# whwu95/MVFNet

Measured on AMD Instinct MI355X. Metric: clips/sec (fwd+bwd) MVFNet-R50 8x8 224^2, higher is better.
Workload: dtype bf16; 1 GPU; MVFNet-ResNet50 8x8, 32 clips/GPU of 8x3x224x224, bf16, train step: fwd (batch-stat BN) + loss + bwd + clip + SGD-nesterov; all through the HIP C ABI (stem + 16 bottlenecks + MVF + TSN head); clips_per_gpu=32, frames_per_clip=8, parallelism=dp1: replicas, one flat gradient all-reduce per step

## Files before the change

### include/mvfnet_hip.h

```cpp
#ifndef MVFNET_HIP_H
#define MVFNET_HIP_H

#include <stddef.h>
#include <stdint.h>

#ifdef __cplusplus
extern "C" {
#endif

#define MVF_ABI_VERSION 2

enum { MVF_OK = 0, MVF_EINVAL = -1, MVF_ESHAPE = -2, MVF_EWS = -3, MVF_EHIP = -4, MVF_EUNSUPPORTED = -5 };
enum { MVF_F32 = 0, MVF_BF16 = 1 };
enum { MVF_NCHW = 0, MVF_NHWC = 1 };
enum { MVF_VIEW_T = 1, MVF_VIEW_H = 2, MVF_VIEW_W = 4 };

int mvf_abi_version(void);
const char* mvf_last_error(void);

typedef struct {
    int32_t nt, c, h, w;
    int32_t n_segment;
    int32_t cs;
    int32_t mode;
// ... 34 lines not shown
    int32_t relu;
    int32_t split_c;
    int32_t x2_pix_stride;
    int32_t in_dil;
    int32_t res_c0;
    int32_t x_c0;
} mvf_conv_desc_t;

int mvf_conv2d_nhwc_fwd(const mvf_conv_desc_t* d, const void* x, const void* x2, const void* w_packed,
                        const float* bias, const void* residual, void* y, void* stream);
size_t mvf_conv2d_workspace_bytes(const mvf_conv_desc_t* d);
int mvf_conv2d_nhwc_fwd_ws(const mvf_conv_desc_t* d, const void* x, const void* x2, const void* w_packed,
                           const float* bias, const void* residual, void* y, void* ws, size_t ws_bytes, void* stream);
int mvf_conv2d_nhwc_fwd_mvf(const mvf_conv_desc_t* d, const void* x, const void* w_packed, const float* bias, const float* mvf_coef,
                            int cs, int n_segment, int act, void* y, void* ws, size_t ws_bytes, void* stream);
int mvf_conv2d_nhwc_fwd_bnapply(const mvf_conv_desc_t* d, const void* x, const void* x2, const void* w_packed, const float* bn_scale,
                                const float* bn_shift, const void* residual, const float* res_scale, const float* res_shift, void* out,
                                unsigned char* sign_bits, void* ws, size_t ws_bytes, void* stream);
int mvf_conv2d_nhwc_fwd_bnbwd_sums(const mvf_conv_desc_t* d, const void* x, const void* x2, const void* w_packed, const void* g,
                                   const unsigned char* sign_bits, const float* bn_mean, const float* bn_invstd, float* sums_part, void* ws,
                                   size_t ws_bytes, void* stream);
int mvf_conv2d_nhwc_fwd_bnbwd_apply(const mvf_conv_desc_t* d, const void* x, const void* x2, const void* w_packed, const void* g,
                                    const unsigned char* sign_bits, const float* bn_gamma, const float* bn_mean, const float* bn_invstd,
                                    const float* dgamma, const float* dbeta, void* dz, void* ws, size_t ws_bytes, void* stream);
int mvf_conv2d_nhwc_fwd_resmask(const mvf_conv_desc_t* d, const void* x, const void* x2, const void* w_packed,
                                const float* bias, const void* residual, const unsigned char* res_sign_bits, void* y,
                                void* ws, size_t ws_bytes, void* stream);
int mvf_conv2d_nhwc_fwd_resmask_gate(const mvf_conv_desc_t* d, const void* x, const void* x2, const void* w_packed, const float* bias,
                                     const void* residual, const unsigned char* res_sign_bits, const unsigned char* out_gate_bits, void* y,
                                     void* ws, size_t ws_bytes, void* stream);
int mvf_conv2d_nhwc_fwd_resmask_gate_colsums(const mvf_conv_desc_t* d, const void* x, const void* x2, const void* w_packed, const void* residual,
                                             const unsigned char* res_sign_bits, const unsigned char* out_gate_bits, void* y, float* sums_part, void* ws,
                                             size_t ws_bytes, void* stream);
int mvf_conv2d_nhwc_dgrad_bnsums(const mvf_conv_desc_t* d, const void* dz, const void* w_packed_dgrad, void* y, const void* bn_z,
                                 const float* bn_mean, const float* bn_invstd, const float* bn_scale, const float* bn_shift,
                                 float* sums_part, void* ws, size_t ws_bytes, void* stream);
int mvf_bn_bwd_finalize(const float* sums_part, int nblk, int c, float* dgamma, float* dbeta, void* stream);
int mvf_conv2d_stats_rows(const mvf_conv_desc_t* d);
int mvf_conv2d_nhwc_fwd_stats(const mvf_conv_desc_t* d, const void* x, const void* x2, const void* w_packed, void* y,
                              float* stats_part, const float* stats_shift, void* ws, size_t ws_bytes, void* stream);

int mvf_pack_conv_weight(const float* w_oihw, int cout, int cin, int kh, int kw, int kw_pad, int cin_pad,
                         const float* scale, void* w_packed, int dtype, void* stream);
int mvf_bn_fold(const float* gamma, const float* beta, const float* mean, const float* var, float eps, int c,
                float* scale, float* shift, void* stream);

int mvf_stem_prep(const float* x_nchw, int n, int c, int h, int w, int pad, int wp, void* out, int dtype, void* stream);

int mvf_frames_prep_u8(const unsigned char* frames_hwc, int n, int hs, int ws, const int* window, int h, int w,
                       const float* mean3, const float* std3, int to_rgb, int div_255, int pad, int wp, void* out_stem,
                       float* out_nchw, int dtype, void* stream);
int mvf_frames_resample_u8(const unsigned char* frames_hwc, int n, int hs, int ws, const int* rows, int h, int w,
                           const float* mean3, const float* std3, int to_rgb, int div_255, int pad, int wp, void* out_stem,
                           float* out_nchw, int dtype, void* stream);
int mvf_frames_resample_color_u8(const unsigned char* frames_hwc, int n, int hs, int ws, const int* rows, const float* color, int h, int w,
                                 const float* mean3, const float* std3, int to_rgb, int div_255, int pad, int wp, void* out_stem,
                                 float* out_nchw, int dtype, void* stream);
int mvf_frames_gather_resample_u8(const unsigned char* frames_hwc, int n_src, int hs, int ws, const int* src_index, int n_out, const int* rows,
                                  const float* color, int h, int w, const float* mean3, const float* std3, int to_rgb, int div_255, int pad,
                                  int wp, void* out_stem, float* out_nchw, int dtype, void* stream);
int mvf_frames_yuv420_gather_resample_u8(const unsigned char* frames, int n_src, int hs, int ws, int pitch, int layout, int standard, int order,
                                         const int* src_index, int n_out, const int* rows, const float* color, int h, int w, const float* mean3,
                                         const float* std3, int to_rgb, int div_255, int pad, int wp, void* out_stem, float* out_nchw, int dtype,
                                         void* stream);

int mvf_maxpool3x3s2_nhwc(const void* x, int n, int h, int w, int c, void* y, int dtype, void* stream);

int mvf_head_pool_fc(const void* feat, int clips, int t, int hw, int c, const float* fc_w, const float* fc_b,
                     int classes, float* pooled_ws, float* scores, int dtype, void* stream);
int mvf_average_clip(const float* scores, int clips, int classes, int kind, float* out, void* stream);

int mvf_conv2d_nhwc_dgrad_bnsums_split(const mvf_conv_desc_t* d, const void* x, const void* x2, const void* w_packed, const float* bias, void* y,
                                       const void* bn_z, const float* bn_mean, const float* bn_invstd, const float* bn_scale, const float* bn_shift,
                                       float* sums_part, void* ws, size_t ws_bytes, void* stream);
int mvf_bn_bwd_dzfree_prep(const void* w_packed_dgrad, int c, int k, const float* gamma, const float* mean, const float* invstd, const float* dgamma,
                           const float* dbeta, long m, void* w_out, float* bias_out, int dtype, void* stream);
int mvf_bn_bwd_dzfree_wgrad(float* dw, const void* w_packed, const float* gram, const float* a_mean, const float* gamma, const float* mean,
                            const float* invstd, const float* dgamma, const float* dbeta, long m, int c, int k, int dtype, void* stream);
int mvf_bn_bwd_dzfree_sums(const float* q, const void* w_packed, int c, int k, const float* mean, const float* invstd, const float* part_lo, int rows_lo,
                           int c_split, const float* part_hi, int rows_hi, float* dgamma, float* dbeta, int dtype, void* stream);
size_t mvf_bn_workspace_bytes(long m, int c);
int mvf_bn_train_stats(const void* z, long m, int c, const float* gamma, const float* beta, float eps, float momentum,
                       float* running_mean, float* running_var, float* save_mean, float* save_invstd, float* scale,
                       float* shift, void* ws, size_t ws_bytes, int dtype, void* stream);
int mvf_bn_train_finalize(const float* part, int nblk, long m, int c, const float* gamma, const float* beta, float eps,
                          float momentum, float* running_mean, float* running_var, float* save_mean, float* save_invstd,
                          float* scale, float* shift, void* stream);
int mvf_bn_train_stats_gram(const float* gram, const float* a_mean, const void* w_packed, long m, int c, int k, const float* gamma, const float* beta,
                            float eps, float momentum, float* running_mean, float* running_var, float* save_mean, float* save_invstd, float* scale,
                            float* shift, int dtype, void* stream);
int mvf_bn_apply_colmeans(const void* z, long m, int c, const float* scale, const float* shift, int act, void* out, float* mean_out, void* ws,
                          size_t ws_bytes, int dtype, void* stream);
int mvf_bn_apply(const void* z, long m, int c, const float* scale, const float* shift, const void* residual,
                 const float* rscale, const float* rshift, int act, void* out, int dtype, void* stream);
int mvf_bn_bwd_reduce(const void* g, int g_pitch, const void* z, const void* ymask, long m, int c, const float* mean,
                      const float* invstd, const float* scale, const float* shift, int mask_mode, void* gm_out,
                      float* dgamma, float* dbeta, void* ws, size_t ws_bytes, int dtype, void* stream);
int mvf_bn_bwd_apply(const void* g, int g_pitch, const void* z, long m, int c, const float* gamma, const float* mean,
                     const float* invstd, const float* scale, const float* shift, const float* dgamma,
                     const float* dbeta, int mask_mode, void* dz, int dtype, void* stream);
int mvf_bn_apply_bits(const void* z, long m, int c, const float* scale, const float* shift, const void* residual,
                      const float* rscale, const float* rshift, int relu, void* out, unsigned char* sign_bits, int dtype,
                      void* stream);
int mvf_bn_bwd_apply_masked(const void* g, int g_pitch, const void* z, const void* ymask, long m, int c, const float* gamma,
                            const float* mean, const float* invstd, const float* scale, const float* shift,
                            const float* dgamma, const float* dbeta, int mask_mode, void* dz, int dtype, void* stream);
int mvf_bn_bwd_pair(const void* g, int g_pitch, const void* z_a, const void* z_b, const unsigned char* sign_bits, long m, int c,
                    const float* gamma_a, const float* mean_a, const float* invstd_a, float* dgamma_a, float* dbeta_a,
                    const float* gamma_b, const float* mean_b, const float* invstd_b, float* dgamma_b, float* dbeta_b,
                    void* dz_a, void* dz_b, void* ws, size_t ws_bytes, int dtype, void* stream);
int mvf_bn_bwd_wgrad_splits(long m, int c, int k, int nbn, int mask_mode);
size_t mvf_bn_bwd_wgrad_slab_bytes(long m, int c, int k, int nbn, int mask_mode);
int mvf_bn_bwd_apply_wgrad(const void* g, int g_pitch, const void* z, const void* ymask, long m, int c, const float* gamma, const float* mean,
                           const float* invstd, const float* scale, const float* shift, const float* dgamma, const float* dbeta, int mask_mode,
                           void* dz, const void* x, int x_pitch, int k, float* slabs, size_t slab_bytes, int dtype, void* stream);
int mvf_bn_bwd_pair_wgrad(const void* g, int g_pitch, const void* z_a, const void* z_b, const unsigned char* sign_bits, long m, int c,
                          const float* gamma_a, const float* mean_a, const float* invstd_a, float* dgamma_a, float* dbeta_a,
                          const float* gamma_b, const float* mean_b, const float* invstd_b, float* dgamma_b, float* dbeta_b,
                          void* dz_a, void* dz_b, const void* x_a, int xa_pitch, const void* x_b, int xb_pitch, int k,
                          float* slabs_a, float* slabs_b, size_t slab_bytes, void* ws, size_t ws_bytes, int dtype, void* stream);
int mvf_conv1x1_bwd_fused_splits(long m, int c, int k);
int mvf_conv1x1_bwd_fused(const void* a_in, int a_pitch, const void* w_packed, const void* g, int g_pitch, const unsigned char* sign_bits, long m, int c,
                          int k, const float* gamma, const float* mean, const float* invstd, const float* dgamma, const float* dbeta, const void* z_in,
                          const float* in_mean, const float* in_invstd, const float* in_scale, const float* in_shift, void* dx, float* sums_part,
                          int sums_rows, float* slabs, size_t slab_bytes, int dtype, void* stream);
int mvf_conv1x1_bnbwd_sums_pair(const void* a_in, int a_pitch, const void* w_a, const void* x_in, int x_pitch, const void* w_b, const void* g, int g_pitch,
                                const unsigned char* sign_bits, long m, int c, int k, const float* mean_a, const float* invstd_a, const float* mean_b,
                                const float* invstd_b, float* part_a, float* part_b, int rows, int dtype, void* stream);
int mvf_wgrad_slab_reduce(const float* slabs, int nsplit, int cout, int k, float* dw_oihw, void* stream);
int mvf_maxpool_bn_relu_fwd(const void* z, int n, int h, int w, int c, const float* scale, const float* shift, void* y,
                            unsigned char* argmax, int dtype, void* stream);
int mvf_maxpool_bn_relu_bwd(const unsigned char* argmax, const void* g, int n, int h, int w, int c, void* ga, int dtype,
                            void* stream);
int mvf_maxpool_bwd_sums_rows(int n, int h);
int mvf_maxpool_bn_relu_bwd_apply(const unsigned char* argmax, const void* g, int n, int h, int w, int c, const void* z, const float* gamma,
                                  const float* mean, const float* invstd, const float* scale, const float* shift, const float* dgamma,
                                  const float* dbeta, void* dz, int dtype, void* stream);
int mvf_maxpool_bn_relu_bwd_sums(const unsigned char* argmax, const void* g, int n, int h, int w, int c, void* ga, const void* z, const float* mean,
                                 const float* invstd, const float* scale, const float* shift, float* sums_part, int dtype, void* stream);
int mvf_head_train_fwd(const void* feat, int clips, int t, int hw, int c, const float* fc_w, const float* fc_b, int classes,
                       const long long* labels, const float* drop_mask ,
                       float* pooled, float* scores, float* dscores, float* loss_part, float* loss, int dtype, void* stream);
int mvf_ce_loss(const float* scores, const long long* labels, int clips, int classes, float* dscores, float* loss_part, float* loss,
                void* stream);
int mvf_head_train_bwd(const float* dscores, const float* pooled, const float* fc_w, const float* drop_mask, int clips, int t,
                       int hw, int c, int classes, float* dfc_w, float* dfc_b, float* dpool_ws , void* dfeat, int dtype,
                       void* stream);
size_t mvf_conv2d_wgrad_workspace_bytes(const mvf_conv_desc_t* d);
int mvf_conv2d_nhwc_wgrad(const mvf_conv_desc_t* d, const void* dz, const void* x, const void* x2, int kw_real,
                          int cin_real, int kw_packed, int cin_packed, float* dw_oihw, void* ws, size_t ws_bytes,
                          void* stream);
int mvf_conv2d_nhwc_wgrad_wgs(const mvf_conv_desc_t* d, const void* dz, const void* x, const void* x2, int kw_real,
                              int cin_real, int kw_packed, int cin_packed, float* dw_oihw, void* ws, size_t ws_bytes, int wgs, void* stream);
typedef struct {
    const float* w;
    void* out;
    int cout, cin, kh, kw, kw_pad, cin_pad;
    int kind, first_block;
} mvf_pack_job_t;
int mvf_pack_conv_weights_batched(const mvf_pack_job_t* jobs_dev, int njobs, int total_blocks, int dtype, void* stream);

int mvf_pack_conv_weight_dgrad(const float* w_oihw, int cout, int cin, int kh, int kw, void* w_packed, int dtype,
                               void* stream);
int mvf_nhwc_stencil(const mvf_desc_t* d, const void* x, int x_c, void* out, int out_c, const float* w_t,
                     const float* w_h, const float* w_w, const float* scale, const float* shift, int flip,
                     const void* addend, int addend_c, const unsigned char* addend_sign_bits, void* stream);
int mvf_nhwc_stencil_gate(const mvf_desc_t* d, const void* x, int x_c, void* out, int out_c, const float* w_t,
                          const float* w_h, const float* w_w, const float* scale, const float* shift, int flip,
                          const void* addend, int addend_c, const unsigned char* addend_sign_bits,
                          const unsigned char* out_gate_bits, void* stream);
int mvf_nhwc_stencil_gate_colsums(const mvf_desc_t* d, const void* x, int x_c, void* out, int out_c, const float* w_t, const float* w_h,
                                  const float* w_w, int flip, const void* addend, int addend_c, const unsigned char* addend_sign_bits,
                                  const unsigned char* out_gate_bits, float* sums_part, void* stream);
int mvf_nhwc_stencil_stats_rows(const mvf_desc_t* d, int x_c, int out_c);
int mvf_nhwc_stencil_tile_plan(const mvf_desc_t* d, int x_c, int out_c, int* rows_per_band, int* chan_per_wg);
int mvf_nhwc_stencil_stats(const mvf_desc_t* d, const void* x, int x_c, void* out, int out_c, const float* w_t, const float* w_h,
                           const float* w_w, float* stats_part, const float* stats_shift, void* stream);
size_t mvf_nhwc_tapgrad_workspace_bytes(const mvf_desc_t* d);
int mvf_nhwc_tapgrad(const mvf_desc_t* d, const void* x, int x_c, const void* dy, int dy_c, float* dw_t, float* dw_h,
                     float* dw_w, void* ws, size_t ws_bytes, void* stream);
size_t mvf_sgd_workspace_bytes(long n);
int mvf_sgd_nesterov_step(float* params, const float* grads, float* momentum_buf, long n, float grad_scale, float max_norm,
                          float lr, float momentum, float weight_decay, int first_step, float* norm_out, void* ws,
                          size_t ws_bytes, void* stream);
typedef struct mvf_sgd_segment {
    long long first;
    float lr_mult, decay_mult;
} mvf_sgd_segment_t;
int mvf_sgd_step_segments(float* params, const float* grads, float* momentum_buf, long n, float grad_scale, float max_norm, float lr,
                          float momentum, float weight_decay, int first_step, int nesterov, const mvf_sgd_segment_t* segments, int nseg,
                          float* norm_out, void* ws, size_t ws_bytes, void* stream);

enum { MVF_PLAN_CALL = 0, MVF_PLAN_RECORD = 1, MVF_PLAN_WAIT = 2 };
typedef struct mvf_plan_op {
    int kind, n_int, n_flt, reserved;
    void* fn;
    long long word0, float0;
} mvf_plan_op_t;
int mvf_plan_run(const mvf_plan_op_t* ops, int n_ops, const unsigned long long* words, const float* floats, int* failed_op);

#ifdef __cplusplus
}
#endif
#endif
```

### mvfnet_amd/_lib.py

```python
import ctypes as C
import os

import torch

_HERE = os.path.dirname(os.path.abspath(__file__))
LIB_PATH = os.environ.get("MVF_LIB_PATH") or os.path.join(_HERE, "libmvfnet_hip.so")

MVF_F32, MVF_BF16 = 0, 1
MVF_NCHW, MVF_NHWC = 0, 1
VIEW_T, VIEW_H, VIEW_W = 1, 2, 4
MODE_BITS = {"T": 1, "TH": 3, "THW": 7}
ERRNAMES = {-1: "MVF_EINVAL", -2: "MVF_ESHAPE", -3: "MVF_EWS", -4: "MVF_EHIP", -5: "MVF_EUNSUPPORTED"}


class MvfDesc(C.Structure):
    _fields_ = [("nt", C.c_int32), ("c", C.c_int32), ("h", C.c_int32), ("w", C.c_int32), ("n_segment", C.c_int32),
                ("cs", C.c_int32), ("mode", C.c_int32), ("layout", C.c_int32), ("dtype", C.c_int32)]


class ConvDesc(C.Structure):
    _fields_ = [("n", C.c_int32), ("h", C.c_int32), ("w", C.c_int32), ("cin", C.c_int32), ("cout", C.c_int32),
                ("kh", C.c_int32), ("kw", C.c_int32), ("stride", C.c_int32), ("pad", C.c_int32),
                ("ho", C.c_int32), ("wo", C.c_int32), ("x_pix_stride", C.c_int32),
                ("dtype", C.c_int32), ("relu", C.c_int32), ("split_c", C.c_int32), ("x2_pix_stride", C.c_int32), ("in_dil", C.c_int32),
# ... 27 lines not shown
    lib.mvf_last_error.restype = C.c_char_p
    lib.mvf_last_error.argtypes = []
    lib.mvf_fwd_infer.restype = i32
    lib.mvf_fwd_infer.argtypes = [dp, vp, vp, fp, fp, fp, fp, fp, vp]
    lib.mvf_fwd_train_workspace_bytes.restype = sz
    lib.mvf_fwd_train_workspace_bytes.argtypes = [dp]
    lib.mvf_fwd_train.restype = i32
    lib.mvf_fwd_train.argtypes = [dp, vp, vp, fp, fp, fp, fp, fp, f32, f32, fp, fp, fp, fp, vp, sz, vp]
    lib.mvf_bwd_workspace_bytes.restype = sz
    lib.mvf_bwd_workspace_bytes.argtypes = [dp]
    lib.mvf_bwd.restype = i32
    lib.mvf_bwd.argtypes = [dp, vp, vp, fp, fp, fp, fp, fp, fp, fp, i32, vp, fp, fp, fp, fp, fp, vp, sz, vp]
    lib.mvf_fwd_infer_slice.restype = i32
    lib.mvf_fwd_infer_slice.argtypes = [dp, vp, vp, fp, fp, fp, fp, fp, vp]
    cp = C.POINTER(ConvDesc)
    lib.mvf_conv2d_nhwc_fwd.restype = i32
    lib.mvf_conv2d_nhwc_fwd.argtypes = [cp, vp, vp, vp, fp, vp, vp, vp]
    lib.mvf_conv2d_workspace_bytes.restype = sz
    lib.mvf_conv2d_workspace_bytes.argtypes = [cp]
    lib.mvf_conv2d_nhwc_fwd_ws.restype = i32
    lib.mvf_conv2d_nhwc_fwd_ws.argtypes = [cp, vp, vp, vp, fp, vp, vp, vp, sz, vp]
    lib.mvf_conv2d_nhwc_dgrad_bnsums.restype = i32
    lib.mvf_conv2d_nhwc_dgrad_bnsums.argtypes = [cp, vp, vp, vp, vp, fp, fp, fp, fp, fp, vp, sz, vp]
    lib.mvf_bn_bwd_finalize.restype = i32
    lib.mvf_bn_bwd_finalize.argtypes = [fp, i32, i32, fp, fp, vp]
    lib.mvf_conv2d_nhwc_fwd_bnapply.restype = i32
    lib.mvf_conv2d_nhwc_fwd_bnapply.argtypes = [cp, vp, vp, vp, fp, fp, vp, fp, fp, vp, vp, vp, sz, vp]
    lib.mvf_conv2d_nhwc_fwd_bnbwd_sums.restype = i32
    lib.mvf_conv2d_nhwc_fwd_bnbwd_sums.argtypes = [cp, vp, vp, vp, vp, vp, fp, fp, fp, vp, sz, vp]
    lib.mvf_conv2d_nhwc_fwd_bnbwd_apply.restype = i32
    lib.mvf_conv2d_nhwc_fwd_bnbwd_apply.argtypes = [cp, vp, vp, vp, vp, vp, fp, fp, fp, fp, fp, vp, vp, sz, vp]
    lib.mvf_conv2d_nhwc_fwd_resmask.restype = i32
    lib.mvf_conv2d_nhwc_fwd_resmask.argtypes = [cp, vp, vp, vp, fp, vp, vp, vp, vp, sz, vp]
    i64_ = C.c_long
    lib.mvf_conv2d_nhwc_fwd_resmask_gate.restype = i32
    lib.mvf_conv2d_nhwc_fwd_resmask_gate.argtypes = [cp, vp, vp, vp, fp, vp, vp, vp, vp, vp, sz, vp]
    lib.mvf_conv2d_nhwc_fwd_resmask_gate_colsums.restype = i32
    lib.mvf_conv2d_nhwc_fwd_resmask_gate_colsums.argtypes = [cp, vp, vp, vp, vp, vp, vp, vp, fp, vp, sz, vp]
    lib.mvf_nhwc_stencil_gate_colsums.restype = i32
    lib.mvf_nhwc_stencil_gate_colsums.argtypes = [dp, vp, i32, vp, i32, fp, fp, fp, i32, vp, i32, vp, vp, fp, vp]
    lib.mvf_conv2d_nhwc_dgrad_bnsums_split.restype = i32
    lib.mvf_conv2d_nhwc_dgrad_bnsums_split.argtypes = [cp, vp, vp, vp, fp, vp, vp, fp, fp, fp, fp, fp, vp, sz, vp]
    lib.mvf_bn_bwd_dzfree_prep.restype = i32
    lib.mvf_bn_bwd_dzfree_prep.argtypes = [vp, i32, i32, fp, fp, fp, fp, fp, i64_, vp, fp, i32, vp]
    lib.mvf_bn_bwd_dzfree_wgrad.restype = i32
    lib.mvf_bn_bwd_dzfree_wgrad.argtypes = [fp, vp, fp, fp, fp, fp, fp, fp, fp, i64_, i32, i32, i32, vp]
    lib.mvf_bn_bwd_dzfree_sums.restype = i32
    lib.mvf_bn_bwd_dzfree_sums.argtypes = [fp, vp, i32, i32, fp, fp, fp, i32, i32, fp, i32, fp, fp, i32, vp]
    lib.mvf_nhwc_stencil_stats_rows.restype = i32
    lib.mvf_nhwc_stencil_stats_rows.argtypes = [dp, i32, i32]
    lib.mvf_nhwc_stencil_tile_plan.restype = i32
    lib.mvf_nhwc_stencil_tile_plan.argtypes = [dp, i32, i32, C.POINTER(C.c_int), C.POINTER(C.c_int)]
    lib.mvf_nhwc_stencil_stats.restype = i32
    lib.mvf_nhwc_stencil_stats.argtypes = [dp, vp, i32, vp, i32, fp, fp, fp, fp, fp, vp]
    lib.mvf_nhwc_stencil_gate.restype = i32
    lib.mvf_nhwc_stencil_gate.argtypes = [dp, vp, i32, vp, i32, fp, fp, fp, fp, fp, i32, vp, i32, vp, vp, vp]
    lib.mvf_conv2d_stats_rows.restype = i32
    lib.mvf_conv2d_stats_rows.argtypes = [cp]
    lib.mvf_conv2d_nhwc_fwd_stats.restype = i32
    lib.mvf_conv2d_nhwc_fwd_stats.argtypes = [cp, vp, vp, vp, vp, fp, fp, vp, sz, vp]
    lib.mvf_pack_conv_weight.restype = i32
    lib.mvf_pack_conv_weight.argtypes = [fp, i32, i32, i32, i32, i32, i32, fp, vp, i32, vp]
    lib.mvf_pack_conv_weights_batched.restype = i32
    lib.mvf_pack_conv_weights_batched.argtypes = [vp, i32, i32, i32, vp]
    lib.mvf_bn_fold.restype = i32
    lib.mvf_bn_fold.argtypes = [fp, fp, fp, fp, f32, i32, fp, fp, vp]
    lib.mvf_stem_prep.restype = i32
    lib.mvf_stem_prep.argtypes = [fp, i32, i32, i32, i32, i32, i32, vp, i32, vp]
    lib.mvf_frames_prep_u8.restype = i32
    lib.mvf_frames_prep_u8.argtypes = [vp, i32, i32, i32, vp, i32, i32, C.POINTER(C.c_float), C.POINTER(C.c_float),
                                       i32, i32, i32, i32, vp, vp, i32, vp]
    lib.mvf_frames_resample_u8.restype = i32
    lib.mvf_frames_resample_u8.argtypes = [vp, i32, i32, i32, vp, i32, i32, C.POINTER(C.c_float), C.POINTER(C.c_float),
                                           i32, i32, i32, i32, vp, vp, i32, vp]
    lib.mvf_frames_resample_color_u8.restype = i32
    lib.mvf_frames_resample_color_u8.argtypes = [vp, i32, i32, i32, vp, vp, i32, i32, C.POINTER(C.c_float), C.POINTER(C.c_float),
                                                 i32, i32, i32, i32, vp, vp, i32, vp]
    lib.mvf_frames_gather_resample_u8.restype = i32
    lib.mvf_frames_gather_resample_u8.argtypes = [vp, i32, i32, i32, vp, i32, vp, vp, i32, i32, C.POINTER(C.c_float), C.POINTER(C.c_float),
                                                  i32, i32, i32, i32, vp, vp, i32, vp]
    lib.mvf_frames_yuv420_gather_resample_u8.restype = i32
    lib.mvf_frames_yuv420_gather_resample_u8.argtypes = [vp, i32, i32, i32, i32, i32, i32, i32, vp, i32, vp, vp, i32, i32, C.POINTER(C.c_float),
                                                         C.POINTER(C.c_float), i32, i32, i32, i32, vp, vp, i32, vp]
    lib.mvf_maxpool3x3s2_nhwc.restype = i32
    lib.mvf_maxpool3x3s2_nhwc.argtypes = [vp, i32, i32, i32, i32, vp, i32, vp]
    lib.mvf_head_pool_fc.restype = i32
    lib.mvf_head_pool_fc.argtypes = [vp, i32, i32, i32, i32, fp, fp, i32, fp, fp, i32, vp]
    lib.mvf_average_clip.restype = i32
    lib.mvf_average_clip.argtypes = [fp, i32, i32, i32, fp, vp]
    i64, ll = C.c_long, C.c_void_p
    lib.mvf_bn_workspace_bytes.restype = sz
    lib.mvf_bn_workspace_bytes.argtypes = [i64, i32]
    lib.mvf_bn_train_stats.restype = i32
    lib.mvf_bn_train_stats.argtypes = [vp, i64, i32, fp, fp, f32, f32, fp, fp, fp, fp, fp, fp, vp, sz, i32, vp]
    lib.mvf_bn_train_finalize.restype = i32
    lib.mvf_bn_train_finalize.argtypes = [fp, i32, i64, i32, fp, fp, f32, f32, fp, fp, fp, fp, fp, fp, vp]
    lib.mvf_bn_train_stats_gram.restype = i32
    lib.mvf_bn_train_stats_gram.argtypes = [fp, fp, vp, i64, i32, i32, fp, fp, f32, f32, fp, fp, fp, fp, fp, fp, i32, vp]
    lib.mvf_bn_apply_colmeans.restype = i32
    lib.mvf_bn_apply_colmeans.argtypes = [vp, i64, i32, fp, fp, i32, vp, fp, vp, sz, i32, vp]
    lib.mvf_bn_apply.restype = i32
    lib.mvf_bn_apply.argtypes = [vp, i64, i32, fp, fp, vp, fp, fp, i32, vp, i32, vp]
    lib.mvf_bn_apply_bits.restype = i32
    lib.mvf_bn_apply_bits.argtypes = [vp, i64, i32, fp, fp, vp, fp, fp, i32, vp, vp, i32, vp]
    lib.mvf_bn_bwd_apply_masked.restype = i32
    lib.mvf_bn_bwd_apply_masked.argtypes = [vp, i32, vp, vp, i64, i32, fp, fp, fp, fp, fp, fp, fp, i32, vp, i32, vp]
    lib.mvf_bn_bwd_reduce.restype = i32
    lib.mvf_bn_bwd_reduce.argtypes = [vp, i32, vp, vp, i64, i32, fp, fp, fp, fp, i32, vp, fp, fp, vp, sz, i32, vp]
    lib.mvf_bn_bwd_apply.restype = i32
    lib.mvf_bn_bwd_apply.argtypes = [vp, i32, vp, i64, i32, fp, fp, fp, fp, fp, fp, fp, i32, vp, i32, vp]
    lib.mvf_maxpool_bn_relu_fwd.restype = i32
    lib.mvf_maxpool_bn_relu_fwd.argtypes = [vp, i32, i32, i32, i32, fp, fp, vp, vp, i32, vp]
    lib.mvf_maxpool_bn_relu_bwd.restype = i32
    lib.mvf_maxpool_bn_relu_bwd.argtypes = [vp, vp, i32, i32, i32, i32, vp, i32, vp]
    lib.mvf_maxpool_bwd_sums_rows.restype = i32
    lib.mvf_maxpool_bwd_sums_rows.argtypes = [i32, i32]
    lib.mvf_maxpool_bn_relu_bwd_apply.restype = i32
    lib.mvf_maxpool_bn_relu_bwd_apply.argtypes = [vp, vp, i32, i32, i32, i32, vp, fp, fp, fp, fp, fp, fp, fp, vp, i32, vp]
    lib.mvf_maxpool_bn_relu_bwd_sums.restype = i32
    lib.mvf_maxpool_bn_relu_bwd_sums.argtypes = [vp, vp, i32, i32, i32, i32, vp, vp, fp, fp, fp, fp, fp, i32, vp]
    lib.mvf_head_train_fwd.restype = i32
    lib.mvf_head_train_fwd.argtypes = [vp, i32, i32, i32, i32, fp, fp, i32, ll, fp, fp, fp, fp, fp, fp, i32, vp]
    lib.mvf_conv2d_nhwc_fwd_mvf.restype = i32
    lib.mvf_conv2d_nhwc_fwd_mvf.argtypes = [cp, vp, vp, fp, fp, i32, i32, i32, vp, vp, sz, vp]
    lib.mvf_bn_bwd_pair.restype = i32
    lib.mvf_bn_bwd_pair.argtypes = [vp, i32, vp, vp, vp, i64, i32, fp, fp, fp, fp, fp, fp, fp, fp, fp, fp, vp, vp, vp, sz, i32, vp]
    lib.mvf_bn_bwd_wgrad_splits.restype = i32
    lib.mvf_bn_bwd_wgrad_splits.argtypes = [i64, i32, i32, i32, i32]
    lib.mvf_bn_bwd_wgrad_slab_bytes.restype = sz
    lib.mvf_bn_bwd_wgrad_slab_bytes.argtypes = [i64, i32, i32, i32, i32]
    lib.mvf_bn_bwd_apply_wgrad.restype = i32
    lib.mvf_bn_bwd_apply_wgrad.argtypes = [vp, i32, vp, vp, i64, i32, fp, fp, fp, fp, fp, fp, fp, i32, vp, vp, i32, i32, fp, sz, i32, vp]
    lib.mvf_bn_bwd_pair_wgrad.restype = i32
    lib.mvf_bn_bwd_pair_wgrad.argtypes = [vp, i32, vp, vp, vp, i64, i32, fp, fp, fp, fp, fp, fp, fp, fp, fp, fp, vp, vp, vp, i32, vp, i32, i32,
                                          fp, fp, sz, vp, sz, i32, vp]
    lib.mvf_conv1x1_bwd_fused_splits.restype = i32
    lib.mvf_conv1x1_bwd_fused_splits.argtypes = [i64, i32, i32]
    lib.mvf_conv1x1_bwd_fused.restype = i32
    lib.mvf_conv1x1_bwd_fused.argtypes = [vp, i32, vp, vp, i32, vp, i64, i32, i32, fp, fp, fp, fp, fp, vp, fp, fp, fp, fp, vp, fp, i32, fp, sz, i32, vp]
    lib.mvf_conv1x1_bnbwd_sums_pair.restype = i32
    lib.mvf_conv1x1_bnbwd_sums_pair.argtypes = [vp, i32, vp, vp, i32, vp, vp, i32, vp, i64, i32, i32, fp, fp, fp, fp, fp, fp, i32, i32, vp]
    lib.mvf_wgrad_slab_reduce.restype = i32
    lib.mvf_wgrad_slab_reduce.argtypes = [fp, i32, i32, i32, fp, vp]
    lib.mvf_ce_loss.restype = i32
    lib.mvf_ce_loss.argtypes = [fp, ll, i32, i32, fp, fp, fp, vp]
    lib.mvf_head_train_bwd.restype = i32
    lib.mvf_head_train_bwd.argtypes = [fp, fp, fp, fp, i32, i32, i32, i32, i32, fp, fp, fp, vp, i32, vp]
    lib.mvf_conv2d_wgrad_workspace_bytes.restype = sz
    lib.mvf_conv2d_wgrad_workspace_bytes.argtypes = [cp]
    lib.mvf_conv2d_nhwc_wgrad.restype = i32
    lib.mvf_conv2d_nhwc_wgrad.argtypes = [cp, vp, vp, vp, i32, i32, i32, i32, fp, vp, sz, vp]
    lib.mvf_conv2d_nhwc_wgrad_wgs.restype = i32
    lib.mvf_conv2d_nhwc_wgrad_wgs.argtypes = [cp, vp, vp, vp, i32, i32, i32, i32, fp, vp, sz, i32, vp]
    lib.mvf_pack_conv_weight_dgrad.restype = i32
    lib.mvf_pack_conv_weight_dgrad.argtypes = [fp, i32, i32, i32, i32, vp, i32, vp]
    lib.mvf_nhwc_stencil.restype = i32
    lib.mvf_nhwc_stencil.argtypes = [dp, vp, i32, vp, i32, fp, fp, fp, fp, fp, i32, vp, i32, vp, vp]
    lib.mvf_nhwc_tapgrad_workspace_bytes.restype = sz
    lib.mvf_nhwc_tapgrad_workspace_bytes.argtypes = [dp]
    lib.mvf_nhwc_tapgrad.restype = i32
    lib.mvf_nhwc_tapgrad.argtypes = [dp, vp, i32, vp, i32, fp, fp, fp, vp, sz, vp]
    lib.mvf_sgd_workspace_bytes.restype = sz
    lib.mvf_sgd_workspace_bytes.argtypes = [i64]
    lib.mvf_sgd_nesterov_step.restype = i32
    lib.mvf_sgd_nesterov_step.argtypes = [fp, fp, fp, i64, f32, f32, f32, f32, f32, i32, fp, vp, sz, vp]
    lib.mvf_sgd_step_segments.restype = i32
    lib.mvf_sgd_step_segments.argtypes = [fp, fp, fp, i64, f32, f32, f32, f32, f32, i32, i32, vp, i32, fp, vp, sz, vp]
    lib.mvf_plan_run.restype = i32
    lib.mvf_plan_run.argtypes = [C.POINTER(PlanOp), i32, C.POINTER(C.c_ulonglong), C.POINTER(C.c_float), C.POINTER(C.c_int)]
    missing = [n for n in declared_symbols() if hasattr(lib, n) and getattr(lib, n).argtypes is None]
    if missing:
        raise ImportError("mvfnet_amd._lib: no argtypes declared for %s" % missing)
    return lib


def check(rc, what=""):
    if rc != 0:
        msg = lib.mvf_last_error().decode("utf-8", "replace")
        raise RuntimeError("%s failed: %s (%s)" % (what or "libmvfnet_hip", ERRNAMES.get(rc, rc), msg))


def declared_symbols():
    import re
    hdr = os.path.join(os.path.dirname(_HERE), "include", "mvfnet_hip.h")
    txt = open(hdr).read()
    txt = re.sub(r"/\*.*?\*/", "", txt, flags=re.S)
    return sorted(set(re.findall(r"\b((?:mvf|mvfnet)_[a-z0-9_]+)\s*\(", txt)))


lib = _load()
```

### mvfnet_amd/csrc/common.h

```cpp
#pragma once
#include <hip/hip_runtime.h>
#include <stdlib.h>
#include <string.h>
#include <strings.h>
#include <stdint.h>
#include <stdio.h>

#include "mvfnet_hip.h"

void mvf_set_error(const char* fmt, ...);

#define MVF_HIP_OK(call)                                                                        \
    do {                                                                                        \
        hipError_t e__ = (call);                                                                \
        if (e__ != hipSuccess) {                                                                \
            mvf_set_error("%s:%d: %s -> %s", __FILE__, __LINE__, #call, hipGetErrorString(e__)); \
            return MVF_EHIP;                                                                    \
        }                                                                                       \
    } while (0)

#define MVF_REQUIRE(cond, code, ...)    \
    do {                                \
        if (!(cond)) {                  \
            mvf_set_error(__VA_ARGS__); \
            return (code);              \
        }                               \
    } while (0)

#define MVF_LAUNCH_CHECK()                                                              \
    do {                                                                                \
        hipError_t e__ = hipGetLastError();                                             \
        if (e__ != hipSuccess) {                                                        \
            mvf_set_error("%s:%d: launch -> %s", __FILE__, __LINE__, hipGetErrorString(e__)); \
            return MVF_EHIP;                                                            \
        }                                                                               \
    } while (0)

struct bf16_t {
    uint16_t v;
};

__device__ __forceinline__ float bf16_to_f32(uint16_t v) { return __uint_as_float(((uint32_t)v) << 16); }
typedef __bf16 mvf_bf16x2 __attribute__((ext_vector_type(2)));
typedef float mvf_f32x2 __attribute__((ext_vector_type(2)));
__device__ __forceinline__ uint32_t pack_bf16x2(float lo, float hi) {
    const mvf_f32x2 v = {lo, hi};
    const mvf_bf16x2 b = __builtin_convertvector(v, mvf_bf16x2);
    uint32_t u;
    __builtin_memcpy(&u, &b, 4);
    return u;
}
__device__ __forceinline__ uint16_t f32_to_bf16(float f) { return (uint16_t)(pack_bf16x2(f, 0.f) & 0xffffu); }

__device__ __forceinline__ float ldf(const float* p) { return *p; }
__device__ __forceinline__ float ldf(const bf16_t* p) { return bf16_to_f32(p->v); }
__device__ __forceinline__ void stf(float* p, float v) { *p = v; }
__device__ __forceinline__ void stf(bf16_t* p, float v) { p->v = f32_to_bf16(v); }

__device__ __forceinline__ float4 ld4(const float* p) { return *reinterpret_cast<const float4*>(p); }
__device__ __forceinline__ float4 ld4(const bf16_t* p) {
    uint2 r = *reinterpret_cast<const uint2*>(p);
    return make_float4(__uint_as_float(r.x << 16), __uint_as_float(r.x & 0xffff0000u),
                       __uint_as_float(r.y << 16), __uint_as_float(r.y & 0xffff0000u));
}
__device__ __forceinline__ void st4(float* p, float4 v) { *reinterpret_cast<float4*>(p) = v; }
__device__ __forceinline__ void st4(bf16_t* p, float4 v) {
    uint2 r;
    r.x = pack_bf16x2(v.x, v.y);
    r.y = pack_bf16x2(v.z, v.w);
    *reinterpret_cast<uint2*>(p) = r;
}

__device__ __forceinline__ float hswish_f(float u) { return u * fminf(fmaxf(u + 3.0f, 0.0f), 6.0f) * (1.0f / 6.0f); }
__device__ __forceinline__ float hswish_grad_f(float u) {
    float r6 = fminf(fmaxf(u + 3.0f, 0.0f), 6.0f);
    float inner = (u > -3.0f && u < 3.0f) ? 1.0f : 0.0f;
    return r6 * (1.0f / 6.0f) + u * inner * (1.0f / 6.0f);
}

static inline size_t align_up(size_t v, size_t a) { return (v + a - 1) / a * a; }

static inline bool mvf_policy_lookup(const char* name, long* out) {
    const char* p = getenv("MVF_POLICY");
    if (!p) return false;
    const size_t n = strlen(name);
    while (*p) {
        while (*p == ',' || *p == ';' || *p == ' ') ++p;
        const char* e = p;
        while (*e && *e != ',' && *e != ';') ++e;
        const char* eq = (const char*)memchr(p, '=', (size_t)(e - p));
        if (eq && (size_t)(eq - p) == n && strncasecmp(p, name, n) == 0) {
            *out = strtol(eq + 1, nullptr, 10);
            return true;
        }
        p = e;
    }
    return false;
}
static inline int mvf_policy_int(const char* name, int dflt) {
    long v;
    return mvf_policy_lookup(name, &v) ? (int)v : dflt;
}
static inline bool mvf_policy_has(const char* name) {
    long v;
    return mvf_policy_lookup(name, &v);
}

struct StemDirectArgs {
    const void* x;
    const void* w;
    void* y;
    const float* bias;
    float* stats_part;
    const float* stats_shift;
    int stats_rows, epi;
    int N, H, W, Ho, Wo;
    long wK;
};
struct Conv3x3C64Args {
    const void* x;
    const void* w;
    void* y;
    const float* bias;
    float* stats_part;
    const float* stats_shift;
    const void* bn_z;
    const float *bn_mean, *bn_invstd, *bn_scale, *bn_shift;
    int stats_rows, epi;
    int N, H, W, xps;
    long wK;
};
struct PwSumsArgs {
    const void* a;
    const void* w;
    const void* g;
    const unsigned char* bits;
    const float* c0;
    const float* c1;
    float* part;
    int rows, mode, M, N, K, xps;
};
struct Wgrad3x3C64Args {
    const void* dz;
    const void* x;
    float* part;
    int N, H, W, xps, nwg;
};
struct WgradStemArgs {
    const void* dz;
    const void* x;
    float* part;
    int N, H, W, Ho, Wo, nwg;
};
namespace mvf_internal {
struct BnBwdWgradArgs {
    const void* g;
    const void* z[2];
    const void* bits;
    const float *gamma[2], *mean[2], *invstd[2], *dgamma[2], *dbeta[2];
    const float *scale, *shift;
    void* dz[2];
    const void* x[2];
    int xps[2];
    float* part[2];
    int g_pitch, M, C, K;
    int rows_per_split, nsplit, ctiles, ktiles;
};
struct PwBwdFusedArgs {
    const void* a;
    const void* w;
    const void* g;
    const unsigned char* bits;
    const float *gamma, *mean, *invstd, *dgamma, *dbeta;
    const void* z_in;
    const float *in_scale, *in_shift, *in_mean, *in_invstd;
    void* dx;
    float* sums_part;
    float* part;
    int aps, g_pitch, M, sums_rows, rows_per_split, nsplit;
    int ablate;
};
struct PwSumsPairArgs {
    const void *a, *x;
    const void *w_a, *w_b;
    const void* g;
    const unsigned char* bits;
    const float *mean_a, *invstd_a, *mean_b, *invstd_b;
    float *part_a, *part_b;
    int aps, xps, g_pitch, M, rows, rows_per_split, nsplit;
};
int pw_sums_pair_launch(const PwSumsPairArgs& a, hipStream_t st);
int pw_bwd_fused_plan(long m, int c, int k, int* rows_per_split);
int pw_bwd_fused_launch(const PwBwdFusedArgs& a, hipStream_t st);
bool bnbwd_wgrad_tile(int c, int k, int nbn, int mask_mode, int* ct, int* kt);
int bnbwd_wgrad_plan(long m, int c, int k, int nbn, int mask_mode, int* rows_per_split, int* ctiles, int* ktiles);
int bnbwd_wgrad_launch(const BnBwdWgradArgs& a, int nbn, int mask_mode, hipStream_t st);
int wgrad_slab_reduce_launch(const float* part, int nsplit, int cout, int k, float* dw_oihw, hipStream_t st);
bool wgrad3x3_c64_ok(int n, int h, int w, int xps);
int wgrad3x3_c64_wgs(int n, int h);
int wgrad3x3_c64_launch(const Wgrad3x3C64Args& a, hipStream_t st);
bool wgrad_stem_ok(int n, int h, int w, int ho, int wo);
int wgrad_stem_wgs(int n, int ho);
int wgrad_stem_launch(const WgradStemArgs& a, hipStream_t st);
int stem_direct_launch(const StemDirectArgs& a, hipStream_t st);
int conv3x3_c64_launch(const Conv3x3C64Args& a, hipStream_t st);
int pw_sums_launch(const PwSumsArgs& a, hipStream_t st);
}

#ifdef __HIPCC__
typedef int i32x4 __attribute__((ext_vector_type(4)));
__device__ __forceinline__ i32x4 rsrc_words(const void* base, unsigned nbytes) {
    const unsigned long p = (unsigned long)base;
    i32x4 r;
    r.x = __builtin_amdgcn_readfirstlane((int)(unsigned)p);
    r.y = __builtin_amdgcn_readfirstlane((int)((unsigned)(p >> 32) & 0xffffu));
    r.z = __builtin_amdgcn_readfirstlane((int)nbytes);
    r.w = 0x00020000;
    return r;
}
__device__ __forceinline__ void glds16(const i32x4 rs, const unsigned lds_dst, const unsigned voff) {
    unsigned keep;
    asm volatile("s_mov_b32 %0, m0\n\ts_mov_b32 m0, %2\n\ts_nop 0\n\tbuffer_load_dwordx4 %1, %3, 0 offen lds\n\ts_mov_b32 m0, %0"
                 : "=&s"(keep) : "v"(voff), "s"(lds_dst), "s"(rs) : "memory");
}

#endif
```

### mvfnet_amd/csrc/train_ops.hip

```cpp
#include <algorithm>
#include <math.h>
#include <stdlib.h>

#include "common.h"

namespace {

constexpr int kThreads = 256;

struct ColPlan {
    int cqb;
    int rl;
    int gx;
    int gy;
    int rows;
};

ColPlan col_plan(long M, int C, int vn = 4, int blocks = 2048) {
    ColPlan p;
    const int cq = C / vn;
    int cqb = 1;
    while (cqb < cq && cqb < 64) cqb <<= 1;
    p.cqb = cqb;
    p.rl = kThreads / cqb;
    p.gx = (cq + cqb - 1) / cqb;
    long want = std::max<long>(1, blocks / p.gx);
    long rows = std::max<long>((M + want - 1) / want, (long)p.rl * 8);
    rows = (rows + p.rl - 1) / p.rl * p.rl;
    p.rows = (int)rows;
    p.gy = (int)((M + rows - 1) / rows);
    return p;
}

template <typename ET, int VN>
__device__ __forceinline__ void ldv(const ET* p, float (&f)[VN]) {
    if constexpr (sizeof(ET) == 4) {
        static_assert(VN == 4, "fp32 lane vector is 4 wide");
        const float4 v = *reinterpret_cast<const float4*>(p);
        f[0] = v.x; f[1] = v.y; f[2] = v.z; f[3] = v.w;
    } else if constexpr (VN == 4) {
        const uint2 r = *reinterpret_cast<const uint2*>(p);
        f[0] = __uint_as_float(r.x << 16); f[1] = __uint_as_float(r.x & 0xffff0000u);
        f[2] = __uint_as_float(r.y << 16); f[3] = __uint_as_float(r.y & 0xffff0000u);
    } else {
        static_assert(VN == 8, "bf16 lane vector is 4 or 8 wide");
        const uint4 r = *reinterpret_cast<const uint4*>(p);
        f[0] = __uint_as_float(r.x << 16); f[1] = __uint_as_float(r.x & 0xffff0000u);
        f[2] = __uint_as_float(r.y << 16); f[3] = __uint_as_float(r.y & 0xffff0000u);
        f[4] = __uint_as_float(r.z << 16); f[5] = __uint_as_float(r.z & 0xffff0000u);
        f[6] = __uint_as_float(r.w << 16); f[7] = __uint_as_float(r.w & 0xffff0000u);
    }
}
template <typename ET, int VN>
__device__ __forceinline__ void stv(ET* p, const float (&f)[VN]) {
    if constexpr (sizeof(ET) == 4) {
        *reinterpret_cast<float4*>(p) = make_float4(f[0], f[1], f[2], f[3]);
    } else if constexpr (VN == 4) {
        uint2 r;
        r.x = pack_bf16x2(f[0], f[1]);
        r.y = pack_bf16x2(f[2], f[3]);
        *reinterpret_cast<uint2*>(p) = r;
    } else {
        uint4 r;
        r.x = pack_bf16x2(f[0], f[1]);
        r.y = pack_bf16x2(f[2], f[3]);
        r.z = pack_bf16x2(f[4], f[5]);
        r.w = pack_bf16x2(f[6], f[7]);
        *reinterpret_cast<uint4*>(p) = r;
    }
}
template <int VN>
__device__ __forceinline__ void ldp(const float* p, int c, float (&f)[VN], float fill = 0.f) {
#pragma unroll
    for (int j = 0; j < VN; j += 4) {
        const float4 v = p ? *reinterpret_cast<const float4*>(p + c + j) : make_float4(fill, fill, fill, fill);
        f[j] = v.x; f[j + 1] = v.y; f[j + 2] = v.z; f[j + 3] = v.w;
    }
}

template <int VN>
__device__ __forceinline__ void rowlane_reduce(float (&a)[VN], float (&b)[VN], int cqb, int rl, float* red) {
    (void)rl;
    const int lane = threadIdx.x & 63, wave = threadIdx.x >> 6, cq = lane % cqb;
    for (int off = cqb; off < 64; off <<= 1) {
#pragma unroll
        for (int j = 0; j < VN; ++j) {
            a[j] += __shfl_xor(a[j], off, 64);
            b[j] += __shfl_xor(b[j], off, 64);
        }
    }
    if (lane < cqb) {
#pragma unroll
        for (int j = 0; j < VN; ++j) {
            red[((wave * 2 * VN) + 2 * j) * cqb + cq] = a[j];
            red[((wave * 2 * VN) + 2 * j + 1) * cqb + cq] = b[j];
        }
    }
    __syncthreads();
    if (threadIdx.x < cqb) {
#pragma unroll
        for (int j = 0; j < VN; ++j) {
            float s = 0.f, t = 0.f;
#pragma unroll
            for (int w = 0; w < kThreads / 64; ++w) {
                s += red[((w * 2 * VN) + 2 * j) * cqb + cq];
                t += red[((w * 2 * VN) + 2 * j + 1) * cqb + cq];
            }
            a[j] = s;
            b[j] = t;
        }
    }
}

template <typename ET, int VN>
__global__ __launch_bounds__(kThreads) void bn_stats_kernel(const ET* z, long M, int C, const float* kshift, int cqb, int rows,
                                                            float* part) {
    __shared__ float red[2 * VN * kThreads];
    const int rl = kThreads / cqb;
    const int cq = blockIdx.x * cqb + threadIdx.x % cqb, lane_r = threadIdx.x / cqb;
    const bool ok = cq * VN < C;
    const int c = cq * VN;
    float k[VN], s1[VN], s2[VN];
#pragma unroll
    for (int j = 0; j < VN; ++j) k[j] = s1[j] = s2[j] = 0.f;
    if (ok && kshift) ldp<VN>(kshift, c, k);
    const long r0 = (long)blockIdx.y * rows, r1 = min(M, r0 + rows);
    if (ok) {
        auto accum = [&](const float (&a)[VN]) {
#pragma unroll
            for (int j = 0; j < VN; ++j) {
                const float d = a[j] - k[j];
                s1[j] += d;
                s2[j] += d * d;
            }
        };
        long r = r0 + lane_r;
        for (; r + 3 * rl < r1; r += 4 * rl) {
            float a0[VN], a1[VN], a2[VN], a3[VN];
            ldv<ET, VN>(z + r * C + c, a0); ldv<ET, VN>(z + (r + rl) * C + c, a1);
            ldv<ET, VN>(z + (r + 2 * rl) * C + c, a2); ldv<ET, VN>(z + (r + 3 * rl) * C + c, a3);
            accum(a0); accum(a1); accum(a2); accum(a3);
        }
        for (; r < r1; r += rl) {
            float a0[VN];
            ldv<ET, VN>(z + r * C + c, a0);
            accum(a0);
        }
    }
    rowlane_reduce<VN>(s1, s2, cqb, rl, red);
    if (ok && lane_r == 0) {
        float* p = part + ((long)blockIdx.y * C + c) * 2;
#pragma unroll
        for (int j = 0; j < VN; ++j) { p[2 * j] = s1[j]; p[2 * j + 1] = s2[j]; }
    }
}

constexpr int kFinCh = 4;
// ... 624 lines not shown
template <typename ET>
__global__ __launch_bounds__(256) void maxpool_bn_bwd_rows_sums_kernel(const unsigned char* amax, const ET* g, int n, int h, int w, int c, int ho, int wo, ET* ga,
                                                                       const ET* z, const float* mean, const float* invstd, const float* scale, const float* shift,
                                                                       float* part, int nblk) {
    __shared__ float red[256 * 8];
    const int c4 = c >> 2;
    const int per = w * c4;
    const int cq = threadIdx.x % c4;
    const float4 sc = *reinterpret_cast<const float4*>(scale + cq * 4), sh = *reinterpret_cast<const float4*>(shift + cq * 4);
    const float4 mu = *reinterpret_cast<const float4*>(mean + cq * 4), rs = *reinterpret_cast<const float4*>(invstd + cq * 4);
    float s1[4] = {0.f, 0.f, 0.f, 0.f}, s2[4] = {0.f, 0.f, 0.f, 0.f};
    const int row_end = min(n * h, ((int)blockIdx.x + 1) * kPoolRB);
    for (int row = blockIdx.x * kPoolRB; row < row_end; ++row) {
        const int img = row / h, ih = row - img * h;
        for (int i = threadIdx.x; i < per; i += 256) {
            const int iw = i / c4;
            float acc[4] = {0.f, 0.f, 0.f, 0.f};
            unsigned amv[4];
            float4 gvv[4];
            bool okv[4];
            unsigned mev[4];
            const long zi = ((long)row * w + iw) * c + cq * 4;
            const float4 zv = ld4(z + zi);
#pragma unroll
            for (int k = 0; k < 4; ++k) {
                const int oh = (ih + (k >> 1)) >> 1, ow = (iw + (k & 1)) >> 1;
                okv[k] = oh < ho && ow < wo && ((k >> 1) == 0 || (ih & 1)) && ((k & 1) == 0 || (iw & 1));
                const int ohc = min(oh, ho - 1), owc = min(ow, wo - 1);
                mev[k] = (unsigned)(ih - (oh * 2 - 1)) * 3u + (unsigned)(iw - (ow * 2 - 1));
                const long oidx = (((long)img * ho + ohc) * wo + owc) * c + cq * 4;
                amv[k] = *reinterpret_cast<const unsigned*>(amax + oidx);
                gvv[k] = ld4(g + oidx);
            }
#pragma unroll
            for (int k = 0; k < 4; ++k) {
                const unsigned am = amv[k], me = mev[k];
                if (okv[k] && (am & 255u) == me) acc[0] += gvv[k].x;
                if (okv[k] && ((am >> 8) & 255u) == me) acc[1] += gvv[k].y;
                if (okv[k] && ((am >> 16) & 255u) == me) acc[2] += gvv[k].z;
                if (okv[k] && (am >> 24) == me) acc[3] += gvv[k].w;
            }
            if (ga) st4(ga + zi, make_float4(acc[0], acc[1], acc[2], acc[3]));
            if constexpr (sizeof(ET) == 2) {
#pragma unroll
                for (int j = 0; j < 4; ++j) acc[j] = bf16_to_f32(f32_to_bf16(acc[j]));
            }
            const float zz[4] = {zv.x, zv.y, zv.z, zv.w};
            const float scv[4] = {sc.x, sc.y, sc.z, sc.w}, shv[4] = {sh.x, sh.y, sh.z, sh.w};
            const float muv[4] = {mu.x, mu.y, mu.z, mu.w}, rsv[4] = {rs.x, rs.y, rs.z, rs.w};
#pragma unroll
            for (int j = 0; j < 4; ++j) {
                const float gm = (zz[j] * scv[j] + shv[j]) > 0.f ? acc[j] : 0.f;
                s1[j] += gm;
                s2[j] += gm * ((zz[j] - muv[j]) * rsv[j]);
            }
        }
    }
#pragma unroll
    for (int j = 0; j < 4; ++j) {
        red[(2 * j) * 256 + threadIdx.x] = s1[j];
        red[(2 * j + 1) * 256 + threadIdx.x] = s2[j];
    }
    __syncthreads();
    if ((int)threadIdx.x < c4 * 4) {
        const int q = threadIdx.x >> 2, j = threadIdx.x & 3;
        float a = 0.f, b = 0.f;
        for (int t = q; t < 256; t += c4) {
            a += red[(2 * j) * 256 + t];
            b += red[(2 * j + 1) * 256 + t];
        }
        reinterpret_cast<float2*>(part)[(long)(q * 4 + j) * nblk + blockIdx.x] = make_float2(a, b);
    }
}

template <typename ET>
__global__ __launch_bounds__(256) void maxpool_bn_bwd_rows_apply_kernel(const unsigned char* amax, const ET* g, int n, int h, int w, int c, int ho, int wo,
                                                                        const ET* z, const float* gamma, const float* mean, const float* invstd,
                                                                        const float* scale, const float* shift, const float* dgamma, const float* dbeta,
                                                                        float inv_m, ET* dz) {
    const int c4 = c >> 2;
    const int per = w * c4;
    const int cq = threadIdx.x % c4;
    float av[4], d0[4], kx[4], muv[4], scv[4], shv[4];
    {
        const float4 ga_ = *reinterpret_cast<const float4*>(gamma + cq * 4), rs = *reinterpret_cast<const float4*>(invstd + cq * 4);
        const float4 dg = *reinterpret_cast<const float4*>(dgamma + cq * 4), db = *reinterpret_cast<const float4*>(dbeta + cq * 4);
        const float4 mu = *reinterpret_cast<const float4*>(mean + cq * 4);
        const float4 sc = *reinterpret_cast<const float4*>(scale + cq * 4), sh = *reinterpret_cast<const float4*>(shift + cq * 4);
        const float gav[4] = {ga_.x, ga_.y, ga_.z, ga_.w}, rsv[4] = {rs.x, rs.y, rs.z, rs.w}, dgv[4] = {dg.x, dg.y, dg.z, dg.w}, dbv[4] = {db.x, db.y, db.z, db.w};
        const float mu_[4] = {mu.x, mu.y, mu.z, mu.w}, sc_[4] = {sc.x, sc.y, sc.z, sc.w}, sh_[4] = {sh.x, sh.y, sh.z, sh.w};
#pragma unroll
        for (int j = 0; j < 4; ++j) {
            av[j] = gav[j] * rsv[j];
            d0[j] = dbv[j] * inv_m;
            kx[j] = rsv[j] * dgv[j] * inv_m;
            muv[j] = mu_[j]; scv[j] = sc_[j]; shv[j] = sh_[j];
        }
    }
    const int row_end = min(n * h, ((int)blockIdx.x + 1) * kPoolRB);
    for (int row = blockIdx.x * kPoolRB; row < row_end; ++row) {
        const int img = row / h, ih = row - img * h;
        for (int i = threadIdx.x; i < per; i += 256) {
            const int iw = i / c4;
            float acc[4] = {0.f, 0.f, 0.f, 0.f};
            unsigned amv[4];
            float4 gvv[4];
            bool okv[4];
            unsigned mev[4];
            const long zi = ((long)row * w + iw) * c + cq * 4;
            const float4 zv = ld4(z + zi);
#pragma unroll
            for (int k = 0; k < 4; ++k) {
                const int oh = (ih + (k >> 1)) >> 1, ow = (iw + (k & 1)) >> 1;
                okv[k] = oh < ho && ow < wo && ((k >> 1) == 0 || (ih & 1)) && ((k & 1) == 0 || (iw & 1));
                const int ohc = min(oh, ho - 1), owc = min(ow, wo - 1);
                mev[k] = (unsigned)(ih - (oh * 2 - 1)) * 3u + (unsigned)(iw - (ow * 2 - 1));
                const long oidx = (((long)img * ho + ohc) * wo + owc) * c + cq * 4;
                amv[k] = *reinterpret_cast<const unsigned*>(amax + oidx);
                gvv[k] = ld4(g + oidx);
            }
#pragma unroll
            for (int k = 0; k < 4; ++k) {
                const unsigned am = amv[k], me = mev[k];
                if (okv[k] && (am & 255u) == me) acc[0] += gvv[k].x;
                if (okv[k] && ((am >> 8) & 255u) == me) acc[1] += gvv[k].y;
                if (okv[k] && ((am >> 16) & 255u) == me) acc[2] += gvv[k].z;
                if (okv[k] && (am >> 24) == me) acc[3] += gvv[k].w;
            }
            if constexpr (sizeof(ET) == 2) {
#pragma unroll
                for (int j = 0; j < 4; ++j) acc[j] = bf16_to_f32(f32_to_bf16(acc[j]));
            }
            const float zz[4] = {zv.x, zv.y, zv.z, zv.w};
            float o[4];
#pragma unroll
            for (int j = 0; j < 4; ++j) {
                const float gm = (zz[j] * scv[j] + shv[j]) > 0.f ? acc[j] : 0.f;
                o[j] = av[j] * (gm - d0[j] - (zz[j] - muv[j]) * kx[j]);
            }
            st4(dz + zi, make_float4(o[0], o[1], o[2], o[3]));
        }
    }
}

template <typename ET, int MODE>
__global__ __launch_bounds__(256) void maxpool_bn_bwd_blk_kernel(const unsigned char* amax, const ET* g, int n, int h, int w, int c, int ho, int wo, ET* ga,
                                                                 const ET* z, const float* gamma, const float* mean, const float* invstd, const float* scale,
                                                                 const float* shift, const float* dgamma, const float* dbeta, float inv_m, float* part, int nblk,
                                                                 ET* dz) {
    constexpr int VC = 16 / (int)sizeof(ET);
    __shared__ float red[MODE == 0 ? 256 * 2 * VC : 1];
    const int ncg = c / VC, hw2 = w >> 1, hb = h >> 1;
    const int cq = threadIdx.x % ncg;
    float scv[VC], shv[VC], muv[VC], k1[VC], k2[VC], k3[VC];
#pragma unroll
    for (int j = 0; j < VC; ++j) {
        const int ch = cq * VC + j;
        scv[j] = scale[ch]; shv[j] = shift[ch]; muv[j] = mean[ch];
        if constexpr (MODE == 0) { k1[j] = invstd[ch]; k2[j] = 0.f; k3[j] = 0.f; }
        else { k1[j] = gamma[ch] * invstd[ch]; k2[j] = dbeta[ch] * inv_m; k3[j] = invstd[ch] * dgamma[ch] * inv_m; }
    }
    float s1[VC], s2[VC];
#pragma unroll
    for (int j = 0; j < VC; ++j) { s1[j] = 0.f; s2[j] = 0.f; }
    auto ldv = [](const ET* p, float (&f)[VC]) {
        const uint4 u = *reinterpret_cast<const uint4*>(p);
        if constexpr (sizeof(ET) == 4) {
            f[0] = __uint_as_float(u.x); f[1] = __uint_as_float(u.y); f[2] = __uint_as_float(u.z); f[3] = __uint_as_float(u.w);
        } else {
            f[0] = __uint_as_float(u.x << 16); f[1] = __uint_as_float(u.x & 0xffff0000u); f[2] = __uint_as_float(u.y << 16); f[3] = __uint_as_float(u.y & 0xffff0000u);
            f[4] = __uint_as_float(u.z << 16); f[5] = __uint_as_float(u.z & 0xffff0000u); f[6] = __uint_as_float(u.w << 16); f[7] = __uint_as_float(u.w & 0xffff0000u);
        }
    };
    auto stv = [](ET* p, const float (&f)[VC]) {
        uint4 u;
        if constexpr (sizeof(ET) == 4) {
            u = make_uint4(__float_as_uint(f[0]), __float_as_uint(f[1]), __float_as_uint(f[2]), __float_as_uint(f[3]));
        } else {
            u = make_uint4(pack_bf16x2(f[0], f[1]), pack_bf16x2(f[2], f[3]), pack_bf16x2(f[4], f[5]), pack_bf16x2(f[6], f[7]));
        }
        *reinterpret_cast<uint4*>(p) = u;
    };
    const int items = (kPoolRB / 2) * hw2 * ncg;
    const long brows = (long)n * hb;
    for (int i = threadIdx.x; i < items; i += 256) {
        const int bi = i / ncg;
        const int br = bi / hw2, bw = bi - br * hw2;
        const long R = (long)blockIdx.x * (kPoolRB / 2) + br;
        if (R >= brows) break;
        const int img = (int)(R / hb), bh = (int)(R - (long)img * hb);
        float gv[4][VC], zv[4][VC];
        unsigned char am[4][VC];
        bool okw[4];
#pragma unroll
        for (int k = 0; k < 4; ++k) {
            const int oh = bh + (k >> 1), ow = bw + (k & 1);
            okw[k] = oh < ho && ow < wo;
            const long oidx = (((long)img * ho + min(oh, ho - 1)) * wo + min(ow, wo - 1)) * c + cq * VC;
            if constexpr (VC == 8) {
                const uint2 a8 = *reinterpret_cast<const uint2*>(amax + oidx);
#pragma unroll
                for (int j = 0; j < 4; ++j) { am[k][j] = (unsigned char)(a8.x >> (8 * j)); am[k][4 + j] = (unsigned char)(a8.y >> (8 * j)); }
            } else {
                const unsigned a4 = *reinterpret_cast<const unsigned*>(amax + oidx);
#pragma unroll
                for (int j = 0; j < 4; ++j) am[k][j] = (unsigned char)(a4 >> (8 * j));
            }
            ldv(g + oidx, gv[k]);
        }
        long zi[4];
#pragma unroll
        for (int p = 0; p < 4; ++p) {
            zi[p] = (((long)img * h + 2 * bh + (p >> 1)) * w + 2 * bw + (p & 1)) * c + cq * VC;
            ldv(z + zi[p], zv[p]);
        }
#pragma unroll
        for (int p = 0; p < 4; ++p) {
            const int a = p >> 1, b = p & 1;
            float acc[VC];
#pragma unroll
            for (int j = 0; j < VC; ++j) acc[j] = 0.f;
#pragma unroll
            for (int k = 0; k < 4; ++k) {
                const int wi = k >> 1, wj = k & 1;
                if ((wi == 1 && a == 0) || (wj == 1 && b == 0)) continue;
                const unsigned me = (unsigned)(a + 1 - 2 * wi) * 3u + (unsigned)(b + 1 - 2 * wj);
#pragma unroll
                for (int j = 0; j < VC; ++j)
                    if (okw[k] && am[k][j] == me) acc[j] += gv[k][j];
            }
            if constexpr (MODE == 0) {
                if (ga) stv(ga + zi[p], acc);
            }
            if constexpr (sizeof(ET) == 2) {
#pragma unroll
                for (int j = 0; j < VC; ++j) acc[j] = bf16_to_f32(f32_to_bf16(acc[j]));
            }
            if constexpr (MODE == 0) {
#pragma unroll
                for (int j = 0; j < VC; ++j) {
                    const float gm = (zv[p][j] * scv[j] + shv[j]) > 0.f ? acc[j] : 0.f;
                    s1[j] += gm;
                    s2[j] += gm * ((zv[p][j] - muv[j]) * k1[j]);
                }
            } else {
                float o[VC];
#pragma unroll
                for (int j = 0; j < VC; ++j) {
                    const float gm = (zv[p][j] * scv[j] + shv[j]) > 0.f ? acc[j] : 0.f;
                    o[j] = k1[j] * (gm - k2[j] - (zv[p][j] - muv[j]) * k3[j]);
                }
                stv(dz + zi[p], o);
            }
        }
    }
    if constexpr (MODE == 0) {
#pragma unroll
        for (int j = 0; j < VC; ++j) {
            red[(2 * j) * 256 + threadIdx.x] = s1[j];
            red[(2 * j + 1) * 256 + threadIdx.x] = s2[j];
        }
        __syncthreads();
        if ((int)threadIdx.x < c) {
            const int q = threadIdx.x / VC, j = threadIdx.x - q * VC;
            float a = 0.f, b = 0.f;
            for (int t = q; t < 256; t += ncg) {
                a += red[(2 * j) * 256 + t];
                b += red[(2 * j + 1) * 256 + t];
            }
            reinterpret_cast<float2*>(part)[(long)threadIdx.x * nblk + blockIdx.x] = make_float2(a, b);
        }
    }
}

template <typename ET>
__global__ void maxpool_bn_bwd_kernel(const unsigned char* amax, const ET* g, int n, int h, int w, int c, int ho, int wo, ET* ga) {
    const int c4 = c >> 2;
    const long total = (long)n * h * w * c4;
    for (long i = (long)blockIdx.x * blockDim.x + threadIdx.x; i < total; i += (long)gridDim.x * blockDim.x) {
        int cq, iw, ih, img;
        if (total <= 0x7fffffffL) {
            unsigned t = (unsigned)i;
            cq = (int)(t % (unsigned)c4); t /= (unsigned)c4;
            iw = (int)(t % (unsigned)w); t /= (unsigned)w;
            ih = (int)(t % (unsigned)h);
            img = (int)(t / (unsigned)h);
        } else {
            cq = (int)(i % c4);
            long t = i / c4;
            iw = (int)(t % w); t /= w;
            ih = (int)(t % h);
            img = (int)(t / h);
        }
        float acc[4] = {0.f, 0.f, 0.f, 0.f};
        unsigned amv[4];
        float4 gvv[4];
        bool okv[4];
        unsigned mev[4];
#pragma unroll
        for (int k = 0; k < 4; ++k) {
            const int oh = (ih + (k >> 1)) >> 1, ow = (iw + (k & 1)) >> 1;
            okv[k] = oh < ho && ow < wo && ((k >> 1) == 0 || (ih & 1)) && ((k & 1) == 0 || (iw & 1));
            const int ohc = min(oh, ho - 1), owc = min(ow, wo - 1);
            mev[k] = (unsigned)(ih - (oh * 2 - 1)) * 3u + (unsigned)(iw - (ow * 2 - 1));
            const long oidx = (((long)img * ho + ohc) * wo + owc) * c + cq * 4;
            amv[k] = *reinterpret_cast<const unsigned*>(amax + oidx);
            gvv[k] = ld4(g + oidx);
        }
#pragma unroll
        for (int k = 0; k < 4; ++k) {
            const unsigned am = amv[k], me = mev[k];
            if (okv[k] && (am & 255u) == me) acc[0] += gvv[k].x;
            if (okv[k] && ((am >> 8) & 255u) == me) acc[1] += gvv[k].y;
            if (okv[k] && ((am >> 16) & 255u) == me) acc[2] += gvv[k].z;
            if (okv[k] && (am >> 24) == me) acc[3] += gvv[k].w;
        }
        st4(ga + i * 4, make_float4(acc[0], acc[1], acc[2], acc[3]));
    }
}

template <typename ET>
__global__ void frame_pool_kernel(const ET* feat, int hw, int c, const float* drop_mask, float* pooled) {
    const int f = blockIdx.y, ch = blockIdx.x * blockDim.x + threadIdx.x;
    if (ch >= c) return;
    const ET* p = feat + (long)f * hw * c + ch;
    float s = 0.f;
    for (int r = 0; r < hw; ++r) s += ldf(p + (long)r * c);
    s = s / (float)hw;
    if (drop_mask) s *= drop_mask[(long)f * c + ch];
    pooled[(long)f * c + ch] = s;
}

__global__ void ce_loss_kernel(const float* scores, const long long* labels, int clips, int classes, float* loss_part, float* dscores) {
    __shared__ float red[256];
    const int cl = blockIdx.x, tid = threadIdx.x;
    const float* s = scores + (long)cl * classes;
    float mx = -INFINITY;
    for (int k = tid; k < classes; k += blockDim.x) mx = fmaxf(mx, s[k]);
    red[tid] = mx;
    __syncthreads();
    for (int o = blockDim.x >> 1; o > 0; o >>= 1) { if (tid < o) red[tid] = fmaxf(red[tid], red[tid + o]); __syncthreads(); }
    mx = red[0];
    __syncthreads();
    float e = 0.f;
    for (int k = tid; k < classes; k += blockDim.x) e += expf(s[k] - mx);
    red[tid] = e;
    __syncthreads();
    for (int o = blockDim.x >> 1; o > 0; o >>= 1) { if (tid < o) red[tid] += red[tid + o]; __syncthreads(); }
    const float den = red[0];
    const int lab = (int)labels[cl];
    if (tid == 0) loss_part[cl] = (logf(den) + mx) - s[lab];
    if (!dscores) return;
    for (int k = tid; k < classes; k += blockDim.x) {
        const float p = expf(s[k] - mx) / den;
        dscores[(long)cl * classes + k] = (p - (k == lab ? 1.f : 0.f)) / (float)clips;
    }
}

__global__ void mean_reduce_kernel(const float* v, int n, float* out) {
    if (blockIdx.x == 0 && threadIdx.x == 0) {
        double s = 0.0;
        for (int i = 0; i < n; ++i) s += v[i];
        out[0] = (float)(s / n);
    }
}

constexpr int kHeadKc = 4;
__global__ void head_clipmean_kernel(const float* pooled, int T, int c, float* pcm) {
    const int cl = blockIdx.y, ch = blockIdx.x * blockDim.x + threadIdx.x;
    if (ch >= c) return;
    float s = 0.f;
    for (int t = 0; t < T; ++t) s += pooled[((long)cl * T + t) * c + ch];
    pcm[(long)cl * c + ch] = s / (float)T;
}
__global__ __launch_bounds__(256) void head_fc_bwd_w_kernel(const float* dscores, const float* pcm, int clips, int T, int c, int classes, float* dw, float* db) {
    const int k0 = blockIdx.y * kHeadKc, ch = blockIdx.x * blockDim.x + threadIdx.x;
    const int nk = min(kHeadKc, classes - k0);
    if (ch < c) {
        float acc[kHeadKc];
#pragma unroll
        for (int j = 0; j < kHeadKc; ++j) acc[j] = 0.f;
        for (int cl0 = 0; cl0 < clips; cl0 += 16) {
            float pcv[16];
#pragma unroll
            for (int q = 0; q < 16; ++q) pcv[q] = pcm[(long)min(cl0 + q, clips - 1) * c + ch];
#pragma unroll
            for (int j = 0; j < kHeadKc; ++j) {
                if (j < nk) {
#pragma unroll
                    for (int q = 0; q < 16; ++q)
                        if (cl0 + q < clips) acc[j] += dscores[(long)(cl0 + q) * classes + k0 + j] * pcv[q];
                }
            }
        }
#pragma unroll
        for (int j = 0; j < kHeadKc; ++j)
            if (j < nk) dw[(long)(k0 + j) * c + ch] = acc[j];
    }
    if (blockIdx.x == 0 && threadIdx.x < nk) {
        float s = 0.f;
        for (int cl = 0; cl < clips; ++cl) s += dscores[(long)cl * classes + k0 + threadIdx.x];
        db[k0 + threadIdx.x] = s;
    }
}

__global__ void head_dpool_kernel(const float* dscores, const float* w, int classes, int c, float scale, float* dpool) {
    const int cl = blockIdx.y, ch = blockIdx.x * blockDim.x + threadIdx.x;
    if (ch >= c) return;
    float a[8] = {0.f, 0.f, 0.f, 0.f, 0.f, 0.f, 0.f, 0.f};
    const float* ds = dscores + (long)cl * classes;
    int k = 0;
    for (; k + 8 <= classes; k += 8) {
#pragma unroll
        for (int u = 0; u < 8; ++u) a[u] += ds[k + u] * w[(long)(k + u) * c + ch];
    }
    for (; k < classes; ++k) a[0] += ds[k] * w[(long)k * c + ch];
    dpool[(long)cl * c + ch] = (((a[0] + a[1]) + (a[2] + a[3])) + ((a[4] + a[5]) + (a[6] + a[7]))) * scale;
}
template <typename ET>
__global__ void head_dfeat_kernel(const float* dpool, const float* drop_mask, int T, int hw, int c, long total, ET* dfeat) {
    const int frame = blockIdx.y, c4 = c >> 2;
    const int per = hw * c4;
    for (int i = blockIdx.x * blockDim.x + threadIdx.x; i < per; i += gridDim.x * blockDim.x) {
        const int q = i % c4;
        float4 v = *reinterpret_cast<const float4*>(dpool + (long)(frame / T) * c + q * 4);
        if (drop_mask) {
            const float4 mk = *reinterpret_cast<const float4*>(drop_mask + (long)frame * c + q * 4);
            v.x *= mk.x; v.y *= mk.y; v.z *= mk.z; v.w *= mk.w;
        }
        st4(dfeat + ((long)frame * hw * c + (long)i * 4), v);
    }
}

__global__ void sqsum_partial_kernel(const float* g, long n, float* part) {
    __shared__ float red[256];
    float s = 0.f;
    for (long i = (long)blockIdx.x * blockDim.x + threadIdx.x; i < n; i += (long)gridDim.x * blockDim.x) s += g[i] * g[i];
    red[threadIdx.x] = s;
    __syncthreads();
    for (int o = blockDim.x >> 1; o > 0; o >>= 1) { if (threadIdx.x < o) red[threadIdx.x] += red[threadIdx.x + o]; __syncthreads(); }
    if (threadIdx.x == 0) part[blockIdx.x] = red[0];
}
__global__ void norm_finalize_kernel(const float* part, int nblk, float max_norm, float gscale, float* out ) {
    __shared__ double red[64];
    double acc = 0.0;
    for (int i = threadIdx.x; i < nblk; i += 64) acc += part[i];
    red[threadIdx.x] = acc;
    __syncthreads();
    if (blockIdx.x == 0 && threadIdx.x == 0) {
        double s = 0.0;
        for (int i = 0; i < 64; ++i) s += red[i];
        const float nrm = fabsf(gscale) * (float)sqrt(s);
        out[0] = nrm;
        float coef = max_norm > 0.f ? max_norm / (nrm + 1e-6f) : 1.f;
        out[1] = coef < 1.f ? coef : 1.f;
    }
}
__global__ void sgd_nesterov_kernel(float* p, const float* g, float* buf, long n, const float* coef_ptr, float gscale, float lr,
                                    float momentum, float wd, int first_step) {
    const float coef = (coef_ptr ? coef_ptr[1] : 1.f) * gscale;
    for (long i = (long)blockIdx.x * blockDim.x + threadIdx.x; i < n; i += (long)gridDim.x * blockDim.x) {
        const float pv = p[i];
        const float d = g[i] * coef + wd * pv;
        const float b = first_step ? d : momentum * buf[i] + d;
        buf[i] = b;
        p[i] = pv - lr * (d + momentum * b);
    }
}
__device__ __forceinline__ int seg_of(const mvf_sgd_segment_t* seg, int nseg, long i) {
    int lo = 0, hi = nseg - 1;
    while (lo < hi) {
        const int mid = (lo + hi + 1) >> 1;
        if (seg[mid].first <= i) lo = mid; else hi = mid - 1;
    }
    return lo;
}
__global__ void sqsum_segments_kernel(const float* g, long n, const mvf_sgd_segment_t* seg, int nseg, float* part) {
    __shared__ float red[256];
    float s = 0.f;
    for (long i = (long)blockIdx.x * blockDim.x + threadIdx.x; i < n; i += (long)gridDim.x * blockDim.x)
        if (seg[seg_of(seg, nseg, i)].lr_mult >= 0.f) s += g[i] * g[i];
    red[threadIdx.x] = s;
    __syncthreads();
    for (int o = blockDim.x >> 1; o > 0; o >>= 1) { if (threadIdx.x < o) red[threadIdx.x] += red[threadIdx.x + o]; __syncthreads(); }
    if (threadIdx.x == 0) part[blockIdx.x] = red[0];
}
__global__ void sgd_segments_kernel(float* p, const float* g, float* buf, long n, const float* coef_ptr, float gscale, float lr,
                                    float momentum, float wd, int first_step, int nesterov, const mvf_sgd_segment_t* seg, int nseg) {
    const float coef = (coef_ptr ? coef_ptr[1] : 1.f) * gscale;
    for (long i = (long)blockIdx.x * blockDim.x + threadIdx.x; i < n; i += (long)gridDim.x * blockDim.x) {
        const int lo = seg_of(seg, nseg, i);
        if (seg[lo].lr_mult < 0.f) continue;
        const float lr_i = lr * seg[lo].lr_mult, wd_i = wd * seg[lo].decay_mult;
        const float pv = p[i];
        const float d = g[i] * coef + wd_i * pv;
        const float b = first_step ? d : momentum * buf[i] + d;
        buf[i] = b;
        p[i] = pv - lr_i * (nesterov ? d + momentum * b : b);
    }
}

inline int grid_for(long total, int cap = 256 * 16) { return (int)std::min<long>((total + 255) / 256, cap); }

}

extern "C" {

size_t mvf_bn_workspace_bytes(long m, int c) {
    if (m <= 0 || c <= 0 || c % 4) return 0;
    int gy = col_plan(m, c, 4).gy;
    if (c % 8 == 0) gy = std::max(gy, col_plan(m, c, 8).gy);
    return align_up((size_t)gy * c * 2 * sizeof(float), 256);
}

#define MVF_BN_DISPATCH(KERNEL, WIDE_OK, BLOCKS, ...)                                                                        \
    do {                                                                                                                     \
        if (dtype == MVF_F32) {                                                                                              \
            using ET = float;                                                                                                \
            const ColPlan p = col_plan(m, c, 4, BLOCKS);                                                                     \
            hipLaunchKernelGGL((KERNEL<float, 4>), dim3(p.gx, p.gy), dim3(kThreads), 0, st, __VA_ARGS__);                    \
        } else if (WIDE_OK) {                                                                                                \
            using ET = bf16_t;                                                                                               \
            const ColPlan p = col_plan(m, c, 8, BLOCKS);                                                                     \
            hipLaunchKernelGGL((KERNEL<bf16_t, 8>), dim3(p.gx, p.gy), dim3(kThreads), 0, st, __VA_ARGS__);                   \
        } else {                                                                                                             \
            using ET = bf16_t;                                                                                               \
            const ColPlan p = col_plan(m, c, 4, BLOCKS);                                                                     \
            hipLaunchKernelGGL((KERNEL<bf16_t, 4>), dim3(p.gx, p.gy), dim3(kThreads), 0, st, __VA_ARGS__);                   \
        }                                                                                                                    \
    } while (0)

#define MVF_BN_DISPATCH_MM1(KERNEL, MMV, WIDE_OK, BLOCKS, ...)                                                               \
    do {                                                                                                                     \
        if (dtype == MVF_F32) {                                                                                              \
            using ET = float;                                                                                                \
            const ColPlan p = col_plan(m, c, 4, BLOCKS);                                                                     \
            hipLaunchKernelGGL((KERNEL<float, 4, MMV>), dim3(p.gx, p.gy), dim3(kThreads), 0, st, __VA_ARGS__);               \
        } else if (WIDE_OK) {                                                                                                \
            using ET = bf16_t;                                                                                               \
            const ColPlan p = col_plan(m, c, 8, BLOCKS);                                                                     \
            hipLaunchKernelGGL((KERNEL<bf16_t, 8, MMV>), dim3(p.gx, p.gy), dim3(kThreads), 0, st, __VA_ARGS__);              \
        } else {                                                                                                             \
            using ET = bf16_t;                                                                                               \
            const ColPlan p = col_plan(m, c, 4, BLOCKS);                                                                     \
            hipLaunchKernelGGL((KERNEL<bf16_t, 4, MMV>), dim3(p.gx, p.gy), dim3(kThreads), 0, st, __VA_ARGS__);              \
        }                                                                                                                    \
    } while (0)
#define MVF_BN_DISPATCH_MM(KERNEL, MODE, WIDE_OK, BLOCKS, ...)                                \
    do {                                                                                      \
        switch (MODE) {                                                                       \
            case 0: MVF_BN_DISPATCH_MM1(KERNEL, 0, WIDE_OK, BLOCKS, __VA_ARGS__); break;      \
            case 1: MVF_BN_DISPATCH_MM1(KERNEL, 1, WIDE_OK, BLOCKS, __VA_ARGS__); break;      \
            case 2: MVF_BN_DISPATCH_MM1(KERNEL, 2, WIDE_OK, BLOCKS, __VA_ARGS__); break;      \
            case 3: MVF_BN_DISPATCH_MM1(KERNEL, 3, WIDE_OK, BLOCKS, __VA_ARGS__); break;      \
            default: MVF_BN_DISPATCH_MM1(KERNEL, 4, WIDE_OK, BLOCKS, __VA_ARGS__); break;     \
        }                                                                                     \
    } while (0)

constexpr int kFinLongRows = 1024;
static inline bool al16(const void* p) { return ((uintptr_t)p & 15) == 0; }

int mvf_bn_train_stats(const void* z, long m, int c, const float* gamma, const float* beta, float eps, float momentum,
                       float* running_mean, float* running_var, float* save_mean, float* save_invstd, float* scale,
                       float* shift, void* ws, size_t ws_bytes, int dtype, void* stream) {
    MVF_REQUIRE(z && gamma && beta && save_mean && save_invstd && scale && shift && m > 0 && c > 0 && c % 4 == 0, MVF_EINVAL, "bn_train_stats: bad argument (c %% 4?)");
    MVF_REQUIRE(ws && ws_bytes >= mvf_bn_workspace_bytes(m, c), MVF_EWS, "bn_train_stats: workspace too small");
    hipStream_t st = (hipStream_t)stream;
    float* part = (float*)ws;
    const bool wide = c % 8 == 0 && al16(z);
    const int gy = col_plan(m, c, (dtype != MVF_F32 && wide) ? 8 : 4).gy;
    MVF_BN_DISPATCH(bn_stats_kernel, wide, 2048, (const ET*)z, m, c, running_mean, p.cqb, p.rows, part);
    MVF_LAUNCH_CHECK();
    hipLaunchKernelGGL(bn_stats_finalize_kernel<0>, dim3((c + kFinCh - 1) / kFinCh), dim3(256), 0, st, c, gy, m, part, gamma, beta, eps, momentum,
                       running_mean, running_var, save_mean, save_invstd, scale, shift);
    MVF_LAUNCH_CHECK();
    return MVF_OK;
}

int mvf_bn_train_finalize(const float* part, int nblk, long m, int c, const float* gamma, const float* beta, float eps,
                          float momentum, float* running_mean, float* running_var, float* save_mean, float* save_invstd,
                          float* scale, float* shift, void* stream) {
    MVF_REQUIRE(part && gamma && beta && save_mean && save_invstd && scale && shift && nblk > 0 && m > 0 && c > 0, MVF_EINVAL, "bn_train_finalize: bad argument");
    if (nblk >= kFinLongRows)
        hipLaunchKernelGGL(bn_stats_finalize_kernel<1>, dim3(c), dim3(256), 0, (hipStream_t)stream, c, nblk, m, part, gamma, beta, eps, momentum,
                           running_mean, running_var, save_mean, save_invstd, scale, shift);
    else
        hipLaunchKernelGGL(bn_stats_finalize_kernel<2>, dim3((c + 3) / 4), dim3(256), 0, (hipStream_t)stream, c, nblk, m, part, gamma, beta, eps, momentum,
                           running_mean, running_var, save_mean, save_invstd, scale, shift);
    MVF_LAUNCH_CHECK();
    return MVF_OK;
}

int mvf_bn_apply_bits(const void* z, long m, int c, const float* scale, const float* shift, const void* residual,
                      const float* rscale, const float* rshift, int relu, void* out, unsigned char* sign_bits, int dtype,
                      void* stream) {
    MVF_REQUIRE(z && scale && shift && out && m > 0 && c > 0 && c % 4 == 0, MVF_EINVAL, "bn_apply: bad argument");
    MVF_REQUIRE((rscale == nullptr) == (rshift == nullptr), MVF_EINVAL, "bn_apply: rscale/rshift must come together");
    hipStream_t st = (hipStream_t)stream;
    const bool wide = c % 8 == 0 && al16(z) && al16(out) && al16(residual) && ((uintptr_t)sign_bits & 1) == 0;
    MVF_BN_DISPATCH(bn_apply_kernel, wide, 4096, (const ET*)z, m, c, scale, shift, (const ET*)residual, rscale, rshift, relu, (ET*)out, sign_bits,
                    p.cqb, p.rows);
    MVF_LAUNCH_CHECK();
    return MVF_OK;
}

int mvf_bn_apply_colmeans(const void* z, long m, int c, const float* scale, const float* shift, int act, void* out, float* mean_out, void* ws, size_t ws_bytes,
                          int dtype, void* stream) {
    MVF_REQUIRE(z && scale && shift && out && mean_out && ws && m > 0 && c > 0 && c % 8 == 0, MVF_EINVAL, "bn_apply_colmeans: bad argument (c %% 8?)");
    MVF_REQUIRE(al16(z) && al16(out), MVF_EINVAL, "bn_apply_colmeans: z / out must be 16-byte aligned");
    hipStream_t st = (hipStream_t)stream;
    const int gy = col_plan(m, c, dtype == MVF_F32 ? 4 : 8, 4096).gy;
    MVF_REQUIRE(ws_bytes >= (size_t)gy * c * 2 * sizeof(float), MVF_EWS, "bn_apply_colmeans: workspace too small (%d partial rows)", gy);
    float* part = (float*)ws;
    const bool wide = true;
    MVF_BN_DISPATCH(bn_apply_cs_kernel, wide, 4096, (const ET*)z, m, c, scale, shift, act, (ET*)out, p.cqb, p.rows, part);
    MVF_LAUNCH_CHECK();
    hipLaunchKernelGGL(colmean_finalize_kernel, dim3((c + kFinCh - 1) / kFinCh), dim3(256), 0, st, c, gy, m, part, mean_out);
    MVF_LAUNCH_CHECK();
    return MVF_OK;
}

int mvf_bn_apply(const void* z, long m, int c, const float* scale, const float* shift, const void* residual,
                 const float* rscale, const float* rshift, int relu, void* out, int dtype, void* stream) {
    return mvf_bn_apply_bits(z, m, c, scale, shift, residual, rscale, rshift, relu, out, nullptr, dtype, stream);
}

int mvf_bn_bwd_reduce(const void* g, int g_pitch, const void* z, const void* ymask, long m, int c, const float* mean, const float* invstd,
                      const float* scale, const float* shift, int mask_mode, void* gm_out, float* dgamma, float* dbeta,
                      void* ws, size_t ws_bytes, int dtype, void* stream) {
    MVF_REQUIRE(g && z && mean && invstd && dgamma && dbeta && m > 0 && c > 0 && c % 4 == 0, MVF_EINVAL, "bn_bwd_reduce: bad argument");
    MVF_REQUIRE(mask_mode >= 0 && mask_mode <= 4 && ((mask_mode != 1 && mask_mode != 4) || ymask) &&
                    ((mask_mode != 2 && mask_mode != 3) || (scale && shift)) && g_pitch >= c && g_pitch % 4 == 0,
                MVF_EINVAL, "bn_bwd_reduce: bad mask_mode / pitch");
// ... 459 lines not shown
```

### mvfnet_amd/csrc/wgrad_nhwc.hip

```cpp
#include <algorithm>

#include <stdlib.h>

#include "common.h"

namespace {

constexpr int kThreads = 256;
constexpr int BMR = 32;
typedef float f32x16 __attribute__((ext_vector_type(16)));

struct WgArgs {
    const void* dz;
    const void* x;
    const void* x2;
    float* part;
    int N, H, W, Cin, Cout, KH, KW, stride, pad, Ho, Wo, xps, split_c, x2ps;
    int M, K, rows_per_split, tiles_k;
    int tiles, nsplit;
    unsigned fd_hw_mul, fd_hw_shr, fd_w_mul, fd_w_shr;
    int xcd_rr;
    int abl;
};

// ... 955 lines not shown
}

int launch_wgrad_bf16_big(const WgArgs& a, int tiles, int nsplit, hipStream_t st) {
    constexpr size_t lds = (size_t)2 * BMR16 * (256 * 2 + 256 * 2);
    auto kd = wgrad_bf16_kernel<2, 4, true, 4>;
    auto kp = wgrad_bf16_p4_kernel;
    static bool attr_d = false;
    if (!attr_d) {
        MVF_HIP_OK(hipFuncSetAttribute((const void*)kd, hipFuncAttributeMaxDynamicSharedMemorySize, (int)lds));
        MVF_HIP_OK(hipFuncSetAttribute((const void*)kp, hipFuncAttributeMaxDynamicSharedMemorySize, (int)lds));
        attr_d = true;
    }
    static const int p4_on = mvf_policy_int("wgrad_p4", 1);
    if (p4_on && a.Cin % 64 == 0) {
        hipLaunchKernelGGL(kp, dim3(nsplit * tiles), dim3(512), lds, st, a);
        MVF_LAUNCH_CHECK();
        return MVF_OK;
    }
    hipLaunchKernelGGL(kd, dim3(nsplit * tiles), dim3(512), lds, st, a);
    MVF_LAUNCH_CHECK();
    return MVF_OK;
}

__global__ __launch_bounds__(256) void wgrad_reduce1_kernel(const float* part, int nsplit, int cout, int cin, int kh, int kw, int kwp, int cinp,
                                    float* dw) {
    __shared__ float red[4][64];
    const long K = (long)kh * kwp * cinp;
    const long total = (long)cout * K;
    const int e = threadIdx.x & 63, sl = threadIdx.x >> 6;
    const long i = (long)blockIdx.x * 64 + e;
    float s0 = 0.f, s1 = 0.f, s2 = 0.f, s3 = 0.f;
    if (i < total) {
        int k = sl;
        for (; k + 12 < nsplit; k += 16) {
            s0 += part[(long)k * total + i];
            s1 += part[(long)(k + 4) * total + i];
            s2 += part[(long)(k + 8) * total + i];
            s3 += part[(long)(k + 12) * total + i];
        }
        for (; k < nsplit; k += 4) s0 += part[(long)k * total + i];
    }
    red[sl][e] = (s0 + s1) + (s2 + s3);
    __syncthreads();
    if (sl == 0 && i < total) {
        long t = i;
        const int ci = (int)(t % cinp); t /= cinp;
        const int x = (int)(t % kwp); t /= kwp;
        const int y = (int)(t % kh);
        const int co = (int)(t / kh);
        if (ci < cin && x < kw) dw[(((long)co * cin + ci) * kh + y) * kw + x] = (red[0][e] + red[1][e]) + (red[2][e] + red[3][e]);
    }
}
int launch_wgrad_reduce(const float* part, int nsplit, int cout, int cin, int kh, int kw, int kwp, int cinp, float* dw, hipStream_t st) {
    const long total = (long)cout * kh * kwp * cinp;
    hipLaunchKernelGGL(wgrad_reduce1_kernel, dim3((int)((total + 63) / 64)), dim3(256), 0, st, part, nsplit, cout, cin, kh, kw, kwp, cinp, dw);
    MVF_LAUNCH_CHECK();
    return MVF_OK;
}

template <typename ET>
__global__ void pack_dgrad_weight_kernel(const float* w, int cout, int cin, int kh, int kw, ET* out) {
    const long total = (long)cin * kh * kw * cout;
    for (long i = (long)blockIdx.x * blockDim.x + threadIdx.x; i < total; i += (long)gridDim.x * blockDim.x) {
        long t = i;
        const int co = (int)(t % cout); t /= cout;
        const int x = (int)(t % kw); t /= kw;
        const int y = (int)(t % kh);
        const int ci = (int)(t / kh);
        stf(out + i, w[(((long)co * cin + ci) * kh + (kh - 1 - y)) * kw + (kw - 1 - x)]);
    }
}

constexpr int kPackT = 32, kPackTapsMax = 9;
template <typename ET>
__global__ __launch_bounds__(256) void pack_batched_kernel(const mvf_pack_job_t* jobs, int njobs) {
    __shared__ float tile[kPackT * (kPackT * kPackTapsMax + 1)];
    int lo = 0, hi = njobs - 1;
    while (lo < hi) {
        const int mid = (lo + hi + 1) >> 1;
        if (jobs[mid].first_block <= (int)blockIdx.x) lo = mid; else hi = mid - 1;
    }
    const mvf_pack_job_t j = jobs[lo];
    const float* w = j.w;
    ET* out = reinterpret_cast<ET*>(j.out);
    if (j.kind >= 2) {
        const int taps = j.kh * j.kw, run = kPackT * taps, pitch = run + 1;
        const int b = (int)blockIdx.x - j.first_block, tiles_ci = j.cin / kPackT;
        const int co0 = (b / tiles_ci) * kPackT, ci0 = (b % tiles_ci) * kPackT;
        for (int e = threadIdx.x; e < kPackT * run; e += 256) {
            const int r = e / run, q = e - r * run;
            tile[r * pitch + q] = w[((long)(co0 + r) * j.cin + ci0) * taps + q];
        }
        __syncthreads();
        const int l = threadIdx.x & 31, g = threadIdx.x >> 5;
        if (j.kind == 2) {
            for (int p = g; p < kPackT * taps; p += 8) {
                const int r = p / taps, t = p - r * taps;
                stf(out + ((long)(co0 + r) * taps + t) * j.cin + ci0 + l, tile[r * pitch + l * taps + t]);
            }
        } else {
            for (int p = g; p < kPackT * taps; p += 8) {
                const int c = p / taps, t = p - c * taps;
                stf(out + ((long)(ci0 + c) * taps + t) * j.cout + co0 + l, tile[l * pitch + c * taps + (taps - 1 - t)]);
            }
        }
        return;
    }
    const long base = (long)((int)blockIdx.x - j.first_block) * 2048;
    const long total = j.kind == 0 ? (long)j.cout * j.kh * j.kw_pad * j.cin_pad : (long)j.cin * j.kh * j.kw * j.cout;
#pragma unroll
    for (int u = 0; u < 8; ++u) {
        const long i = base + u * 256 + threadIdx.x;
        if (i >= total) break;
        long t = i;
        float v = 0.f;
        if (j.kind == 0) {
            const int ci = (int)(t % j.cin_pad); t /= j.cin_pad;
            const int x = (int)(t % j.kw_pad); t /= j.kw_pad;
            const int yk = (int)(t % j.kh);
            const int co = (int)(t / j.kh);
            if (ci < j.cin && x < j.kw) v = w[(((long)co * j.cin + ci) * j.kh + yk) * j.kw + x];
        } else {
            const int co = (int)(t % j.cout); t /= j.cout;
            const int x = (int)(t % j.kw); t /= j.kw;
            const int y = (int)(t % j.kh);
            const int ci = (int)(t / j.kh);
            v = w[(((long)co * j.cin + ci) * j.kh + (j.kh - 1 - y)) * j.kw + (j.kw - 1 - x)];
        }
        stf(out + i, v);
    }
}

int plan_split(int M, int tiles, int target_override = 0) {
    static const int target_env = std::max(64, mvf_policy_int("wgrad_wgs", 1024));
    const int target = target_override > 0 ? target_override : target_env;
    int want = std::max(1, target / std::max(tiles, 1));
    int rows = std::max((M + want - 1) / want, 256);
    rows = (rows + 63) / 64 * 64;
    return rows;
}

struct WgTile { int bco, bk; };
WgTile pick_tile(int cout, int K) {
    if (cout <= 64) return {64, 128};
    if (K <= 64) return {128, 64};
    return {128, 128};
}

}

namespace mvf_internal {
int wgrad_slab_reduce_launch(const float* part, int nsplit, int cout, int k, float* dw_oihw, hipStream_t st) {
    return launch_wgrad_reduce(part, nsplit, cout, k, 1, 1, 1, k, dw_oihw, st);
}
}

extern "C" {

static bool wg_big_shape(const mvf_conv_desc_t* d) {
    static const int big_env = mvf_policy_int("wgrad_big", 1);
    const long K = (long)d->kh * d->kw * d->cin;
    if (big_env >= 2 && (d->kh != 1 || d->kw != 1)) return false;
    if (big_env >= 3 && d->cout < 512) return false;
    return big_env && d->dtype == MVF_BF16 && d->cout % 256 == 0 && K % 256 == 0 && d->cin % 8 == 0 && d->x_pix_stride % 4 == 0 &&
           (d->split_c == 0 || (d->split_c % 256 == 0 && d->cin % 256 == 0));
}
static int wg_big_rows(const mvf_conv_desc_t* d, int wgs_override = 0) {
    const int M = d->n * d->ho * d->wo, K = d->kh * d->kw * d->cin;
    static const int big_wgs = std::max(32, mvf_policy_int("wgrad_big_wgs", 128));
    return plan_split(M, (d->cout / 256) * (K / 256), wgs_override > 0 ? wgs_override : big_wgs);
}

static bool wg_direct3x3(const mvf_conv_desc_t* d) {
    return d->dtype == MVF_BF16 && d->cin == 64 && d->cout == 64 && d->kh == 3 && d->kw == 3 && d->stride == 1 && d->pad == 1 && d->split_c == 0 &&
           d->ho == d->h && d->wo == d->w && mvf_internal::wgrad3x3_c64_ok(d->n, d->h, d->w, d->x_pix_stride);
}

static bool wg_direct_stem(const mvf_conv_desc_t* d) {
    return d->dtype == MVF_BF16 && d->cin == 32 && d->cout == 64 && d->kh == 7 && d->kw == 1 && d->stride == 2 && d->pad == 0 && d->split_c == 0 &&
           d->x_pix_stride == 4 && mvf_internal::wgrad_stem_ok(d->n, d->h, d->w, d->ho, d->wo);
}

size_t mvf_conv2d_wgrad_workspace_bytes(const mvf_conv_desc_t* d) {
    if (!d || d->cout <= 0 || d->cin <= 0) return 0;
    const int M = d->n * d->ho * d->wo, K = d->kh * d->kw * d->cin;
    const WgTile t = pick_tile(d->cout, K);
    const int tiles = ((d->cout + t.bco - 1) / t.bco) * ((K + t.bk - 1) / t.bk);
    const int rows = plan_split(M, tiles);
    int nsplit = (M + rows - 1) / rows;
    if (wg_big_shape(d)) nsplit = std::max(nsplit, (M + wg_big_rows(d) - 1) / wg_big_rows(d));
    if (wg_direct3x3(d)) nsplit = std::max(nsplit, mvf_internal::wgrad3x3_c64_wgs(d->n, d->h));
    if (wg_direct_stem(d)) nsplit = std::max(nsplit, mvf_internal::wgrad_stem_wgs(d->n, d->ho));
    return align_up((size_t)nsplit * d->cout * K * sizeof(float), 256);
}

}
static int wgrad_impl(const mvf_conv_desc_t* d, const void* dz, const void* x, const void* x2, int kw_real, int cin_real,
                      int kw_packed, int cin_packed, float* dw_oihw, void* ws, size_t ws_bytes, void* stream, int wgs_target) {
    MVF_REQUIRE(d && dz && x && dw_oihw, MVF_EINVAL, "wgrad: NULL argument");
    MVF_REQUIRE(d->dtype == MVF_F32 || d->dtype == MVF_BF16, MVF_EINVAL, "wgrad: bad dtype");
    MVF_REQUIRE(d->cin % 4 == 0 && d->cout % 4 == 0 && d->x_pix_stride > 0, MVF_ESHAPE, "wgrad: cin/cout must be multiples of 4");
    MVF_REQUIRE(kw_packed * cin_packed == d->kw * d->cin && kw_real <= kw_packed && cin_real <= cin_packed, MVF_EINVAL, "wgrad: packed extents inconsistent");
    MVF_REQUIRE(ws && ws_bytes >= mvf_conv2d_wgrad_workspace_bytes(d), MVF_EWS, "wgrad: workspace too small");
    if (d->split_c) MVF_REQUIRE(x2 && d->kh == 1 && d->kw == 1 && d->split_c % 4 == 0, MVF_EINVAL, "wgrad: bad split_c");
    hipStream_t st0 = (hipStream_t)stream;
    if (wg_direct3x3(d) && kw_real == 3 && cin_real == 64 && kw_packed == 3 && cin_packed == 64 && ((uintptr_t)dz | (uintptr_t)x) % 16 == 0) {
        Wgrad3x3C64Args w = {dz, x, (float*)ws, d->n, d->h, d->w, d->x_pix_stride, mvf_internal::wgrad3x3_c64_wgs(d->n, d->h)};
        const int rc = mvf_internal::wgrad3x3_c64_launch(w, st0);
        if (rc != MVF_OK) return rc;
        return launch_wgrad_reduce((const float*)ws, w.nwg, 64, 64, 3, 3, 3, 64, dw_oihw, st0);
    }
    if (wg_direct_stem(d) && kw_real == 7 && cin_real == 3 && kw_packed == 8 && cin_packed == 4 && ((uintptr_t)dz | (uintptr_t)x) % 16 == 0) {
        WgradStemArgs w = {dz, x, (float*)ws, d->n, d->h, d->w, d->ho, d->wo, mvf_internal::wgrad_stem_wgs(d->n, d->ho)};
        const int rc = mvf_internal::wgrad_stem_launch(w, st0);
        if (rc != MVF_OK) return rc;
        return launch_wgrad_reduce((const float*)ws, w.nwg, 64, 3, 7, 7, 8, 4, dw_oihw, st0);
    }
    WgArgs a = {};
    a.dz = dz; a.x = x; a.x2 = x2; a.part = (float*)ws;
    a.N = d->n; a.H = d->h; a.W = d->w; a.Cin = d->cin; a.Cout = d->cout; a.KH = d->kh; a.KW = d->kw;
    a.stride = d->stride; a.pad = d->pad; a.Ho = d->ho; a.Wo = d->wo; a.xps = d->x_pix_stride;
    a.split_c = d->split_c; a.x2ps = d->x2_pix_stride;
    a.M = d->n * d->ho * d->wo; a.K = d->kh * d->kw * d->cin;
    WgTile t = pick_tile(d->cout, a.K);
    static const int gram_env = std::max(8, mvf_policy_int("gram_wgs", 32));
    const int gram_wgs = wgs_target > 0 ? wgs_target : (dz == x && !x2 && d->kh == 1 && d->kw == 1 && d->cin == d->cout) ? gram_env : 0;
    bool big = wg_big_shape(d) && wgs_target <= 0 && ((uintptr_t)dz | (uintptr_t)x | (uintptr_t)(x2 ? x2 : x)) % 16 == 0 &&
               (long)a.N * a.H * a.W * std::max(a.xps, a.x2ps) * 2 < 0x7ffffff0L;
    if (big) {
        const int rows = wg_big_rows(d, gram_wgs);
        big = rows >= 4 * 64 && ((long)rows + 6 * 64) * d->cout * 2 < 0x7ffffff0L;
        if (big) t = WgTile{256, 256};
    }
    a.tiles_k = (a.K + t.bk - 1) / t.bk;
    const int tiles = ((d->cout + t.bco - 1) / t.bco) * a.tiles_k;
    static const int x3_env = (mvf_policy_int("f32_x3", 1) != 0) && (mvf_policy_int("wgrad_x3", 1) != 0);
    bool x3 = d->dtype == MVF_F32 && x3_env && d->cin % 4 == 0 && d->cout % 4 == 0 && d->x_pix_stride % 4 == 0 && d->split_c % 4 == 0 &&
              (d->x2_pix_stride % 4 == 0 || !d->split_c) && ((uintptr_t)dz | (uintptr_t)x | (uintptr_t)(x2 ? x2 : x)) % 16 == 0;
    static const bool wgs_forced = mvf_policy_has("wgrad_wgs");
    const int bf16_wgs = (d->dtype == MVF_BF16 && !wgs_forced) ? 256 : 0;
    a.rows_per_split = big ? wg_big_rows(d, gram_wgs) : plan_split(a.M, tiles, gram_wgs ? gram_wgs : (x3 && !wgs_forced ? 768 : bf16_wgs));
    x3 = x3 && ((long)a.rows_per_split + 64) * d->cout * 4 < 0x7ffffff0L;
    if (d->dtype == MVF_F32 && !x3 && !wgs_forced && !gram_wgs) a.rows_per_split = plan_split(a.M, tiles);
    const int nsplit = (a.M + a.rows_per_split - 1) / a.rows_per_split;
    MVF_REQUIRE(ws_bytes >= (size_t)nsplit * d->cout * a.K * sizeof(float), MVF_EWS, "wgrad: workspace too small for %d slabs", nsplit);
    a.tiles = tiles;
    a.nsplit = nsplit;
    a.xcd_rr = nsplit % 8 == 0;
#ifdef MVF_WGRAD_ABLATE
    a.abl = mvf_policy_int("wgrad_abl", 0);
#endif
    wg_fd_make((unsigned)(a.Ho * a.Wo), a.fd_hw_mul, a.fd_hw_shr);
    wg_fd_make((unsigned)a.Wo, a.fd_w_mul, a.fd_w_shr);
    hipStream_t st = (hipStream_t)stream;
    static const int dma32_env = mvf_policy_int("wgrad_dma_f32", 1);
    const bool dma32 = d->dtype == MVF_F32 && dma32_env && d->cin % 4 == 0 && d->cout % 4 == 0 && d->x_pix_stride % 4 == 0 &&
                       (a.split_c == 0 || (a.split_c % t.bk == 0 && a.Cin % t.bk == 0)) &&
                       ((uintptr_t)dz | (uintptr_t)x | (uintptr_t)(x2 ? x2 : x)) % 16 == 0 &&
                       (long)a.N * a.H * a.W * std::max(a.xps, a.x2ps) * 4 < 0x7ffffff0L && ((long)a.rows_per_split + 64) * d->cout * 4 < 0x7ffffff0L;
    if (x3) {
        if (t.bco == 64) hipLaunchKernelGGL((wgrad_x3_kernel<1, 2>), dim3(nsplit * tiles), dim3(256), 0, st, a);
        else if (t.bk == 64) hipLaunchKernelGGL((wgrad_x3_kernel<2, 1>), dim3(nsplit * tiles), dim3(256), 0, st, a);
        else hipLaunchKernelGGL((wgrad_x3_kernel<2, 2>), dim3(nsplit * tiles), dim3(256), 0, st, a);
    } else if (dma32) {
        if (t.bco == 64) hipLaunchKernelGGL((wgrad_kernel<float, 1, 2, true>), dim3(nsplit * tiles), dim3(kThreads), 0, st, a);
        else if (t.bk == 64) hipLaunchKernelGGL((wgrad_kernel<float, 2, 1, true>), dim3(nsplit * tiles), dim3(kThreads), 0, st, a);
        else hipLaunchKernelGGL((wgrad_kernel<float, 2, 2, true>), dim3(nsplit * tiles), dim3(kThreads), 0, st, a);
    } else if (d->dtype == MVF_F32) {
        if (t.bco == 64) hipLaunchKernelGGL((wgrad_kernel<float, 1, 2>), dim3(nsplit * tiles), dim3(kThreads), 0, st, a);
        else if (t.bk == 64) hipLaunchKernelGGL((wgrad_kernel<float, 2, 1>), dim3(nsplit * tiles), dim3(kThreads), 0, st, a);
        else hipLaunchKernelGGL((wgrad_kernel<float, 2, 2>), dim3(nsplit * tiles), dim3(kThreads), 0, st, a);
    } else if (d->cin % 8 == 0 && d->cout % 8 == 0 && d->x_pix_stride % 4 == 0 && (d->split_c % 8) == 0 &&
               ((uintptr_t)dz | (uintptr_t)x | (uintptr_t)(x2 ? x2 : x)) % 16 == 0 &&
               ((long)a.rows_per_split + 6 * 64) * d->cout * 2 < 0x7ffffff0L) {
        int rc;
        if (big) rc = launch_wgrad_bf16_big(a, tiles, nsplit, st);
        else if (t.bco == 64) rc = launch_wgrad_bf16<1, 2>(a, tiles, nsplit, st);
        else if (t.bk == 64) rc = launch_wgrad_bf16<2, 1>(a, tiles, nsplit, st);
        else rc = launch_wgrad_bf16<2, 2>(a, tiles, nsplit, st);
        if (rc) return rc;
    } else {
        if (t.bco == 64) hipLaunchKernelGGL((wgrad_kernel<bf16_t, 1, 2>), dim3(nsplit * tiles), dim3(kThreads), 0, st, a);
        else if (t.bk == 64) hipLaunchKernelGGL((wgrad_kernel<bf16_t, 2, 1>), dim3(nsplit * tiles), dim3(kThreads), 0, st, a);
        else hipLaunchKernelGGL((wgrad_kernel<bf16_t, 2, 2>), dim3(nsplit * tiles), dim3(kThreads), 0, st, a);
    }
    MVF_LAUNCH_CHECK();
    const int kh_p = d->kh * d->kw * d->cin / (kw_packed * cin_packed);
    return launch_wgrad_reduce(a.part, nsplit, d->cout, cin_real, kh_p, kw_real, kw_packed, cin_packed, dw_oihw, st);
}
extern "C" {

int mvf_conv2d_nhwc_wgrad(const mvf_conv_desc_t* d, const void* dz, const void* x, const void* x2, int kw_real, int cin_real,
                          int kw_packed, int cin_packed, float* dw_oihw, void* ws, size_t ws_bytes, void* stream) {
    return wgrad_impl(d, dz, x, x2, kw_real, cin_real, kw_packed, cin_packed, dw_oihw, ws, ws_bytes, stream, 0);
}

int mvf_conv2d_nhwc_wgrad_wgs(const mvf_conv_desc_t* d, const void* dz, const void* x, const void* x2, int kw_real, int cin_real,
                              int kw_packed, int cin_packed, float* dw_oihw, void* ws, size_t ws_bytes, int wgs, void* stream) {
    MVF_REQUIRE(wgs >= 8 && wgs <= 4096, MVF_EINVAL, "wgrad_wgs: wgs=%d outside 8 .. 4096", wgs);
    return wgrad_impl(d, dz, x, x2, kw_real, cin_real, kw_packed, cin_packed, dw_oihw, ws, ws_bytes, stream, wgs);
}

int mvf_pack_conv_weights_batched(const mvf_pack_job_t* jobs_dev, int njobs, int total_blocks, int dtype, void* stream) {
    MVF_REQUIRE(jobs_dev && njobs > 0 && total_blocks > 0 && (dtype == MVF_F32 || dtype == MVF_BF16), MVF_EINVAL, "pack_conv_weights_batched: bad argument");
    if (dtype == MVF_F32)
        hipLaunchKernelGGL(pack_batched_kernel<float>, dim3(total_blocks), dim3(256), 0, (hipStream_t)stream, jobs_dev, njobs);
// ... 20 lines not shown
```

### mvfnet_amd/csrc/wgrad_stem.hip

```cpp
#include <algorithm>
#include <stdlib.h>

#include "common.h"

namespace {

typedef float f32x16 __attribute__((ext_vector_type(16)));
typedef short bf16x8_t __attribute__((ext_vector_type(8)));

struct KArgs {
    const char* dz;
    const char* x;
    float* part;
    int N, H, W, Ho, Wo;
    int bands_per_frame, bands;
    int rowb;
    int xbytes, dpix;
    int ksr;
    unsigned fd_bpf_mul, fd_bpf_shr, fd_ksr_mul, fd_ksr_shr;
};

__device__ __forceinline__ int fdiv(int n, unsigned mul, unsigned shr) { return (int)((__umulhi((unsigned)n, mul) + (unsigned)n) >> shr); }
__device__ __forceinline__ int swzf(int pixel) { return ((pixel >> 1) & 1) << 2; }

template <int kR>
__global__ __launch_bounds__(256, 2) void wgrad_stem_kernel(KArgs a) {
    extern __shared__ __attribute__((aligned(16))) char smem[];
    char* Xs = smem;
    char* Ds = smem + (a.xbytes + 1023) / 1024 * 1024;
    const int tid = threadIdx.x, lane = tid & 63;
    const int wave = __builtin_amdgcn_readfirstlane(tid >> 6);
    const int wm = wave & 1, kg = wave >> 1;
    constexpr unsigned kOOB = 0x80000000u;
    const i32x4 gs_x = rsrc_words(a.x, (unsigned)((long)a.N * a.H * a.rowb));
    const i32x4 gs_d = rsrc_words(a.dz, (unsigned)((long)a.N * a.Ho * a.Wo * 128));
    const unsigned lds_x = (unsigned)__builtin_amdgcn_readfirstlane((int)(unsigned)(size_t)(__attribute__((address_space(3))) char*)Xs);
    const unsigned lds_d = (unsigned)__builtin_amdgcn_readfirstlane((int)(unsigned)(size_t)(__attribute__((address_space(3))) char*)Ds);
    const int nx = (a.xbytes + 1023) >> 10, nd = a.dpix >> 3;
    const int lp = lane >> 3, lu = lane & 7;

    const int tg = lane >> 4, ti = lane & 15;
    const int trow = (ti >> 2) + 8 * (tg >> 1);
    const int tunit = 2 * (tg & 1) + ((ti & 3) >> 1), thalf = ti & 1;
    const int offA = trow * 128 + (((wm * 4 + tunit) ^ swzf(trow)) << 4) + thalf * 8;
    const int offB = 16 * trow + 32 * (tg & 1) + 8 * (ti & 3);
    typedef short v4s __attribute__((ext_vector_type(4)));
    typedef __attribute__((address_space(3))) v4s* lds_v4s;
    auto gather = [&](const char* lo_p, const char* hi_p) {
        const v4s lo = __builtin_amdgcn_ds_read_tr16_b64_v4i16((lds_v4s)(lo_p));
        const v4s hi = __builtin_amdgcn_ds_read_tr16_b64_v4i16((lds_v4s)(hi_p));
        bf16x8_t v;
        v[0] = lo[0]; v[1] = lo[1]; v[2] = lo[2]; v[3] = lo[3];
        v[4] = hi[0]; v[5] = hi[1]; v[6] = hi[2]; v[7] = hi[3];
        return v;
    };

    f32x16 acc[4];
#pragma unroll
    for (int t = 0; t < 4; ++t)
#pragma unroll
        for (int r = 0; r < 16; ++r) acc[t][r] = 0.f;

    const int nks = a.dpix >> 4;
    for (int b = blockIdx.x; b < a.bands; b += gridDim.x) {
        const int img = fdiv(b, a.fd_bpf_mul, a.fd_bpf_shr);
        const int oh0 = (b - img * a.bands_per_frame) * kR;
        __syncthreads();
        {
            const long xbase = ((long)img * a.H + 2 * oh0) * a.rowb;
            for (int i = wave; i < nx; i += 4) {
                const int o = i * 1024 + lane * 16;
                glds16(gs_x, lds_x + (unsigned)(i * 1024), o < a.xbytes ? (unsigned)(xbase + o) : kOOB);
            }
            const long dbase = ((long)img * a.Ho + oh0) * a.Wo * 128;
            for (int i = wave; i < nd; i += 4) {
                const int p = i * 8 + lp;
                glds16(gs_d, lds_d + (unsigned)(i * 1024), (unsigned)(dbase + p * 128 + ((lu ^ swzf(p)) << 4)));
            }
        }
        asm volatile("s_waitcnt vmcnt(0)" ::: "memory");
        __syncthreads();
        for (int ks = 0; ks < nks; ++ks) {
            const int r = fdiv(ks, a.fd_ksr_mul, a.fd_ksr_shr), ow0 = (ks - r * a.ksr) * 16;
            const bf16x8_t fa = gather(Ds + ks * 2048 + offA, Ds + ks * 2048 + offA + 4 * 128);
            const char* xb = Xs + (2 * r + 4 * kg) * a.rowb + ow0 * 16 + offB;
            bf16x8_t fb[4];
#pragma unroll
            for (int t = 0; t < 4; ++t) {
                if (t < 3 || kg == 0) fb[t] = gather(xb + t * a.rowb, xb + t * a.rowb + 64);
            }
#pragma unroll
            for (int t = 0; t < 4; ++t) {
                if (t < 3 || kg == 0) acc[t] = __builtin_amdgcn_mfma_f32_32x32x16_bf16(fa, fb[t], acc[t], 0, 0, 0);
            }
        }
    }
    const int lr = lane >> 5, lc = lane & 31;
    float* out = a.part + (long)blockIdx.x * 64 * 224;
#pragma unroll
    for (int t = 0; t < 4; ++t) {
        if (t < 3 || kg == 0) {
            const int col = (4 * kg + t) * 32 + lc;
#pragma unroll
            for (int r = 0; r < 16; ++r) {
                const int row = wm * 32 + (r & 3) + 8 * (r >> 2) + 4 * lr;
                out[row * 224 + col] = acc[t][r];
            }
        }
    }
}

inline void fd_make(unsigned d, unsigned& mul, unsigned& shr) {
    unsigned l = 0;
    while ((1ull << l) < d) ++l;
    mul = (unsigned)((((1ull << l) - d) << 32) / d + 1);
    shr = l;
}

static int band_rows() {
    static const int r = mvf_policy_int("wgrad_stem_r", 2);
    return r == 1 ? 1 : 2;
}

}

namespace mvf_internal {

bool wgrad_stem_ok(int n, int h, int w, int ho, int wo) {
    static const bool on = (mvf_policy_int("wgrad_stem_direct", 1) != 0);
    return on && n > 0 && wo >= 16 && wo % 16 == 0 && ho % 2 == 0 && (w * 8) % 16 == 0 && 2 * (ho - 1) + 6 < h && 2 * (wo - 1) + 7 < w &&
           (long)n * h * w * 8 < 0x7ffffff0L && (long)n * ho * wo * 128 < 0x7ffffff0L &&
           (2 * 2 + 5) * w * 8 + 1024 + 2 * wo * 128 <= 72 * 1024;
}

int wgrad_stem_wgs(int n, int ho) {
    static const int env = std::max(1, mvf_policy_int("wgrad_stem_wgs", 768));
    return (int)std::min<long>(env, (long)n * (ho / band_rows()));
}

int wgrad_stem_launch(const WgradStemArgs& w, hipStream_t st) {
    KArgs a = {};
    a.dz = (const char*)w.dz; a.x = (const char*)w.x; a.part = w.part;
    a.N = w.N; a.H = w.H; a.W = w.W; a.Ho = w.Ho; a.Wo = w.Wo;
    const int kR = band_rows();
    a.bands_per_frame = w.Ho / kR;
    a.bands = w.N * a.bands_per_frame;
    a.rowb = w.W * 8;
    a.xbytes = (2 * kR + 5) * a.rowb;
    a.dpix = kR * w.Wo;
    a.ksr = w.Wo / 16;
    fd_make((unsigned)a.bands_per_frame, a.fd_bpf_mul, a.fd_bpf_shr);
    fd_make((unsigned)a.ksr, a.fd_ksr_mul, a.fd_ksr_shr);
    const int lds = (a.xbytes + 1023) / 1024 * 1024 + a.dpix * 128;
    static bool attr = false;
    if (!attr) {
        MVF_HIP_OK(hipFuncSetAttribute((const void*)wgrad_stem_kernel<1>, hipFuncAttributeMaxDynamicSharedMemorySize, 72 * 1024));
        MVF_HIP_OK(hipFuncSetAttribute((const void*)wgrad_stem_kernel<2>, hipFuncAttributeMaxDynamicSharedMemorySize, 72 * 1024));
        attr = true;
    }
    if (kR == 1) hipLaunchKernelGGL(wgrad_stem_kernel<1>, dim3(w.nwg), dim3(256), lds, st, a);
    else hipLaunchKernelGGL(wgrad_stem_kernel<2>, dim3(w.nwg), dim3(256), lds, st, a);
    MVF_LAUNCH_CHECK();
    return MVF_OK;
}

}
```

### mvfnet_amd/train_engine.py

```python
import ctypes as C
import os

import torch

from . import _lib
from ._lib import ConvDesc, MvfDesc, check, lib

F32 = _lib.MVF_F32

_ConvDescT, _MvfDescT = ConvDesc, MvfDesc
_DESC_CACHE = {}


def ConvDesc(*a):
    d = _DESC_CACHE.get(a)
    if d is None:
        d = _DESC_CACHE[a] = _ConvDescT(*a)
    return d


def MvfDesc(*a):
    k = ("mvf",) + a
    d = _DESC_CACHE.get(k)
    if d is None:
# ... 195 lines not shown
        self.dw = eng.grad_of(conv.weight)
        self.cout, self.cin, self.kh, self.kw = conv.weight.shape
        self.stride, self.pad = conv.stride[0], conv.padding[0]
        self.stem = stem
        dev = conv.weight.device
        td = eng.tdtype
        if stem:
            self.wp = torch.empty(self.cout, self.kh, 8, 4, device=dev, dtype=td)
            self.wd = None
        else:
            same = self.kh == 1 and self.kw == 1 and td == torch.float32
            self.wp = self.w if same else torch.empty(self.cout, self.kh, self.kw, self.cin, device=dev, dtype=td)
            self.wd = torch.empty(self.cin, self.kh, self.kw, self.cout, device=dev, dtype=td)

    def pack(self, need_dgrad=True):
        if self.stem:
            check(lib.mvf_pack_conv_weight(_p(self.w), self.cout, self.cin, self.kh, self.kw, 8, 4, None, _p(self.wp), self.eng.dt, _st()), "pack")
            return
        if self.wp is not self.w:
            check(lib.mvf_pack_conv_weight(_p(self.w), self.cout, self.cin, self.kh, self.kw, self.kw, self.cin, None, _p(self.wp), self.eng.dt, _st()), "pack")
        if need_dgrad:
            self.pack_dgrad()

    def pack_jobs(self):
        if self.stem:
            return (self.w, self.wp, self.cout, self.cin, self.kh, self.kw, 8, 4, 0), None
        fwd = None if self.wp is self.w else (self.w, self.wp, self.cout, self.cin, self.kh, self.kw, self.kw, self.cin, 0)
        return fwd, (self.w, self.wd, self.cout, self.cin, self.kh, self.kw, self.kw, self.cin, 1)

    def pack_dgrad(self):
        if not self.stem:
            check(lib.mvf_pack_conv_weight_dgrad(_p(self.w), self.cout, self.cin, self.kh, self.kw, _p(self.wd), self.eng.dt, _st()), "pack_dgrad")

    def desc(self, n, h, w, ho, wo, x_pitch, split_c=0):
        if self.stem:
            return ConvDesc(n, h, w, 32, self.cout, self.kh, 1, 2, 0, ho, wo, 4, self.eng.dt, 0, 0, 0, 0)
        return ConvDesc(n, h, w, self.cin, self.cout, self.kh, self.kw, self.stride, self.pad, ho, wo, x_pitch, self.eng.dt, 0, split_c, split_c, 0)

    def out_hw(self, h, w):
        return (h + 2 * self.pad - self.kh) // self.stride + 1, (w + 2 * self.pad - self.kw) // self.stride + 1

    def forward(self, x, n, h, w, x_pitch=None, x2=None, split_c=0, ho=None, wo=None, bn=None, store=True):
        if ho is None:
            ho, wo = self.out_hw(h, w)
        d = self.desc(n, h, w, ho, wo, x_pitch or self.cin, split_c)
        z = self.eng.buf((id(self), "z"), (n * ho * wo, self.cout)) if store else None
        ws = _conv_ws(x.device)
        if bn is None or not self.eng.fuse_stats or bn.frozen:
            self.launch_fwd(d, x, x2, z, ws, None, None)
            if bn is not None:
                bn.stats(z, n * ho * wo, self.eng)
            return z, ho, wo
        rows = _stats_rows(d)
        part = self.eng.buf((id(self), "part"), (rows, self.cout, 2), torch.float32)
        self.launch_fwd(d, x, x2, z, ws, part, bn.mod.running_mean)
        bn.finalize(part, rows, n * ho * wo)
        return z, ho, wo

    def forward_apply(self, x, n, h, w, bn, residual, rbn=None):
        ho, wo = self.out_hw(h, w)
        d = self.desc(n, h, w, ho, wo, self.cin)
        m = n * ho * wo
        out = self.eng.buf((id(bn), "apply"), (m, self.cout))
        bits = self.eng.buf((id(bn), "bits"), (m, self.cout // 4), torch.uint8)
        self.launch_fwd_apply(d, x, bn, residual, rbn, out, bits, _conv_ws(x.device))
        return out, bits

    def bwd_recompute(self, a_in, g, bits, n, h, w, bn):
        ho, wo = self.out_hw(h, w)
        d = self.desc(n, h, w, ho, wo, self.cin)
        m = n * ho * wo
        ws = _conv_ws(a_in.device)
        rows = _stats_rows(d)
        part = self.eng.buf((id(self), "bwpart"), (rows, self.cout, 2), torch.float32)
        self.launch_bwd_sums(d, a_in, g, bits, bn, part, ws)
        check(lib.mvf_bn_bwd_finalize(_p(part), rows, self.cout, _p(bn.dgamma), _p(bn.dbeta), _st()), "mvf_bn_bwd_finalize")
        dz = self.eng.buf((id(bn), "dz"), (m, self.cout))
        self.launch_bwd_apply(d, a_in, g, bits, bn, dz, ws)
        return dz

    def bwd_fused_ok(self, m):
        return (self.eng.tdtype == torch.bfloat16 and self.kh == 1 and self.kw == 1 and self.stride == 1 and not self.stem and
                lib.mvf_conv1x1_bwd_fused_splits(m, self.cout, self.cin) > 0)

    def bwd_fused(self, a_in, g, bits, n, h, w, bn, bn_in=None, z_in=None, a_pitch=None, sums_done=False):
        pitch = a_pitch or self.cin
        d = self.desc(n, h, w, h, w, pitch)
        m = n * h * w
        ws = _conv_ws(a_in.device)
        rows = _stats_rows(d)
        ns = lib.mvf_conv1x1_bwd_fused_splits(m, self.cout, self.cin)
        if not sums_done and self.eng.pair_ds_sums & 2:
            part = self.eng.buf((id(self), "bwpart_pair"), (self.cout, 2 * ns, 2), torch.float32)
            self.launch_bwd_sums1(m, a_in, pitch, g, bits, bn, part, ns)
            check(lib.mvf_bn_bwd_finalize(_p(part), 2 * ns, self.cout, _p(bn.dgamma), _p(bn.dbeta), _st()), "mvf_bn_bwd_finalize")
        elif not sums_done:
            part = self.eng.buf((id(self), "bwpart"), (rows, self.cout, 2), torch.float32)
            self.launch_bwd_sums(d, a_in, g, bits, bn, part, ws)
            check(lib.mvf_bn_bwd_finalize(_p(part), rows, self.cout, _p(bn.dgamma), _p(bn.dbeta), _st()), "mvf_bn_bwd_finalize")
        dx = self.eng.buf((id(self), "dx"), (m, self.cin))
        spart = self.eng.buf((id(self), "bnsums_fused"), (self.cin, 2 * ns, 2), torch.float32) if bn_in is not None else None
        slabs = self.eng.buf((id(self), "wslab"), (ns * self.cout * self.cin,), torch.float32)
        self.launch_bwd_fused(m, a_in, g, bits, bn, bn_in, z_in, dx, spart, ns, slabs, pitch)
        if bn_in is not None:
            check(lib.mvf_bn_bwd_finalize(_p(spart), 2 * ns, self.cin, _p(bn_in.dgamma), _p(bn_in.dbeta), _st()), "bn bwd finalize")
        self.slab_reduce(slabs, ns, self.eng)
        return dx

    def launch_bwd_sums1(self, m, a_in, a_pitch, g, bits, bn, part, ns):
        check(lib.mvf_conv1x1_bnbwd_sums_pair(_p(a_in), a_pitch, _p(self.wp), None, 0, None, _p(g), self.cout, _p(bits), m, self.cout, self.cin, _p(bn.mean),
                                              _p(bn.invstd), None, None, _p(part), None, 2 * ns, self.eng.dt, _st()), "bn backward sums (one branch)")

    def launch_bwd_fused(self, m, a_in, g, bits, bn, bn_in, z_in, dx, spart, ns, slabs, a_pitch=None):
        i = bn_in
        check(lib.mvf_conv1x1_bwd_fused(_p(a_in), a_pitch or self.cin, _p(self.wp), _p(g), self.cout, _p(bits), m, self.cout, self.cin, _p(bn.gamma), _p(bn.mean),
                                        _p(bn.invstd), _p(bn.dgamma), _p(bn.dbeta), _p(z_in) if i is not None else None, _p(i.mean) if i else None,
                                        _p(i.invstd) if i else None, _p(i.scale) if i else None, _p(i.shift) if i else None,
                                        _p(dx), _p(spart), 2 * ns, _p(slabs), slabs.numel() * 4, self.eng.dt, _st()), "conv1x1 backward fused")

    def launch_bwd_sums(self, d, a_in, g, bits, bn, part, ws):
        check(lib.mvf_conv2d_nhwc_fwd_bnbwd_sums(C.byref(d), _p(a_in), None, _p(self.wp), _p(g), _p(bits), _p(bn.mean), _p(bn.invstd), _p(part),
                                                 _p(ws), ws.numel(), _st()), "conv + bn backward sums")

    def launch_bwd_apply(self, d, a_in, g, bits, bn, dz, ws):
        check(lib.mvf_conv2d_nhwc_fwd_bnbwd_apply(C.byref(d), _p(a_in), None, _p(self.wp), _p(g), _p(bits), _p(bn.gamma), _p(bn.mean), _p(bn.invstd),
                                                  _p(bn.dgamma), _p(bn.dbeta), _p(dz), _p(ws), ws.numel(), _st()), "conv + bn backward apply")

    def launch_fwd_apply(self, d, x, bn, residual, rbn, out, bits, ws):
        check(lib.mvf_conv2d_nhwc_fwd_bnapply(C.byref(d), _p(x), None, _p(self.wp), _p(bn.scale), _p(bn.shift), _p(residual),
                                              _p(rbn.scale if rbn else None), _p(rbn.shift if rbn else None), _p(out), _p(bits),
                                              _p(ws), ws.numel(), _st()), "conv fwd + bn apply")

    def launch_fwd(self, d, x, x2, z, ws, part, shift):
        if part is None:
            check(lib.mvf_conv2d_nhwc_fwd_ws(C.byref(d), _p(x), _p(x2), _p(self.wp), None, None, _p(z), _p(ws), ws.numel(), _st()), "conv fwd")
        else:
            check(lib.mvf_conv2d_nhwc_fwd_stats(C.byref(d), _p(x), _p(x2), _p(self.wp), _p(z), _p(part), _p(shift), _p(ws), ws.numel(), _st()),
                  "conv fwd+stats")

    def wgrad(self, dz, x, n, h, w, ho, wo, eng, x_pitch=None, x2=None, split_c=0, on_main=False):
        d = self.desc(n, h, w, ho, wo, x_pitch or self.cin, split_c)
        kwr, cinr, kwp, cinp = (self.kw, self.cin, 8, 4) if self.stem else (self.kw, self.cin, self.kw, self.cin)
        nbytes = lib.mvf_conv2d_wgrad_workspace_bytes(C.byref(d))
        side = None if on_main else eng.side_stream()
        if side is None:
            ws = eng.workspace(nbytes)
            check(lib.mvf_conv2d_nhwc_wgrad(C.byref(d), _p(dz), _p(x), _p(x2), kwr, cinr, kwp, cinp, _p(self.dw), _p(ws), ws.numel(), _st()), "conv wgrad")
            return
        ws = eng.workspace(nbytes, side=True)

        def launch():
            check(lib.mvf_conv2d_nhwc_wgrad(C.byref(d), _p(dz), _p(x), _p(x2), kwr, cinr, kwp, cinp, _p(self.dw), _p(ws), ws.numel(), _st()), "conv wgrad")
        eng.on_side(launch)

    def fuses_wgrad(self, eng, m, c, mask_mode, nbn=1):
        return (eng.tdtype == torch.bfloat16 and self.kh == 1 and self.kw == 1 and self.stride == 1 and not self.stem and c == self.cout and
                lib.mvf_bn_bwd_wgrad_splits(m, c, self.cin, nbn, mask_mode) > 0)

    def slab_reduce(self, slabs, ns, eng):
        def launch():
            check(lib.mvf_wgrad_slab_reduce(_p(slabs), ns, self.cout, self.cin, _p(self.dw), _st()), "wgrad slab reduce")
        if eng.side_stream() is None:
            launch()
        else:
            eng.on_side(launch)

    def dgrad_bnsums(self, dz, n, ho, wo, h, w, bn, z):
        d = ConvDesc(n, ho, wo, self.cout, self.cin, self.kh, self.kw, 1, self.kh - 1 - self.pad, h, w, self.cout, self.eng.dt, 0, 0, 0,
                     self.stride if self.stride > 1 else 0, 0)
        dx = self.eng.buf((id(self), "dx"), (n * h * w, self.cin))
        ws = _conv_ws(dz.device)
        rows = _stats_rows(d)
        part = self.eng.buf((id(self), "bnsums"), (rows, self.cin, 2), torch.float32)
        self.launch_dgrad_bnsums(d, dz, dx, z, bn, part, ws)
        check(lib.mvf_bn_bwd_finalize(_p(part), rows, self.cin, _p(bn.dgamma), _p(bn.dbeta), _st()), "bn bwd finalize")
        return dx

    def launch_dgrad_bnsums(self, d, dz, dx, z, bn, part, ws):
        check(lib.mvf_conv2d_nhwc_dgrad_bnsums(C.byref(d), _p(dz), _p(self.wd), _p(dx), _p(z), _p(bn.mean), _p(bn.invstd), _p(bn.scale), _p(bn.shift),
                                               _p(part), _p(ws), ws.numel(), _st()), "conv dgrad+bn sums")

    def dgrad(self, dz, n, ho, wo, h, w, residual=None, res_c0=0, res_bits=None, out_gate=None, gsum=None):
        d = ConvDesc(n, ho, wo, self.cout, self.cin, self.kh, self.kw, 1, self.kh - 1 - self.pad, h, w, self.cout, self.eng.dt, 0, 0, 0,
                     self.stride if self.stride > 1 else 0, res_c0)
        dx = self.eng.buf((id(self), "dx"), (n * h * w, self.cin))
        ws = _conv_ws(dz.device)
        if out_gate is not None and gsum is not None:
            bn = gsum["bn"]
            rows = _stats_rows(d)
            part = self.eng.buf((id(bn), "gsum_conv"), (self.cin, rows, 2), torch.float32)
            check(lib.mvf_conv2d_nhwc_fwd_resmask_gate_colsums(C.byref(d), _p(dz), None, _p(self.wd), _p(residual), _p(res_bits), _p(out_gate), _p(dx), _p(part), _p(ws),
                                                               ws.numel(), _st()), "conv dgrad (gated output + column sums)")
            bn._s1 = [None, 0, res_c0, part, rows]
        elif out_gate is not None:
            check(lib.mvf_conv2d_nhwc_fwd_resmask_gate(C.byref(d), _p(dz), None, _p(self.wd), None, _p(residual), _p(res_bits), _p(out_gate), _p(dx), _p(ws),
                                                       ws.numel(), _st()), "conv dgrad (gated output)")
        else:
            check(lib.mvf_conv2d_nhwc_fwd_resmask(C.byref(d), _p(dz), None, _p(self.wd), None, _p(residual), _p(res_bits), _p(dx), _p(ws), ws.numel(),
                                                  _st()), "conv dgrad")
        return dx

    def dzfree_ok(self, m):
        return (self.eng.tdtype == torch.bfloat16 and self.kh == 1 and self.kw == 1 and self.stride == 1 and not self.stem and
                self.cout % 256 == 0 and self.cin % 64 == 0 and self.cout <= 4096 and m * (self.cout + self.cin) * 2 < 0x7ffffff0)

    def dzfree_dgrad(self, gm, a_in, bn, n, h, w, bn_in, z_in, frozen_zero=None):
        eng = self.eng
        c, k, m = self.cout, self.cin, n * h * w
        bd = eng.buf((id(self), "dzfree_w"), (k, c + k))
        bias = eng.buf((id(self), "dzfree_b"), (k,), torch.float32)
        sg, sb = (frozen_zero, frozen_zero) if frozen_zero is not None else (bn.dgamma, bn.dbeta)
        check(lib.mvf_bn_bwd_dzfree_prep(_p(self.wd), c, k, _p(bn.gamma), _p(bn.mean), _p(bn.invstd), _p(sg), _p(sb), m, _p(bd), _p(bias), eng.dt, _st()),
              "bn backward without dz: operands")
        d = ConvDesc(n, h, w, c + k, k, 1, 1, 1, 0, h, w, k, eng.dt, 0, c, c, 0, 0, c)
        dx = eng.buf((id(self), "dx"), (m, k))
        ws = _conv_ws(gm.device)
        rows = _stats_rows(d)
        part = eng.buf((id(self), "bnsums"), (rows, k, 2), torch.float32)
        self.launch_dzfree_dgrad(d, a_in, gm, bd, bias, dx, z_in, bn_in, part, ws)
        check(lib.mvf_bn_bwd_finalize(_p(part), rows, k, _p(bn_in.dgamma), _p(bn_in.dbeta), _st()), "bn bwd finalize")
        return dx

    def launch_dzfree_dgrad(self, d, a_in, gm, bd, bias, dx, z_in, bn_in, part, ws):
        check(lib.mvf_conv2d_nhwc_dgrad_bnsums_split(C.byref(d), _p(a_in), _p(gm), _p(bd), _p(bias), _p(dx), _p(z_in), _p(bn_in.mean), _p(bn_in.invstd),
                                                     _p(bn_in.scale), _p(bn_in.shift), _p(part), _p(ws), ws.numel(), _st()), "conv dgrad on [gm | a] + bn sums")

    def dzfree_q_sums(self, gm, a_in, bn, n, h, w, eng):
        c, k = self.cout, self.cin
        d = self.desc(n, h, w, h, w, k, 0)
        ws = eng.workspace(lib.mvf_conv2d_wgrad_workspace_bytes(C.byref(d)))
        self.launch_q(d, gm, a_in, ws, eng.dzfree_q_wgs)
        lo, rows_lo, c_split, hi, rows_hi = bn._s1
        assert c_split == 0 or lo is not None, "the MVF slice's column sums are missing"
        check(lib.mvf_bn_bwd_dzfree_sums(_p(self.dw), _p(self.wp), c, k, _p(bn.mean), _p(bn.invstd), _p(lo), rows_lo, c_split, _p(hi), rows_hi, _p(bn.dgamma),
                                         _p(bn.dbeta), eng.dt, _st()), "bn backward sums from the weight-gradient GEMM")
        bn._s1 = None

    def launch_q(self, d, gm, a_in, ws, wgs):
        check(lib.mvf_conv2d_nhwc_wgrad_wgs(C.byref(d), _p(gm), _p(a_in), None, self.kw, self.cin, self.kw, self.cin, _p(self.dw), _p(ws), ws.numel(), wgs, _st()),
              "conv wgrad (launch stream)")

    def gram_ok(self):
        return (self.eng.tdtype == torch.bfloat16 and self.kh == 1 and self.kw == 1 and self.stride == 1 and not self.stem and
                self.cin % 32 == 0 and self.cout % 32 == 0)

    def gram_stats(self, a_in, bn, n, h, w, eng, means_done=False):
        c, k, m = self.cout, self.cin, n * h * w
        gram = eng.buf((id(self), "gram"), (k, k), torch.float32)
        amean = eng.buf((id(self), "amean"), (4, k), torch.float32)
        d = ConvDesc(n, h, w, k, k, 1, 1, 1, 0, h, w, k, eng.dt, 0, 0, 0, 0)
        ws = eng.workspace(max(lib.mvf_conv2d_wgrad_workspace_bytes(C.byref(d)), lib.mvf_bn_workspace_bytes(m, k), (eng.gram_stats_wgs + 8) * k * k * 4))
        if k not in eng._ones:
            eng._ones[k] = (torch.ones(k, device=a_in.device), torch.zeros(k, device=a_in.device))
        one, zero = eng._ones[k]
        self.launch_gram(d, a_in, gram, ws, eng.gram_stats_wgs)
        if not means_done:
            check(lib.mvf_bn_train_stats(_p(a_in), m, k, _p(one), _p(zero), C.c_float(1e-5), C.c_float(0.1), None, None, _p(amean[0]), _p(amean[1]),
                                         _p(amean[2]), _p(amean[3]), _p(ws), ws.numel(), eng.dt, _st()), "column means")
        check(lib.mvf_bn_train_stats_gram(_p(gram), _p(amean[0]), _p(self.wp), m, c, k, _p(bn.gamma), _p(bn.beta), C.c_float(bn.eps), C.c_float(bn.momentum),
                                          _p(bn.mod.running_mean), _p(bn.mod.running_var), _p(bn.mean), _p(bn.invstd), _p(bn.scale), _p(bn.shift), eng.dt,
                                          _st()), "bn statistics from the Gram matrix")
        bn._count()

    def launch_gram(self, d, a_in, gram, ws, wgs):
        k = self.cin
        check(lib.mvf_conv2d_nhwc_wgrad_wgs(C.byref(d), _p(a_in), _p(a_in), None, 1, k, 1, k, _p(gram), _p(ws), ws.numel(), wgs, _st()), "gram (launch stream)")

    def dzfree_wgrad(self, gm, a_in, bn, n, h, w, eng, frozen_zero=None, q_done=False, gram_done=False):
        c, k, m = self.cout, self.cin, n * h * w
        if not q_done:
            self.wgrad(gm, a_in, n, h, w, h, w, eng)
        gram = eng.buf((id(self), "gram"), (k, k), torch.float32)
        amean = eng.buf((id(self), "amean"), (4, k), torch.float32)
        d = ConvDesc(n, h, w, k, k, 1, 1, 1, 0, h, w, k, eng.dt, 0, 0, 0, 0)
        nbytes = max(lib.mvf_conv2d_wgrad_workspace_bytes(C.byref(d)), lib.mvf_bn_workspace_bytes(m, k))
        if k not in eng._ones:
            eng._ones[k] = (torch.ones(k, device=gm.device), torch.zeros(k, device=gm.device))
        one, zero = eng._ones[k]
        sg, sb = (frozen_zero, frozen_zero) if frozen_zero is not None else (bn.dgamma, bn.dbeta)
        side = eng.side_stream()
        ws = eng.workspace(nbytes, side=side is not None)

        def launch():
            if not gram_done:
                check(lib.mvf_conv2d_nhwc_wgrad(C.byref(d), _p(a_in), _p(a_in), None, 1, k, 1, k, _p(gram), _p(ws), ws.numel(), _st()), "gram")
                check(lib.mvf_bn_train_stats(_p(a_in), m, k, _p(one), _p(zero), C.c_float(1e-5), C.c_float(0.1), None, None, _p(amean[0]), _p(amean[1]),
                                             _p(amean[2]), _p(amean[3]), _p(ws), ws.numel(), eng.dt, _st()), "column means")
            check(lib.mvf_bn_bwd_dzfree_wgrad(_p(self.dw), _p(self.wp), _p(gram), _p(amean[0]), _p(bn.gamma), _p(bn.mean), _p(bn.invstd), _p(sg), _p(sb),
                                              m, c, k, eng.dt, _st()), "weight gradient without dz: correction")
        if side is None:
            launch()
        else:
            eng.on_side(launch)


class _TMvf(object):
    def __init__(self, mvf, eng):
        self.eng = eng
        self.cs, self.T = mvf.num_shift_channel, mvf.n_segment
        self.mode = _lib.MODE_BITS[mvf.mode]
        self.share, self.use_hs = mvf.share, mvf.use_hs
        cs = self.cs
        self.wt = mvf.shift_conv.weight
        self.wh = mvf.shift_conv.weight if mvf.share else (mvf.h_conv.weight if self.mode & 2 else None)
        self.ww = mvf.shift_conv.weight if mvf.share else (mvf.w_conv.weight if self.mode & 4 else None)
        self.dwt = eng.grad_of(mvf.shift_conv.weight)
# ... 287 lines not shown
        self.c2.wgrad(dz2, s["a1"], nt, h, w, ho, wo, eng)
        del dz2
        w1_done = (eng.fuse_bnwg & 4) and self.mvf is None and self.c1.fuses_wgrad(eng, m, self.c1.cout, 2)
        if w1_done:
            dz1 = self.b1.backward_wgrad(da1, self.c1.cout, s["z1"], m, eng, 2, None, self.c1, s["x"], c, sums_done=fuse1)
        else:
            dz1 = self.b1.backward(da1, self.c1.cout, s["z1"], m, eng, 2, sums_done=fuse1)
        del da1
        resid, rbits = (g, None) if g_gated else (g, bits)
        if resid_ds is not None:
            resid, rbits = resid_ds, None
        elif self.cd is not None:
            if dzd is None:
                dzd = self.bd.backward(g, self.cd.cout, s["zd"], m2, eng, 4, ymask=bits)
            resid, rbits = self.cd.dgrad(dzd, nt, ho, wo, h, w), None
            if not wd_done:
                self.cd.wgrad(dzd, s["x"], nt, h, w, ho, wo, eng, x_pitch=c)
            del dzd
        if self.mvf is None:
            dx = self.c1.dgrad(dz1, nt, h, w, h, w, residual=resid, res_bits=rbits, out_gate=out_gate, gsum=gsum)
            self.gated_out, self.sums_out = out_gate is not None, (gsum["sums"] if gsum is not None else False)
            if not w1_done:
                self.c1.wgrad(dz1, s["x"], nt, h, w, h, w, eng, x_pitch=c)
        else:
            fuse = self.mvf.cs % 4 == 0
            og = out_gate if fuse else None
            gs = gsum if fuse else None
            dxp = self.c1.dgrad(dz1, nt, h, w, h, w, residual=resid if fuse else None, res_c0=self.mvf.cs, res_bits=rbits if fuse else None, out_gate=og, gsum=gs)
            self.gated_out, self.sums_out = og is not None, (gs["sums"] if gs is not None else False)
            if self.split_ok:
                self.c1.wgrad(dz1, s["x"], nt, h, w, h, w, eng, x_pitch=c, x2=s["o"], split_c=self.mvf.cs)
            else:
                self.c1.wgrad(dz1, s["xin"], nt, h, w, h, w, eng, x_pitch=c)
            self.mvf.backward(dxp, s["x"], s["y"], nt, h, w, c, eng, addend=resid if fuse else None, addend_bits=rbits if fuse else None, out_gate=og, gsum=gs)
            if not fuse:
                if rbits is not None:
                    resid = resid * (s["out"] > 0).to(resid.dtype)
                dx = eng.add(dxp, resid, key=id(self))
            else:
                dx = dxp
        if eng.keep_io:
            self.io = dict(x=s["x"], out=s["out"], g=g, dx=dx, h=h, w=w, c=c, ho=ho, wo=wo, g_gated=g_gated, dx_gated=self.gated_out)
        self.saved = None
        eng.flush_side(late=True)
        return dx


class _ParamStore(object):

    def _init_store(self, model, dtype=torch.float32, rehome=True):
        if dtype not in (torch.float32, torch.bfloat16):
            raise TypeError("training dtype must be float32 or bfloat16 (activation storage; weights/statistics/gradients stay fp32)")
        self.tdtype = dtype
        self.dt = _lib.MVF_F32 if dtype == torch.float32 else _lib.MVF_BF16
        dev = next(model.parameters()).device
        if dev.type != "cuda":
            raise RuntimeError("the HIP training engine needs the model on an MI355X device; no CPU fallback")
        self.model, self.device = model, dev
        self._side_pending = []
        self._side_keep = []
        params = [p for p in model.parameters()]
        n = sum(p.numel() for p in params)
        pad = lambda k: (k + 3) // 4 * 4
        total = sum(pad(p.numel()) for p in params)
        self.rehomed = bool(rehome)
        self.flat_params = torch.zeros(total, device=dev) if rehome else None
        self.flat_grads = torch.zeros(total, device=dev)
        self.flat_mom = torch.zeros(total, device=dev) if rehome else None
        self._grad_view = {}
        off = 0
        with torch.no_grad():
            for p in params:
                k = p.numel()
                if rehome:
                    v = self.flat_params[off:off + k].view(p.shape)
                    v.copy_(p.data.float())
                    p.data = v
                elif p.dtype != torch.float32 or not p.is_contiguous() or p.device != dev:
                    raise TypeError("stand-alone block: parameters must be contiguous float32 tensors on %s" % dev)
                gv = self.flat_grads[off:off + k].view(p.shape)
                self._grad_view[id(p)] = gv
                off += pad(k)
        self.n_params = n
        if rehome:
            for m_ in model.modules():
                if hasattr(m_, "invalidate_engine"):
                    m_.invalidate_engine()
        self._ws = None
        self.norm_out = torch.zeros(2, device=dev)
        self.steps = 0
        self._ones = {}
        self._bufs = {}
        self._caps = {}
        self._last_shape = {}

    def grad_of(self, p):
        return self._grad_view[id(p)]

    def buf(self, key, shape, dtype=None):
        dt = dtype or self.tdtype
        shape = tuple(shape)
        k = (key, shape, dt)
        step = getattr(self, "forward_count", None)
        if step is not None:
            last = self._last_shape.get((key, dt))
            if last is not None and last[0] == step and last[1] != shape:
                raise RuntimeError("engine buffer %r requested with shapes %s and %s inside one step: they would share storage" % (key, last[1], shape))
            self._last_shape[(key, dt)] = (step, shape)
        t = self._bufs.get(k)
        if t is None:
            n = 1
            for v in shape:
                n *= int(v)
            ck = (key, dt)
            flat = self._caps.get(ck)
            if flat is None or flat.numel() < n:
                if flat is not None:
                    self._side_keep.append(flat)
                    self._storage_epoch += 1
                    for kk in [kk for kk in self._bufs if kk[0] == key and kk[2] == dt]:
                        del self._bufs[kk]
                flat = torch.empty(max(n, 1), device=self.device, dtype=dt)
                self._caps[ck] = flat
            t = flat[:n].view(shape)
            self._bufs[k] = t
        return t

    def workspace(self, nbytes, side=False):
        key = "_ws_side" if side else "_ws"
        ws = getattr(self, key, None)
        if ws is None or ws.numel() < nbytes:
            if ws is not None:
                self._storage_epoch += 1
            ws = torch.empty(max(int(nbytes), 1 << 20), dtype=torch.uint8, device=self.device)
            setattr(self, key, ws)
        return ws

    _storage_epoch = 0

    overlap_wgrad = True
    keep_io = False
    fuse_stats = True
    overlap_downsample = _policy("side_downsample", 1) != 0
    z3_free = _policy("z3_free", 1)
    fuse_bn3_apply = _policy("fuse_bn3_apply", 1)
    fuse_bn_bwd_sums = _policy("fuse_bn_bwd", 1) != 0
    fuse_bn_bwd_strided = _policy("fuse_bn_bwd_strided", 1) != 0
    pair_bn_bwd = _policy("pair_bn_bwd", 1) != 0
    fuse_bnwg = _policy("fuse_bnwg", 7)
    pair_ds_sums = _policy("pair_ds_sums", 3)
    z3_free_ds = _policy("z3_free_ds", 1)
    fuse_c3_bwd = _policy("fuse_c3_bwd", 1)
    fuse_mvf_stats = _policy("fuse_mvf_stats", 1) != 0
    dzfree = _policy("dzfree", 2)
    gate_producer = _policy("gate_producer", 1) != 0
    dzfree_q = _policy("dzfree_q", 1)
    dzfree_q_wgs = _policy("dzfree_q_wgs", 256)
    dzfree_q_maxk = _policy("dzfree_q_maxk", 256)
    dzfree_q_mink = _policy("dzfree_q_mink", 0)
    gram_stats = _policy("gram_stats", 1) != 0
    gram_stats_wgs = _policy("gram_stats_wgs", 256)
    gram_colsums = _policy("gram_colsums", 1) != 0

    def side_stream(self):
        if not self.overlap_wgrad:
            return None
        if getattr(self, "_side", None) is None:
            from .streams import concurrent_stream
            self._side = concurrent_stream(self.main_stream())
        return self._side

    def main_stream(self):
        ms = getattr(self, "_main", None)
        return ms if ms is not None else torch.cuda.current_stream()

    _rec = None

    def _wait(self, dst, src):
        if self._rec is not None:
            self._rec.wait(dst, src)
        else:
            dst.wait_stream(src)

    def _mark(self, stream):
        if self._rec is not None:
            return self._rec.mark(stream)
        ev = torch.cuda.Event()
        ev.record(stream)
        return ev

    def _wait_mark(self, stream, ev):
        if self._rec is not None:
            self._rec.wait_mark(stream, ev)
        else:
            stream.wait_event(ev)

    def on_side(self, launch):
        self._side_keep.append(launch)
        self._side_pending.append(launch)


    def flush_side(self, late=False):
        pend = getattr(self, "_side_pending", None)
        marked = getattr(self, "_side_marked", None)
        if late and pend:
            ev = self._mark(self.main_stream())
            if marked is None:
                marked = self._side_marked = []
            marked.append((ev, list(pend)))
            del pend[:]
            return
        self.issue_marked()
        if pend:
            self._wait(self._side, self.main_stream())
            with _on_stream(self._side):
                for launch in pend:
                    launch()
            del pend[:]

    def issue_marked(self):
        marked = getattr(self, "_side_marked", None)
        if marked:
            for ev, launches in marked:
                self._wait_mark(self._side, ev)
                with _on_stream(self._side):
                    for launch in launches:
                        launch()
            del marked[:]

    def join_side(self):
        self.flush_side()
        if getattr(self, "_side", None) is not None:
            self._wait(self.main_stream(), self._side)
        del self._side_keep[:]

    def add(self, a, b, key=None):
        m, c = a.shape
        if c not in self._ones:
            self._ones[c] = (torch.ones(c, device=a.device), torch.zeros(c, device=a.device))
        one, zero = self._ones[c]
        out = self.buf((key or id(a), "add"), a.shape, a.dtype) if key is not None else torch.empty_like(a)
        check(lib.mvf_bn_apply(_p(a), m, c, _p(one), _p(zero), _p(b), None, None, 0, _p(out), self.dt, _st()), "add")
        return out

    lr, momentum, weight_decay, max_norm = 0.015, 0.9, 1e-4, 40.0

    def trainable_offset(self):
        params = list(self.model.parameters())
        flags = [p.requires_grad for p in params]
        k = flags.index(True) if True in flags else len(flags)
        self._scattered_frozen = not all(flags[k:])
        return self._grad_view[id(params[k])].storage_offset() if k < len(params) else self.flat_grads.numel()

    nesterov = True
    param_options = None

    def set_param_options(self, options):
        self.param_options = {id(p): (float(a), float(b)) for p, (a, b) in options.items()} if options else None
        self._seg_tables = {}

    def _segments(self, off):
        tabs = self.__dict__.setdefault("_seg_tables", {})
        key = (off, tuple(p.requires_grad for p in self.model.parameters()))
        if key not in tabs:
            segs, last = [], None
            for p in self.model.parameters():
                first = self._grad_view[id(p)].storage_offset()
                if first + p.numel() <= off:
                    continue
                mult = (self.param_options or {}).get(id(p), (1.0, 1.0)) if p.requires_grad else (-1.0, 0.0)
                if mult != last:
                    segs.append(_lib.SgdSegment(max(first - off, 0) if segs else 0, mult[0], mult[1]))
                    last = mult
            arr = (_lib.SgdSegment * len(segs))(*segs)
            tabs[key] = (torch.frombuffer(bytearray(bytes(arr)), dtype=torch.uint8).to(self.device), len(segs))
        return tabs[key]

    def apply_sgd(self, lr=None, world=1):
        if not self.rehomed:
            raise RuntimeError("apply_sgd: this store does not own its parameters (stand-alone Bottleneck.forward); use the model's train engine or a torch optimizer")
        off = self.trainable_offset()
        n = self.flat_params.numel() - off
        if n <= 0:
            return None
        ws = self.workspace(lib.mvf_sgd_workspace_bytes(n))
        args = (_p(self.flat_params[off:]), _p(self.flat_grads[off:]), _p(self.flat_mom[off:]), n, C.c_float(1.0 / world),
                C.c_float(self.max_norm or 0.0), C.c_float(self.lr if lr is None else lr), C.c_float(self.momentum),
                C.c_float(self.weight_decay), int(self.steps == 0))
        if self.nesterov and not self.param_options and not self._scattered_frozen:
            check(lib.mvf_sgd_nesterov_step(*(args + (_p(self.norm_out), _p(ws), ws.numel(), _st()))), "sgd step")
        else:
            tab, nseg = self._segments(off)
            check(lib.mvf_sgd_step_segments(*(args + (int(self.nesterov), _p(tab), nseg, _p(self.norm_out), _p(ws), ws.numel(), _st()))), "sgd step")
        self.steps += 1
        return self.norm_out

    def optimizer_state_dict(self):
        from .checkpoint import sgd_state_dict
        params = list(self.model.parameters())
        off = self.trainable_offset()
        bufs = []
        for p in params:
            v = self._grad_view[id(p)]
            first = v.storage_offset()
            stepped = self.steps > 0 and first >= off and p.requires_grad
            bufs.append(self.flat_mom[first:first + p.numel()].view(p.shape).detach().cpu().clone() if stepped else None)
# ... 103 lines not shown
        self._nbt_mods, self._nbt_inc = bns, {}
        self.input_pipeline, self.input_window = None, None
        self._pack_tables = None

    def _pack_all(self, kind):
        if self._pack_tables is None:
            self._pack_tables = {}
            convs = [self.stem] + [cv for blk in self.blocks for cv in blk.convs()]
            for k in (0, 1):
                jobs, first = [], 0
                for cv in convs:
                    j = cv.pack_jobs()[k]
                    if j is None:
                        continue
                    w, out, cout, cin, kh, kw, kwp, cinp, kd = j
                    total = cout * kh * kwp * cinp if kd == 0 else cin * kh * kw * cout
                    tiled = cout % 32 == 0 and cin % 32 == 0 and kh * kw <= 9 and kwp == kw and cinp == cin
                    jobs.append(_lib.PackJob(w.data_ptr(), out.data_ptr(), cout, cin, kh, kw, kwp, cinp, kd + 2 if tiled else kd, first))
                    first += (cout // 32) * (cin // 32) if tiled else (total + 2047) // 2048
                if not jobs:
                    self._pack_tables[k] = None
                    continue
                arr = (_lib.PackJob * len(jobs))(*jobs)
                host = torch.frombuffer(bytearray(bytes(arr)), dtype=torch.uint8)
                self._pack_tables[k] = (host.to(self.device), len(jobs), first)
        t = self._pack_tables[kind]
        if t is not None:
            check(lib.mvf_pack_conv_weights_batched(_p(t[0]), t[1], t[2], self.dt, _st()), "pack_conv_weights_batched")

    def forward(self, imgs, labels, stages=None, _prepared=None):
        if not imgs.is_cuda or imgs.dtype not in (torch.float32, torch.uint8):
            raise RuntimeError("TrainEngine.forward: float32 (or uint8 frames) GPU input required")
        self._main = torch.cuda.current_stream()
        self.forward_count += 1
        with _on_stream(self._main, main=True):
            return self._forward(imgs, labels, stages, _prepared)

    def _step_tensors(self, imgs, labels):
        lab = labels.reshape(-1).to(device=imgs.device, dtype=torch.int64).contiguous()
        mask = None
        if self.dropout > 0.0:
            nt, cc = imgs.shape[0] * imgs.shape[1], self.fc_w.shape[1]
            cache = self.__dict__.setdefault("_drop_ones", {})
            ones = cache.get((nt, cc))
            if ones is None:
                ones = cache[(nt, cc)] = torch.ones(nt, cc, device=imgs.device, dtype=torch.float32)
            mask = torch.nn.functional.dropout(ones, self.dropout, True)
        loss = torch.empty(1, device=imgs.device, dtype=torch.float32)
        return lab, mask, loss

    def set_options(self, lr=None, momentum=None, weight_decay=None, max_norm=None, dtype=None):
        if dtype is not None and dtype != self.tdtype:
            raise RuntimeError("the model's train engine was built with dtype %s; it cannot be switched to %s" % (self.tdtype, dtype))
        for k, v in (("lr", lr), ("momentum", momentum), ("weight_decay", weight_decay), ("max_norm", max_norm)):
            if v is not None:
                setattr(self, k, v)

    def _forward(self, imgs, labels, stages=None, prepared=None):
        b, t = imgs.shape[0], imgs.shape[1]
        lab, mask, loss = prepared if prepared is not None else self._step_tensors(imgs, labels)
        u8 = imgs.dtype == torch.uint8
        if u8:
            if self.input_pipeline is None:
                raise RuntimeError("uint8 frames need engine.input_pipeline = preprocess.FramePipeline(...)")
            x = None
            nt = b * t
            h, w = self.input_pipeline.crop_hw
        else:
            x = imgs.reshape((-1, 3) + tuple(imgs.shape[3:])).contiguous()
            nt, _, h, w = x.shape
        self._pack_all(0)
        side = self.side_stream()
        if side is not None:
            self._wait(side, self.main_stream())
        with _on_stream(side if side is not None else self.main_stream()):
            self._pack_all(1)
        self._packs_on_side = side is not None
        hp, wp = h + 6, (w + 6 + 2 + 1) // 2 * 2
        xp = self.buf("xp", (nt, hp, wp, 4))
        if u8:
            self.input_pipeline.to_stem(imgs, self.input_window, 3, wp, self.tdtype, out=xp)
        else:
            check(lib.mvf_stem_prep(_p(x), nt, 3, h, w, 3, wp, _p(xp), self.dt, _st()), "stem_prep")
        ho, wo = (h + 6 - 7) // 2 + 1, (w + 6 - 7) // 2 + 1
        z0, _, _ = self.stem.forward(xp, nt, hp, wp, ho=ho, wo=wo, bn=self.stem_bn)
        h2, w2 = (ho - 1) // 2 + 1, (wo - 1) // 2 + 1
        p0 = self.buf("p0", (nt * h2 * w2, 64))
        amax = self.buf("amax", (nt * h2 * w2, 64), torch.uint8)
        check(lib.mvf_maxpool_bn_relu_fwd(_p(z0), nt, ho, wo, 64, _p(self.stem_bn.scale), _p(self.stem_bn.shift), _p(p0), _p(amax), self.dt, _st()), "maxpool fwd")
        self.saved = dict(xp=xp, z0=z0, amax=amax, nt=nt, hp=hp, wp=wp, ho=ho, wo=wo, t=t, b=b)
        if stages is not None:
            stages["maxpool"] = p0.view(nt, h2, w2, 64)
        xcur, hc, wc, cc = p0, h2, w2, 64
        ends, k = [], 0
        for name in self.model.backbone.res_layers:
            k += len(getattr(self.model.backbone, name))
            ends.append(k)
        for i, blk in enumerate(self.blocks):
            xcur, hc, wc, cc = blk.forward(xcur, nt, hc, wc, cc, self)
            if stages is not None and (i + 1) in ends:
                stages["layer%d" % (ends.index(i + 1) + 1)] = xcur.view(nt, hc, wc, cc)
        dev = imgs.device
        f32 = torch.float32
        pooled = self.buf("pooled", (nt, cc), f32)
        scores = self.buf("scores", (b, self.num_classes), f32)
        dscores = self.buf("dscores", (b, self.num_classes), f32)
        loss_part = self.buf("loss_part", (b,), f32)
        check(lib.mvf_head_train_fwd(_p(xcur), b, t, hc * wc, cc, _p(self.fc_w), _p(self.fc_b), self.num_classes, _p(lab), _p(mask), _p(pooled),
                                     _p(scores), _p(dscores), _p(loss_part), _p(loss), self.dt, _st()), "head fwd")
        self.saved.update(pooled=pooled, dscores=dscores, mask=mask, hw=hc * wc, c=cc, feat_shape=xcur.shape, scores=scores)
        if self._nbt_touched:
            self._count_batches()
        return loss

    def _count_batches(self):
        key = tuple(m_.training for m_ in self._nbt_mods)
        if all(key):
            self._nbt_flat += 1
        else:
            if key not in self._nbt_inc:
                self._nbt_inc[key] = torch.tensor([int(k) for k in key] or [0], dtype=torch.int64, device=self.device)
            self._nbt_flat += self._nbt_inc[key]
        self._nbt_touched = False

    def backward(self, exchange=False):
        self._main = torch.cuda.current_stream()
        self._exchange = bool(exchange)
        with _on_stream(self._main, main=True):
            self._backward()

    def _backward(self):
        s = self.saved
        if getattr(self, "_packs_on_side", False):
            self._wait(self.main_stream(), self._side)
        nt, b, t = s["nt"], s["b"], s["t"]
        dpool = self.buf("dpool", (b, s["c"]), torch.float32)
        g = self.buf("gfeat", tuple(s["feat_shape"]))
        check(lib.mvf_head_train_bwd(_p(s["dscores"]), _p(s["pooled"]), _p(self.fc_w), _p(s["mask"]), b, t, s["hw"], s["c"], self.num_classes,
                                     _p(self.dfc_w), _p(self.dfc_b), _p(dpool), _p(g), self.dt, _st()), "head bwd")
        gated = sums = False
        for i in range(len(self.blocks) - 1, -1, -1):
            req = self.blocks[i - 1].wants_gated_gradient(self) if i > 0 else None
            g = self.blocks[i].backward(g, nt, self, g_gated=gated, gate=req, sums_done=sums)
            gated, sums = self.blocks[i].gated_out, self.blocks[i].sums_out
            if i == self._tail_block:
                self._launch_tail_allreduce()
        ho, wo = s["ho"], s["wo"]
        bn = self.stem_bn
        rows = lib.mvf_maxpool_bwd_sums_rows(nt, ho)
        part = self.buf("stem_bnsums", (64, rows, 2), torch.float32)
        check(lib.mvf_maxpool_bn_relu_bwd_sums(_p(s["amax"]), _p(g), nt, ho, wo, 64, None, _p(s["z0"]), _p(bn.mean), _p(bn.invstd),
                                               _p(bn.scale), _p(bn.shift), _p(part), self.dt, _st()), "maxpool bwd + bn sums")
        check(lib.mvf_bn_bwd_finalize(_p(part), rows, 64, _p(bn.dgamma), _p(bn.dbeta), _st()), "bn bwd finalize")
        dz0 = self.buf((id(bn), "dz"), s["z0"].shape, s["z0"].dtype)
        sg, sb = (bn._zero, bn._zero) if bn.frozen else (bn.dgamma, bn.dbeta)
        check(lib.mvf_maxpool_bn_relu_bwd_apply(_p(s["amax"]), _p(g), nt, ho, wo, 64, _p(s["z0"]), _p(bn.gamma), _p(bn.mean), _p(bn.invstd), _p(bn.scale),
                                                _p(bn.shift), _p(sg), _p(sb), _p(dz0), self.dt, _st()), "maxpool bwd + bn apply")
        self.flush_side()
        self.stem.wgrad(dz0, s["xp"], nt, s["hp"], s["wp"], ho, wo, self, on_main=True)
        self.join_side()
        if self.keep_io:
            self.io = dict(p0=self.buf("p0", (g.shape[0], 64)), g_p0=g, gfeat=self.buf("gfeat", tuple(s["feat_shape"])), nt=nt, b=b, t=t)
        self.saved = None

    exchange_enabled = True

    def _ddp_active(self):
        import torch.distributed as dist
        return self.exchange_enabled and dist.is_available() and dist.is_initialized() and (dist.get_world_size() > 1 or self.force_allreduce)

    overlap_allreduce = _policy("ddp_overlap", 1) != 0

    def _launch_tail_allreduce(self):
        self._tail_launched = False
        if not (getattr(self, "_exchange", False) and self.overlap_allreduce and self._tail_off and self._ddp_active() and self.overlap_wgrad):
            return
        import torch.distributed as dist
        side = self.side_stream()
        self.flush_side()
        if getattr(self, "_comm", None) is None:
            from .streams import concurrent_stream
            self._comm = concurrent_stream(self.main_stream(), avoid=[side])

        def exchange():
            comm = self._comm
            comm.wait_stream(side)
            comm.wait_stream(self.main_stream())
            with torch.cuda.stream(comm):
                dist.all_reduce(self.flat_grads[self._tail_off:])
            self._tail_launched = True
        if self._rec is not None:
            self._rec.py_op(exchange)
        else:
            exchange()

    def allreduce_grads(self):
        import torch.distributed as dist
        if not self._ddp_active():
            return 1
        if self._tail_launched:
            torch.cuda.current_stream().wait_stream(self._comm)
            dist.all_reduce(self.flat_grads[:self._tail_off])
            self._tail_launched = False
        else:
            dist.all_reduce(self.flat_grads)
        return dist.get_world_size()

    force_allreduce = False

    def step(self, lr=None):
        with _on_stream(torch.cuda.current_stream(), main=True):
            return self._step(lr)

    def _step(self, lr=None):
        world = self.allreduce_grads()
        if self.apply_sgd(lr, world) is None:
            return self.norm_out
        for m_ in (self.model.backbone, self.model.cls_head):
            if hasattr(m_, "invalidate_engine"):
                m_.invalidate_engine()
        return self.norm_out

    use_plan = _policy("plan", 1) != 0
    plan_warmup = 2

    def _plan_key(self, imgs, labels):
        if not (self.use_plan and imgs.dtype == torch.float32 and imgs.is_contiguous() and not self.keep_io and self.input_pipeline is None):
            return None
        if not all(m_.training for m_ in self._nbt_mods):
            return None
        sw = self.__dict__.get("_switch_names")
        if sw is None:
            sw = self._switch_names = sorted(k for c_ in type(self).__mro__ for k, v in vars(c_).items()
                                             if not k.startswith("_") and isinstance(v, (bool, int, float, str)) and k not in ("lr", "momentum", "weight_decay", "max_norm"))
        return (tuple(imgs.shape), tuple(labels.shape), labels.dtype, str(imgs.device), torch.cuda.current_stream().cuda_stream, self._ddp_active(),
                self.dropout > 0.0, tuple(p.requires_grad for p in self.model.parameters()), tuple(getattr(self, k) for k in sw))

    def _record_step(self, imgs, labels, prepared):
        from . import launch_plan
        import sys
        mod = sys.modules[__name__]
        rec = launch_plan.Recorder()
        allocs0 = torch.cuda.memory_stats(imgs.device).get("allocation.all.allocated", 0)
        real_lib, self._rec = mod.lib, rec
        mod.lib = launch_plan.RecordingLib(rec)
        try:
            loss = self.forward(imgs, labels, _prepared=prepared)
            self.backward(exchange=True)
        finally:
            mod.lib, self._rec = real_lib, None
        if torch.cuda.memory_stats(imgs.device).get("allocation.all.allocated", 0) != allocs0:
            rec.unsupported = "the step allocates device memory"
        if rec.unsupported:
            return loss, None
        lab, mask, _ = prepared
        plan = launch_plan.Plan(rec, dict(imgs=imgs.data_ptr(), labels=lab.data_ptr(), mask=mask.data_ptr() if mask is not None else 0, loss=loss.data_ptr()))
        plan.storage_epoch = self._storage_epoch
        return loss, plan

    def train_step(self, imgs, labels, lr=None):
        key = self._plan_key(imgs, labels) if imgs.is_cuda else None
        if key is None:
            loss = self.forward(imgs, labels)
            self.backward(exchange=True)
            self.step(lr)
            return loss
        st = self.__dict__.setdefault("_plans", {}).setdefault(key, dict(eager=0, tries=0, cand=None, plan=None))
        prepared = self._step_tensors(imgs, labels)
        plan = st["plan"]
        if plan is not None and plan.storage_epoch != self._storage_epoch:
            plan = st["plan"] = st["cand"] = None
            st["tries"] = 0
        if plan is not None:
            lab, mask, loss = prepared
            self._main = torch.cuda.current_stream()
            self.forward_count += 1
            self._exchange = True
            self._count_batches()
            plan.run(dict(imgs=imgs.data_ptr(), labels=lab.data_ptr(), mask=mask.data_ptr() if mask is not None else 0, loss=loss.data_ptr()))
        elif st["eager"] < self.plan_warmup or st["tries"] >= 4:
            st["eager"] += 1
            loss = self.forward(imgs, labels, _prepared=prepared)
            self.backward(exchange=True)
        else:
            st["tries"] += 1
            loss, cand = self._record_step(imgs, labels, prepared)
            if cand is not None and st["cand"] is not None and cand.signature == st["cand"].signature and cand.storage_epoch == self._storage_epoch:
                st["plan"], st["cand"] = cand, None
            else:
                st["cand"] = cand
        self.step(lr)
        return loss
```

Baseline: 1819 clips/s.

## Fuse maxpool/BN backward apply into stem weight-gradient kernel; unroll sqsum loops

Adds a pooled variant of the stem wgrad kernel that recomputes the maxpool+BN+ReLU backward dz directly into LDS from argmax, gradient and z0. This avoids writing and re-reading the full-resolution dz0 tensor. The path sits behind a policy flag, stem_wgrad_fused, that defaults to 0, so by default the old separate apply + wgrad calls still run. The gradient squared-sum reduction kernels also get an 8-way unrolled loop to raise memory-level parallelism, and that part is always active.

```diff
diff --git a/include/mvfnet_hip.h b/include/mvfnet_hip.h
--- a/include/mvfnet_hip.h
+++ b/include/mvfnet_hip.h
@@ -210,6 +210,10 @@
                           void* stream);
 int mvf_conv2d_nhwc_wgrad_wgs(const mvf_conv_desc_t* d, const void* dz, const void* x, const void* x2, int kw_real,
                               int cin_real, int kw_packed, int cin_packed, float* dw_oihw, void* ws, size_t ws_bytes, int wgs, void* stream);
+size_t mvf_conv_stem_wgrad_pool_bn_workspace_bytes(int n, int hp, int wp, int ho, int wo, int dtype);
+int mvf_conv_stem_wgrad_pool_bn(const unsigned char* argmax, const void* g, const void* z, const float* gamma, const float* mean, const float* invstd,
+                                const float* scale, const float* shift, const float* dgamma, const float* dbeta, const void* xp, int n, int hp, int wp,
+                                int ho, int wo, float* dw_oihw, void* ws, size_t ws_bytes, int dtype, void* stream);
 typedef struct {
     const float* w;
     void* out;
diff --git a/mvfnet_amd/_lib.py b/mvfnet_amd/_lib.py
--- a/mvfnet_amd/_lib.py
+++ b/mvfnet_amd/_lib.py
@@ -203,6 +203,10 @@
     lib.mvf_conv2d_nhwc_wgrad.argtypes = [cp, vp, vp, vp, i32, i32, i32, i32, fp, vp, sz, vp]
     lib.mvf_conv2d_nhwc_wgrad_wgs.restype = i32
     lib.mvf_conv2d_nhwc_wgrad_wgs.argtypes = [cp, vp, vp, vp, i32, i32, i32, i32, fp, vp, sz, i32, vp]
+    lib.mvf_conv_stem_wgrad_pool_bn_workspace_bytes.restype = sz
+    lib.mvf_conv_stem_wgrad_pool_bn_workspace_bytes.argtypes = [i32, i32, i32, i32, i32, i32]
+    lib.mvf_conv_stem_wgrad_pool_bn.restype = i32
+    lib.mvf_conv_stem_wgrad_pool_bn.argtypes = [vp, vp, vp, fp, fp, fp, fp, fp, fp, fp, vp, i32, i32, i32, i32, i32, fp, vp, sz, i32, vp]
     lib.mvf_pack_conv_weight_dgrad.restype = i32
     lib.mvf_pack_conv_weight_dgrad.argtypes = [fp, i32, i32, i32, i32, vp, i32, vp]
     lib.mvf_nhwc_stencil.restype = i32
diff --git a/mvfnet_amd/csrc/common.h b/mvfnet_amd/csrc/common.h
--- a/mvfnet_amd/csrc/common.h
+++ b/mvfnet_amd/csrc/common.h
@@ -151,6 +151,9 @@
     const void* x;
     float* part;
     int N, H, W, Ho, Wo, nwg;
+    const unsigned char* amax;
+    const void *g, *z;
+    const float *gamma, *mean, *invstd, *scale, *shift, *dgamma, *dbeta;
 };
 namespace mvf_internal {
 struct BnBwdWgradArgs {
@@ -196,6 +199,7 @@
 int bnbwd_wgrad_plan(long m, int c, int k, int nbn, int mask_mode, int* rows_per_split, int* ctiles, int* ktiles);
 int bnbwd_wgrad_launch(const BnBwdWgradArgs& a, int nbn, int mask_mode, hipStream_t st);
 int wgrad_slab_reduce_launch(const float* part, int nsplit, int cout, int k, float* dw_oihw, hipStream_t st);
+int wgrad_stem_reduce_launch(const float* part, int nsplit, float* dw_oihw, hipStream_t st);
 bool wgrad3x3_c64_ok(int n, int h, int w, int xps);
 int wgrad3x3_c64_wgs(int n, int h);
 int wgrad3x3_c64_launch(const Wgrad3x3C64Args& a, hipStream_t st);
diff --git a/mvfnet_amd/csrc/pool_bn_bwd_blk.h b/mvfnet_amd/csrc/pool_bn_bwd_blk.h
--- /dev/null
+++ b/mvfnet_amd/csrc/pool_bn_bwd_blk.h
@@ -0,0 +1,114 @@
+#pragma once
+#include "common.h"
+
+namespace mvf_poolblk {
+
+template <typename ET>
+constexpr int vc_of() { return 16 / (int)sizeof(ET); }
+
+template <typename ET, int VC>
+__device__ __forceinline__ void ldv(const ET* p, float (&f)[VC]) {
+    const uint4 u = *reinterpret_cast<const uint4*>(p);
+    if constexpr (sizeof(ET) == 4) {
+        f[0] = __uint_as_float(u.x); f[1] = __uint_as_float(u.y); f[2] = __uint_as_float(u.z); f[3] = __uint_as_float(u.w);
+    } else {
+        f[0] = __uint_as_float(u.x << 16); f[1] = __uint_as_float(u.x & 0xffff0000u); f[2] = __uint_as_float(u.y << 16); f[3] = __uint_as_float(u.y & 0xffff0000u);
+        f[4] = __uint_as_float(u.z << 16); f[5] = __uint_as_float(u.z & 0xffff0000u); f[6] = __uint_as_float(u.w << 16); f[7] = __uint_as_float(u.w & 0xffff0000u);
+    }
+}
+template <typename ET, int VC>
+__device__ __forceinline__ uint4 packv(const float (&f)[VC]) {
+    if constexpr (sizeof(ET) == 4) {
+        return make_uint4(__float_as_uint(f[0]), __float_as_uint(f[1]), __float_as_uint(f[2]), __float_as_uint(f[3]));
+    } else {
+        return make_uint4(pack_bf16x2(f[0], f[1]), pack_bf16x2(f[2], f[3]), pack_bf16x2(f[4], f[5]), pack_bf16x2(f[6], f[7]));
+    }
+}
+
+template <int VC>
+struct Consts {
+    float scv[VC], shv[VC], muv[VC], k1[VC], k2[VC], k3[VC];
+};
+template <int VC, int MODE>
+__device__ __forceinline__ void load_consts(Consts<VC>& k, int cq, const float* gamma, const float* mean, const float* invstd, const float* scale,
+                                            const float* shift, const float* dgamma, const float* dbeta, float inv_m) {
+#pragma unroll
+    for (int j = 0; j < VC; ++j) {
+        const int ch = cq * VC + j;
+        k.scv[j] = scale[ch]; k.shv[j] = shift[ch]; k.muv[j] = mean[ch];
+        if constexpr (MODE == 0) { k.k1[j] = invstd[ch]; k.k2[j] = 0.f; k.k3[j] = 0.f; }
+        else { k.k1[j] = gamma[ch] * invstd[ch]; k.k2[j] = dbeta[ch] * inv_m; k.k3[j] = invstd[ch] * dgamma[ch] * inv_m; }
+    }
+}
+
+template <typename ET, int MODE, typename Sink>
+__device__ __forceinline__ void block(const unsigned char* amax, const ET* g, const ET* z, int img, int bh, int bw, int cq, int h, int w, int c, int ho, int wo,
+                                      const Consts<vc_of<ET>()>& kc, ET* ga, float (&s1)[vc_of<ET>()], float (&s2)[vc_of<ET>()], Sink&& sink) {
+    constexpr int VC = vc_of<ET>();
+    float gv[4][VC], zv[4][VC];
+    unsigned char am[4][VC];
+    bool okw[4];
+#pragma unroll
+    for (int k = 0; k < 4; ++k) {
+        const int oh = bh + (k >> 1), ow = bw + (k & 1);
+        okw[k] = oh < ho && ow < wo;
+        const long oidx = (((long)img * ho + min(oh, ho - 1)) * wo + min(ow, wo - 1)) * c + cq * VC;
+        if constexpr (VC == 8) {
+            const uint2 a8 = *reinterpret_cast<const uint2*>(amax + oidx);
+#pragma unroll
+            for (int j = 0; j < 4; ++j) { am[k][j] = (unsigned char)(a8.x >> (8 * j)); am[k][4 + j] = (unsigned char)(a8.y >> (8 * j)); }
+        } else {
+            const unsigned a4 = *reinterpret_cast<const unsigned*>(amax + oidx);
+#pragma unroll
+            for (int j = 0; j < 4; ++j) am[k][j] = (unsigned char)(a4 >> (8 * j));
+        }
+        ldv<ET, VC>(g + oidx, gv[k]);
+    }
+    long zi[4];
+#pragma unroll
+    for (int p = 0; p < 4; ++p) {
+        zi[p] = (((long)img * h + 2 * bh + (p >> 1)) * w + 2 * bw + (p & 1)) * c + cq * VC;
+        ldv<ET, VC>(z + zi[p], zv[p]);
+    }
+#pragma unroll
+    for (int p = 0; p < 4; ++p) {
+        const int a = p >> 1, b = p & 1;
+        float acc[VC];
+#pragma unroll
+        for (int j = 0; j < VC; ++j) acc[j] = 0.f;
+#pragma unroll
+        for (int k = 0; k < 4; ++k) {
+            const int wi = k >> 1, wj = k & 1;
+            if ((wi == 1 && a == 0) || (wj == 1 && b == 0)) continue;
+            const unsigned me = (unsigned)(a + 1 - 2 * wi) * 3u + (unsigned)(b + 1 - 2 * wj);
+#pragma unroll
+            for (int j = 0; j < VC; ++j)
+                if (okw[k] && am[k][j] == me) acc[j] += gv[k][j];
+        }
+        if constexpr (MODE == 0) {
+            if (ga) *reinterpret_cast<uint4*>(ga + zi[p]) = packv<ET, VC>(acc);
+        }
+        if constexpr (sizeof(ET) == 2) {
+#pragma unroll
+            for (int j = 0; j < VC; ++j) acc[j] = bf16_to_f32(f32_to_bf16(acc[j]));
+        }
+        if constexpr (MODE == 0) {
+#pragma unroll
+            for (int j = 0; j < VC; ++j) {
+                const float gm = (zv[p][j] * kc.scv[j] + kc.shv[j]) > 0.f ? acc[j] : 0.f;
+                s1[j] += gm;
+                s2[j] += gm * ((zv[p][j] - kc.muv[j]) * kc.k1[j]);
+            }
+        } else {
+            float o[VC];
+#pragma unroll
+            for (int j = 0; j < VC; ++j) {
+                const float gm = (zv[p][j] * kc.scv[j] + kc.shv[j]) > 0.f ? acc[j] : 0.f;
+                o[j] = kc.k1[j] * (gm - kc.k2[j] - (zv[p][j] - kc.muv[j]) * kc.k3[j]);
+            }
+            sink(p, zi[p], o);
+        }
+    }
+}
+
+}
diff --git a/mvfnet_amd/csrc/train_ops.hip b/mvfnet_amd/csrc/train_ops.hip
--- a/mvfnet_amd/csrc/train_ops.hip
+++ b/mvfnet_amd/csrc/train_ops.hip
@@ -3,6 +3,7 @@
 #include <stdlib.h>
 
 #include "common.h"
+#include "pool_bn_bwd_blk.h"
 
 namespace {
 
@@ -933,35 +934,11 @@
     __shared__ float red[MODE == 0 ? 256 * 2 * VC : 1];
     const int ncg = c / VC, hw2 = w >> 1, hb = h >> 1;
     const int cq = threadIdx.x % ncg;
-    float scv[VC], shv[VC], muv[VC], k1[VC], k2[VC], k3[VC];
-#pragma unroll
-    for (int j = 0; j < VC; ++j) {
-        const int ch = cq * VC + j;
-        scv[j] = scale[ch]; shv[j] = shift[ch]; muv[j] = mean[ch];
-        if constexpr (MODE == 0) { k1[j] = invstd[ch]; k2[j] = 0.f; k3[j] = 0.f; }
-        else { k1[j] = gamma[ch] * invstd[ch]; k2[j] = dbeta[ch] * inv_m; k3[j] = invstd[ch] * dgamma[ch] * inv_m; }
-    }
+    mvf_poolblk::Consts<VC> kc;
+    mvf_poolblk::load_consts<VC, MODE>(kc, cq, gamma, mean, invstd, scale, shift, dgamma, dbeta, inv_m);
     float s1[VC], s2[VC];
 #pragma unroll
     for (int j = 0; j < VC; ++j) { s1[j] = 0.f; s2[j] = 0.f; }
-    auto ldv = [](const ET* p, float (&f)[VC]) {
-        const uint4 u = *reinterpret_cast<const uint4*>(p);
-        if constexpr (sizeof(ET) == 4) {
-            f[0] = __uint_as_float(u.x); f[1] = __uint_as_float(u.y); f[2] = __uint_as_float(u.z); f[3] = __uint_as_float(u.w);
-        } else {
-            f[0] = __uint_as_float(u.x << 16); f[1] = __uint_as_float(u.x & 0xffff0000u); f[2] = __uint_as_float(u.y << 16); f[3] = __uint_as_float(u.y & 0xffff0000u);
-            f[4] = __uint_as_float(u.z << 16); f[5] = __uint_as_float(u.z & 0xffff0000u); f[6] = __uint_as_float(u.w << 16); f[7] = __uint_as_float(u.w & 0xffff0000u);
-        }
-    };
-    auto stv = [](ET* p, const float (&f)[VC]) {
-        uint4 u;
-        if constexpr (sizeof(ET) == 4) {
-            u = make_uint4(__float_as_uint(f[0]), __float_as_uint(f[1]), __float_as_uint(f[2]), __float_as_uint(f[3]));
-        } else {
-            u = make_uint4(pack_bf16x2(f[0], f[1]), pack_bf16x2(f[2], f[3]), pack_bf16x2(f[4], f[5]), pack_bf16x2(f[6], f[7]));
-        }
-        *reinterpret_cast<uint4*>(p) = u;
-    };
     const int items = (kPoolRB / 2) * hw2 * ncg;
     const long brows = (long)n * hb;
     for (int i = threadIdx.x; i < items; i += 256) {
@@ -970,70 +947,9 @@
         const long R = (long)blockIdx.x * (kPoolRB / 2) + br;
         if (R >= brows) break;
         const int img = (int)(R / hb), bh = (int)(R - (long)img * hb);
-        float gv[4][VC], zv[4][VC];
-        unsigned char am[4][VC];
-        bool okw[4];
-#pragma unroll
-        for (int k = 0; k < 4; ++k) {
-            const int oh = bh + (k >> 1), ow = bw + (k & 1);
-            okw[k] = oh < ho && ow < wo;
-            const long oidx = (((long)img * ho + min(oh, ho - 1)) * wo + min(ow, wo - 1)) * c + cq * VC;
-            if constexpr (VC == 8) {
-                const uint2 a8 = *reinterpret_cast<const uint2*>(amax + oidx);
-#pragma unroll
-                for (int j = 0; j < 4; ++j) { am[k][j] = (unsigned char)(a8.x >> (8 * j)); am[k][4 + j] = (unsigned char)(a8.y >> (8 * j)); }
-            } else {
-                const unsigned a4 = *reinterpret_cast<const unsigned*>(amax + oidx);
-#pragma unroll
-                for (int j = 0; j < 4; ++j) am[k][j] = (unsigned char)(a4 >> (8 * j));
-            }
-            ldv(g + oidx, gv[k]);
-        }
-        long zi[4];
-#pragma unroll
-        for (int p = 0; p < 4; ++p) {
-            zi[p] = (((long)img * h + 2 * bh + (p >> 1)) * w + 2 * bw + (p & 1)) * c + cq * VC;
-            ldv(z + zi[p], zv[p]);
-        }
-#pragma unroll
-        for (int p = 0; p < 4; ++p) {
-            const int a = p >> 1, b = p & 1;
-            float acc[VC];
-#pragma unroll
-            for (int j = 0; j < VC; ++j) acc[j] = 0.f;
-#pragma unroll
-            for (int k = 0; k < 4; ++k) {
-                const int wi = k >> 1, wj = k & 1;
-                if ((wi == 1 && a == 0) || (wj == 1 && b == 0)) continue;
-                const unsigned me = (unsigned)(a + 1 - 2 * wi) * 3u + (unsigned)(b + 1 - 2 * wj);
-#pragma unroll
-                for (int j = 0; j < VC; ++j)
-                    if (okw[k] && am[k][j] == me) acc[j] += gv[k][j];
-            }
-            if constexpr (MODE == 0) {
-                if (ga) stv(ga + zi[p], acc);
-            }
-            if constexpr (sizeof(ET) == 2) {
-#pragma unroll
-                for (int j = 0; j < VC; ++j) acc[j] = bf16_to_f32(f32_to_bf16(acc[j]));
-            }
-            if constexpr (MODE == 0) {
-#pragma unroll
-                for (int j = 0; j < VC; ++j) {
-                    const float gm = (zv[p][j] * scv[j] + shv[j]) > 0.f ? acc[j] : 0.f;
-                    s1[j] += gm;
-                    s2[j] += gm * ((zv[p][j] - muv[j]) * k1[j]);
-                }
-            } else {
-                float o[VC];
-#pragma unroll
-                for (int j = 0; j < VC; ++j) {
-                    const float gm = (zv[p][j] * scv[j] + shv[j]) > 0.f ? acc[j] : 0.f;
-                    o[j] = k1[j] * (gm - k2[j] - (zv[p][j] - muv[j]) * k3[j]);
-                }
-                stv(dz + zi[p], o);
-            }
-        }
+        mvf_poolblk::block<ET, MODE>(amax, g, z, img, bh, bw, cq, h, w, c, ho, wo, kc, ga, s1, s2, [&](int, long zi, const float (&o)[VC]) {
+            *reinterpret_cast<uint4*>(dz + zi) = mvf_poolblk::packv<ET, VC>(o);
+        });
     }
     if constexpr (MODE == 0) {
 #pragma unroll
@@ -1216,7 +1132,16 @@
 __global__ void sqsum_partial_kernel(const float* g, long n, float* part) {
     __shared__ float red[256];
     float s = 0.f;
-    for (long i = (long)blockIdx.x * blockDim.x + threadIdx.x; i < n; i += (long)gridDim.x * blockDim.x) s += g[i] * g[i];
+    const long stride = (long)gridDim.x * blockDim.x;
+    long i = (long)blockIdx.x * blockDim.x + threadIdx.x;
+    for (; i + 7 * stride < n; i += 8 * stride) {
+        float v[8];
+#pragma unroll
+        for (int u = 0; u < 8; ++u) v[u] = g[i + u * stride];
+#pragma unroll
+        for (int u = 0; u < 8; ++u) s += v[u] * v[u];
+    }
+    for (; i < n; i += stride) s += g[i] * g[i];
     red[threadIdx.x] = s;
     __syncthreads();
     for (int o = blockDim.x >> 1; o > 0; o >>= 1) { if (threadIdx.x < o) red[threadIdx.x] += red[threadIdx.x + o]; __syncthreads(); }
@@ -1259,7 +1184,20 @@
 __global__ void sqsum_segments_kernel(const float* g, long n, const mvf_sgd_segment_t* seg, int nseg, float* part) {
     __shared__ float red[256];
     float s = 0.f;
-    for (long i = (long)blockIdx.x * blockDim.x + threadIdx.x; i < n; i += (long)gridDim.x * blockDim.x)
+    const long stride = (long)gridDim.x * blockDim.x;
+    long i = (long)blockIdx.x * blockDim.x + threadIdx.x;
+    for (; i + 7 * stride < n; i += 8 * stride) {
+        float v[8];
+        bool on[8];
+#pragma unroll
+        for (int u = 0; u < 8; ++u) v[u] = g[i + u * stride];
+#pragma unroll
+        for (int u = 0; u < 8; ++u) on[u] = seg[seg_of(seg, nseg, i + u * stride)].lr_mult >= 0.f;
+#pragma unroll
+        for (int u = 0; u < 8; ++u)
+            if (on[u]) s += v[u] * v[u];
+    }
+    for (; i < n; i += stride)
         if (seg[seg_of(seg, nseg, i)].lr_mult >= 0.f) s += g[i] * g[i];
     red[threadIdx.x] = s;
     __syncthreads();
diff --git a/mvfnet_amd/csrc/wgrad_nhwc.hip b/mvfnet_amd/csrc/wgrad_nhwc.hip
--- a/mvfnet_amd/csrc/wgrad_nhwc.hip
+++ b/mvfnet_amd/csrc/wgrad_nhwc.hip
@@ -1131,6 +1131,9 @@
 namespace mvf_internal {
 int wgrad_slab_reduce_launch(const float* part, int nsplit, int cout, int k, float* dw_oihw, hipStream_t st) {
     return launch_wgrad_reduce(part, nsplit, cout, k, 1, 1, 1, k, dw_oihw, st);
+}
+int wgrad_stem_reduce_launch(const float* part, int nsplit, float* dw_oihw, hipStream_t st) {
+    return launch_wgrad_reduce(part, nsplit, 64, 3, 7, 7, 8, 4, dw_oihw, st);
 }
 }
 
diff --git a/mvfnet_amd/csrc/wgrad_stem.hip b/mvfnet_amd/csrc/wgrad_stem.hip
--- a/mvfnet_amd/csrc/wgrad_stem.hip
+++ b/mvfnet_amd/csrc/wgrad_stem.hip
@@ -2,6 +2,7 @@
 #include <stdlib.h>
 
 #include "common.h"
+#include "pool_bn_bwd_blk.h"
 
 namespace {
 
@@ -18,13 +19,18 @@
     int xbytes, dpix;
     int ksr;
     unsigned fd_bpf_mul, fd_bpf_shr, fd_ksr_mul, fd_ksr_shr;
+    const unsigned char* amax;
+    const bf16_t *g, *z;
+    const float *gamma, *mean, *invstd, *scale, *shift, *dgamma, *dbeta;
+    float inv_m;
 };
 
 __device__ __forceinline__ int fdiv(int n, unsigned mul, unsigned shr) { return (int)((__umulhi((unsigned)n, mul) + (unsigned)n) >> shr); }
 __device__ __forceinline__ int swzf(int pixel) { return ((pixel >> 1) & 1) << 2; }
 
-template <int kR>
+template <int kR, bool kPool = false>
 __global__ __launch_bounds__(256, 2) void wgrad_stem_kernel(KArgs a) {
+    static_assert(!kPool || kR == 2, "the pooled form walks 2 x 2 blocks: bands of two rows");
     extern __shared__ __attribute__((aligned(16))) char smem[];
     char* Xs = smem;
     char* Ds = smem + (a.xbytes + 1023) / 1024 * 1024;
@@ -33,10 +39,11 @@
     const int wm = wave & 1, kg = wave >> 1;
     constexpr unsigned kOOB = 0x80000000u;
     const i32x4 gs_x = rsrc_words(a.x, (unsigned)((long)a.N * a.H * a.rowb));
-    const i32x4 gs_d = rsrc_words(a.dz, (unsigned)((long)a.N * a.Ho * a.Wo * 128));
+    const i32x4 gs_d = rsrc_words(kPool ? (const char*)a.z : a.dz, (unsigned)((long)a.N * a.Ho * a.Wo * 128));
     const unsigned lds_x = (unsigned)__builtin_amdgcn_readfirstlane((int)(unsigned)(size_t)(__attribute__((address_space(3))) char*)Xs);
     const unsigned lds_d = (unsigned)__builtin_amdgcn_readfirstlane((int)(unsigned)(size_t)(__attribute__((address_space(3))) char*)Ds);
     const int nx = (a.xbytes + 1023) >> 10, nd = a.dpix >> 3;
+    (void)gs_d; (void)lds_d; (void)nd;
     const int lp = lane >> 3, lu = lane & 7;
 
     const int tg = lane >> 4, ti = lane & 15;
@@ -55,6 +62,10 @@
         return v;
     };
 
+    const int cq = tid & 7;
+    mvf_poolblk::Consts<8> kc;
+    if constexpr (kPool) mvf_poolblk::load_consts<8, 1>(kc, cq, a.gamma, a.mean, a.invstd, a.scale, a.shift, a.dgamma, a.dbeta, a.inv_m);
+
     f32x16 acc[4];
 #pragma unroll
     for (int t = 0; t < 4; ++t)
@@ -72,10 +83,26 @@
                 const int o = i * 1024 + lane * 16;
                 glds16(gs_x, lds_x + (unsigned)(i * 1024), o < a.xbytes ? (unsigned)(xbase + o) : kOOB);
             }
-            const long dbase = ((long)img * a.Ho + oh0) * a.Wo * 128;
-            for (int i = wave; i < nd; i += 4) {
-                const int p = i * 8 + lp;
-                glds16(gs_d, lds_d + (unsigned)(i * 1024), (unsigned)(dbase + p * 128 + ((lu ^ swzf(p)) << 4)));
+            if constexpr (kPool) {
+                typedef unsigned u32x4 __attribute__((ext_vector_type(4)));
+                typedef __attribute__((address_space(3))) u32x4* lds_u4;
+                const int bh = oh0 >> 1, items = (a.Wo >> 1) * 8;
+                float s1[8], s2[8];
+                for (int i = tid; i < items; i += 256) {
+                    const int bw = i >> 3;
+                    mvf_poolblk::block<bf16_t, 1>(a.amax, a.g, a.z, img, bh, bw, cq, a.Ho, a.Wo, 64, a.Ho >> 1, a.Wo >> 1, kc, (bf16_t*)nullptr, s1, s2,
+                                                  [&](int p, long, const float (&o)[8]) {
+                        const int pix = (p >> 1) * a.Wo + 2 * bw + (p & 1);
+                        const uint4 u = mvf_poolblk::packv<bf16_t, 8>(o);
+                        *(lds_u4)(Ds + pix * 128 + ((cq ^ swzf(pix)) << 4)) = u32x4{u.x, u.y, u.z, u.w};
+                    });
+                }
+            } else {
+                const long dbase = ((long)img * a.Ho + oh0) * a.Wo * 128;
+                for (int i = wave; i < nd; i += 4) {
+                    const int p = i * 8 + lp;
+                    glds16(gs_d, lds_d + (unsigned)(i * 1024), (unsigned)(dbase + p * 128 + ((lu ^ swzf(p)) << 4)));
+                }
             }
         }
         asm volatile("s_waitcnt vmcnt(0)" ::: "memory");
@@ -137,12 +164,22 @@
     static const int env = std::max(1, mvf_policy_int("wgrad_stem_wgs", 768));
     return (int)std::min<long>(env, (long)n * (ho / band_rows()));
 }
+int wgrad_stem_pool_wgs(int n, int ho) {
+    static const int env = std::max(1, mvf_policy_int("wgrad_stem_wgs", 768));
+    return (int)std::min<long>(env, (long)n * (ho / 2));
+}
 
 int wgrad_stem_launch(const WgradStemArgs& w, hipStream_t st) {
     KArgs a = {};
     a.dz = (const char*)w.dz; a.x = (const char*)w.x; a.part = w.part;
     a.N = w.N; a.H = w.H; a.W = w.W; a.Ho = w.Ho; a.Wo = w.Wo;
-    const int kR = band_rows();
+    const bool pool = w.dz == nullptr;
+    const int kR = pool ? 2 : band_rows();
+    if (pool) {
+        a.amax = w.amax; a.g = (const bf16_t*)w.g; a.z = (const bf16_t*)w.z;
+        a.gamma = w.gamma; a.mean = w.mean; a.invstd = w.invstd; a.scale = w.scale; a.shift = w.shift; a.dgamma = w.dgamma; a.dbeta = w.dbeta;
+        a.inv_m = 1.0f / (float)((long)w.N * w.Ho * w.Wo);
+    }
     a.bands_per_frame = w.Ho / kR;
     a.bands = w.N * a.bands_per_frame;
     a.rowb = w.W * 8;
@@ -156,12 +193,46 @@
     if (!attr) {
         MVF_HIP_OK(hipFuncSetAttribute((const void*)wgrad_stem_kernel<1>, hipFuncAttributeMaxDynamicSharedMemorySize, 72 * 1024));
         MVF_HIP_OK(hipFuncSetAttribute((const void*)wgrad_stem_kernel<2>, hipFuncAttributeMaxDynamicSharedMemorySize, 72 * 1024));
+        MVF_HIP_OK(hipFuncSetAttribute((const void*)(wgrad_stem_kernel<2, true>), hipFuncAttributeMaxDynamicSharedMemorySize, 72 * 1024));
         attr = true;
     }
-    if (kR == 1) hipLaunchKernelGGL(wgrad_stem_kernel<1>, dim3(w.nwg), dim3(256), lds, st, a);
+    if (pool) hipLaunchKernelGGL((wgrad_stem_kernel<2, true>), dim3(w.nwg), dim3(256), lds, st, a);
+    else if (kR == 1) hipLaunchKernelGGL(wgrad_stem_kernel<1>, dim3(w.nwg), dim3(256), lds, st, a);
     else hipLaunchKernelGGL(wgrad_stem_kernel<2>, dim3(w.nwg), dim3(256), lds, st, a);
     MVF_LAUNCH_CHECK();
     return MVF_OK;
 }
 
 }
+
+extern "C" {
+
+static bool stem_pool_shape_ok(int n, int hp, int wp, int ho, int wo, int dtype) {
+    static const int blk_on = mvf_policy_int("pool_bwd_block", 1);
+    return dtype == MVF_BF16 && blk_on && n > 0 && ho > 0 && wo > 0 && ho % 2 == 0 && wo % 2 == 0 && (long)n * ho < (1L << 31) &&
+           mvf_internal::wgrad_stem_ok(n, hp, wp, ho, wo);
+}
+
+size_t mvf_conv_stem_wgrad_pool_bn_workspace_bytes(int n, int hp, int wp, int ho, int wo, int dtype) {
+    if (!stem_pool_shape_ok(n, hp, wp, ho, wo, dtype)) return 0;
+    return align_up((size_t)mvf_internal::wgrad_stem_pool_wgs(n, ho) * 64 * 224 * sizeof(float), 256);
+}
+
+int mvf_conv_stem_wgrad_pool_bn(const unsigned char* argmax, const void* g, const void* z, const float* gamma, const float* mean, const float* invstd,
+                                const float* scale, const float* shift, const float* dgamma, const float* dbeta, const void* xp, int n, int hp, int wp,
+                                int ho, int wo, float* dw_oihw, void* ws, size_t ws_bytes, int dtype, void* stream) {
+    MVF_REQUIRE(argmax && g && z && gamma && mean && invstd && scale && shift && dgamma && dbeta && xp && dw_oihw && n > 0 && hp > 0 && wp > 0 && ho > 0 && wo > 0,
+                MVF_EINVAL, "conv_stem_wgrad_pool_bn: bad argument");
+    MVF_REQUIRE(dtype == MVF_F32 || dtype == MVF_BF16, MVF_EINVAL, "conv_stem_wgrad_pool_bn: bad dtype");
+    MVF_REQUIRE(stem_pool_shape_ok(n, hp, wp, ho, wo, dtype), MVF_EUNSUPPORTED,
+                "conv_stem_wgrad_pool_bn: bf16 storage, even sides and the direct stem kernel's shapes only (n=%d, %dx%d -> %dx%d); use the separate calls", n, hp, wp, ho, wo);
+    MVF_REQUIRE((uintptr_t)argmax % 8 == 0 && ((uintptr_t)g | (uintptr_t)z | (uintptr_t)xp) % 16 == 0, MVF_EUNSUPPORTED,
+                "conv_stem_wgrad_pool_bn: operands must be 16-byte aligned (argmax: 8); use the separate calls");
+    MVF_REQUIRE(ws && ws_bytes >= mvf_conv_stem_wgrad_pool_bn_workspace_bytes(n, hp, wp, ho, wo, dtype), MVF_EWS, "conv_stem_wgrad_pool_bn: workspace too small");
+    WgradStemArgs w = {nullptr, xp, (float*)ws, n, hp, wp, ho, wo, mvf_internal::wgrad_stem_pool_wgs(n, ho), argmax, g, z, gamma, mean, invstd, scale, shift, dgamma, dbeta};
+    const int rc = mvf_internal::wgrad_stem_launch(w, (hipStream_t)stream);
+    if (rc != MVF_OK) return rc;
+    return mvf_internal::wgrad_stem_reduce_launch((const float*)ws, w.nwg, dw_oihw, (hipStream_t)stream);
+}
+
+}
diff --git a/mvfnet_amd/train_engine.py b/mvfnet_amd/train_engine.py
--- a/mvfnet_amd/train_engine.py
+++ b/mvfnet_amd/train_engine.py
@@ -371,6 +371,20 @@
         def launch():
             check(lib.mvf_conv2d_nhwc_wgrad(C.byref(d), _p(dz), _p(x), _p(x2), kwr, cinr, kwp, cinp, _p(self.dw), _p(ws), ws.numel(), _st()), "conv wgrad")
         eng.on_side(launch)
+
+    def wgrad_pool_bn(self, amax, g, z0, bn, sg, sb, xp, n, hp, wp, ho, wo, eng):
+        nbytes = lib.mvf_conv_stem_wgrad_pool_bn_workspace_bytes(n, hp, wp, ho, wo, eng.dt)
+        if not (self.stem and nbytes):
+            return False
+        ws = eng.workspace(nbytes)
+        rc = lib.mvf_conv_stem_wgrad_pool_bn(_p(amax), _p(g), _p(z0), _p(bn.gamma), _p(bn.mean), _p(bn.invstd), _p(bn.scale), _p(bn.shift), _p(sg), _p(sb),
+                                             _p(xp), n, hp, wp, ho, wo, _p(self.dw), _p(ws), ws.numel(), eng.dt, _st())
+        if rc == -5:
+            if getattr(eng, "_rec", None) is not None:
+                eng._rec.unsupported = "mvf_conv_stem_wgrad_pool_bn refused the step's operands"
+            return False
+        check(rc, "stem wgrad + maxpool/bn backward apply")
+        return True
 
     def fuses_wgrad(self, eng, m, c, mask_mode, nbn=1):
         return (eng.tdtype == torch.bfloat16 and self.kh == 1 and self.kw == 1 and self.stride == 1 and not self.stem and c == self.cout and
@@ -964,6 +978,7 @@
     z3_free_ds = _policy("z3_free_ds", 1)
     fuse_c3_bwd = _policy("fuse_c3_bwd", 1)
     fuse_mvf_stats = _policy("fuse_mvf_stats", 1) != 0
+    stem_wgrad_fused = _policy("stem_wgrad_fused", 0)
     dzfree = _policy("dzfree", 2)
     gate_producer = _policy("gate_producer", 1) != 0
     dzfree_q = _policy("dzfree_q", 1)
@@ -1373,12 +1388,17 @@
         check(lib.mvf_maxpool_bn_relu_bwd_sums(_p(s["amax"]), _p(g), nt, ho, wo, 64, None, _p(s["z0"]), _p(bn.mean), _p(bn.invstd),
                                                _p(bn.scale), _p(bn.shift), _p(part), self.dt, _st()), "maxpool bwd + bn sums")
         check(lib.mvf_bn_bwd_finalize(_p(part), rows, 64, _p(bn.dgamma), _p(bn.dbeta), _st()), "bn bwd finalize")
-        dz0 = self.buf((id(bn), "dz"), s["z0"].shape, s["z0"].dtype)
         sg, sb = (bn._zero, bn._zero) if bn.frozen else (bn.dgamma, bn.dbeta)
-        check(lib.mvf_maxpool_bn_relu_bwd_apply(_p(s["amax"]), _p(g), nt, ho, wo, 64, _p(s["z0"]), _p(bn.gamma), _p(bn.mean), _p(bn.invstd), _p(bn.scale),
-                                                _p(bn.shift), _p(sg), _p(sb), _p(dz0), self.dt, _st()), "maxpool bwd + bn apply")
-        self.flush_side()
-        self.stem.wgrad(dz0, s["xp"], nt, s["hp"], s["wp"], ho, wo, self, on_main=True)
+        fused = False
+        if self.stem_wgrad_fused:
+            self.flush_side()
+            fused = self.stem.wgrad_pool_bn(s["amax"], g, s["z0"], bn, sg, sb, s["xp"], nt, s["hp"], s["wp"], ho, wo, self)
+        if not fused:
+            dz0 = self.buf((id(bn), "dz"), s["z0"].shape, s["z0"].dtype)
+            check(lib.mvf_maxpool_bn_relu_bwd_apply(_p(s["amax"]), _p(g), nt, ho, wo, 64, _p(s["z0"]), _p(bn.gamma), _p(bn.mean), _p(bn.invstd), _p(bn.scale),
+                                                    _p(bn.shift), _p(sg), _p(sb), _p(dz0), self.dt, _st()), "maxpool bwd + bn apply")
+            self.flush_side()
+            self.stem.wgrad(dz0, s["xp"], nt, s["hp"], s["wp"], ho, wo, self, on_main=True)
         self.join_side()
         if self.keep_io:
             self.io = dict(p0=self.buf("p0", (g.shape[0], 64)), g_p0=g, gfeat=self.buf("gfeat", tuple(s["feat_shape"])), nt=nt, b=b, t=t)
```

Result: no change. 1820 clips/s, median of 3 (+0.0%).
